# UncleBrian3007/UncleRenderer

Hardware: AMD Instinct MI355X
Metric: shaded Mpixels/s, 4K deferred pass (BuildHZB + CullIndirectArgs + DeferredLighting/Sky), Sponza; % HBM roofline (higher is better)
Workload: dtype f32

## Files before the change

### include/ur_hotpath.h

```cpp
#ifndef UR_HOTPATH_H
#define UR_HOTPATH_H

#include <stddef.h>
#include <stdint.h>

#ifdef __cplusplus
extern "C" {
#endif

#define UR_OK 0
#define UR_EINVAL (-1)
#define UR_EHIP (-2)
#define UR_ENOMEM (-3)
#define UR_ENODEVICE (-4)
#define UR_EUNSUPPORTED (-5)
#define UR_ETIMEOUT (-6)

#define UR_MAX_HZB_MIPS 16u
#define UR_CULL_CONSTANT_DWORDS 46u
#define UR_INDIRECT_COMMAND_STRIDE 64u
#define UR_INDIRECT_INSTANCE_COUNT_OFFSET 44u

typedef struct ur_ctx ur_ctx;

// ... 64 lines not shown
    uint32_t env_mip_count;
    const uint16_t* brdf_lut_rg16;
    uint32_t lut_width;
    uint32_t lut_height;
    uint64_t env_cube_texels;
} ur_lighting_tables;


ur_ctx* ur_create(int device, void* stream);
void ur_destroy(ur_ctx* ctx);
int ur_reserve(ur_ctx* ctx, uint32_t max_instances);
int ur_defer_hzb_tail(ur_ctx* ctx, int mode );
int ur_flush(ur_ctx* ctx);
int ur_debug_set_hzb_timeout(ur_ctx* ctx);
int ur_debug_lighting_schedule(const ur_ctx* ctx, uint32_t out8[8]);
int ur_debug_stream_ceiling(ur_ctx* ctx, const void* in0, const void* in1, const void* in2, const void* in3, void* out, uint64_t elements16,
                            void* start_event, void* stop_event);
int ur_debug_timeline(ur_ctx* ctx, unsigned long long* device_pairs, uint32_t capacity_pairs);
int ur_time_next_lighting(ur_ctx* ctx, void* start_event, void* stop_event);
int ur_time_next_cull(ur_ctx* ctx, void* stop_event);
int ur_time_cull_carried(const ur_ctx* ctx);

#define UR_OPT_LIGHTING_STREAM 1
#define UR_OPT_LIGHTING_WAVES_PER_WG 2
#define UR_OPT_LIGHTING_TILED_WAVES 3
#define UR_OPT_LIGHTING_LEAVE_CUS 4
#define UR_OPT_RIDE_WALKERS 5
#define UR_OPT_CULL_STORE 7
#define UR_OPT_LIGHTING_BALANCE 8
#define UR_OPT_BALANCE_POOL_16THS 9
#define UR_OPT_BALANCE_CHUNK_SHIFT 10
#define UR_OPT_DEBUG_HZB_RIDE_STALL 11
#define UR_OPT_TAA_TONEMAP_HISTORY_STORE 12
int ur_set_option(ur_ctx* ctx, int option, int value);
int ur_get_option(const ur_ctx* ctx, int option, int* value);
const char* ur_last_error(void);
const char* ur_version(void);


uint32_t ur_hzb_layout(uint32_t src_w, uint32_t src_h, ur_mip_desc* mips ,
                       uint32_t* mip_count);

int ur_build_hzb(ur_ctx* ctx, const float* depth, uint32_t src_w, uint32_t src_h, float* hzb_base,
                 const ur_mip_desc* mips, uint32_t mip_count);

typedef struct ur_hzb_slice {
    uint32_t offset;
    uint32_t count;
} ur_hzb_slice;
int ur_hzb_band_pieces(uint32_t src_h, uint32_t n_ranks, uint32_t rank, uint32_t* piece_row0, uint32_t* piece_rows);
int ur_hzb_band_slices(const ur_mip_desc* mips, uint32_t mip_count, uint32_t piece_row0, uint32_t piece_rows, ur_hzb_slice* out5);
int ur_build_hzb_band(ur_ctx* ctx, const float* depth, uint32_t src_w, uint32_t src_h, float* hzb_base, const ur_mip_desc* mips,
                      uint32_t mip_count, uint32_t piece_row0, uint32_t piece_rows);
int ur_build_hzb_tail(ur_ctx* ctx, float* hzb_base, const ur_mip_desc* mips, uint32_t mip_count);


int ur_cull_indirect_args(ur_ctx* ctx, const uint32_t* constants, const ur_float4* bounds,
                          const float* hzb_base, const ur_mip_desc* mips, void* indirect_args,
                          uint32_t* stats2, uint32_t* visible_idx, uint32_t* visible_count);
int ur_cull_indirect_args_ex(ur_ctx* ctx, const uint32_t* constants, const ur_float4* bounds,
                             const float* hzb_base, const ur_mip_desc* mips, void* indirect_args,
                             uint32_t* stats2, uint32_t* visible_idx, uint32_t* visible_count,
                             uint32_t index_base);

typedef struct ur_draw_ranges {
    const uint32_t* offsets;
// ... 146 lines not shown
```

### unclerenderer_amd/csrc/cull.hip

```cpp

#include "cull_kernels.h"

namespace ur {

int launch_cull(ur_ctx* ctx, const uint32_t* constants, const ur_float4* bounds, const float* hzb, const ur_mip_desc* mips,
                void* indirect_args, uint32_t* stats2, uint32_t* visible_idx, uint32_t* visible_count, uint32_t index_base,
                const ur_draw_ranges* draws, const ur_cull_view* views, uint32_t view_count)
{
    const int rc = flush_hzb_tail(ctx);
    if (rc != UR_OK) return rc;
    if (views != nullptr && view_count != 0) return launch_cull_views(ctx, constants, bounds, hzb, mips, indirect_args, stats2, visible_idx, visible_count, index_base, draws, views, view_count);
    return cull_launches<false>(ctx, constants, bounds, hzb, mips, indirect_args, stats2, visible_idx, visible_count, index_base, draws, nullptr, 0);
}

}
```

### unclerenderer_amd/csrc/cull_kernels.h

```cpp
#pragma once

#include "ur_internal.h"
#include "ur_device.h"

#include <hip/hip_ext.h>

#include <algorithm>
#include <cstring>

namespace {

struct CullParams {
    float4 FrustumPlanes[6];
    float ViewProjection[16];
    uint32_t ModelCount, HZBEnabled, HZBMipCount, HZBWidth, HZBHeight, DebugPrintEnabled;
    const float4* bounds;
    const float* hzb;
    uint8_t* args;
    uint32_t* stats;
    uint32_t* visible_idx;
    uint32_t* visible_count;
    uint32_t* block_counts;
    uint64_t* wave_masks;
    uint32_t index_base;
    uint32_t store_flavour;
    uint32_t record_valid;
    uint32_t mip_offset[UR_MAX_HZB_MIPS];
    uint32_t mip_width[UR_MAX_HZB_MIPS];
    unsigned long long* timeline;
};

struct DrawParams {
    const uint32_t* offsets;
    uint8_t* commands;
    uint32_t* counts;
    uint32_t range_count;
};

struct ViewParams {
    float4 planes[UR_MAX_CULL_VIEWS][6];
    uint32_t* mask[UR_MAX_CULL_VIEWS];
    uint32_t* visible_idx[UR_MAX_CULL_VIEWS];
    uint32_t* visible_count[UR_MAX_CULL_VIEWS];
    DrawParams D[UR_MAX_CULL_VIEWS];
    uint32_t* block_counts[UR_MAX_CULL_VIEWS];
    uint64_t* wave_masks[UR_MAX_CULL_VIEWS];
    uint32_t count;
};

template <bool RANGES, bool VIEWS = false> struct CullArgs : CullParams { DrawParams D; ViewParams V; };
template <> struct CullArgs<false, true> : CullParams { ViewParams V; };
template <> struct CullArgs<true, false> : CullParams { DrawParams D; };
template <> struct CullArgs<false, false> : CullParams {};

__device__ __forceinline__ float saturate_f(float x) { return fminf(fmaxf(x, 0.0f), 1.0f); }
__device__ __forceinline__ float dot3(float ax, float ay, float az, float bx, float by, float bz) { return (ax * bx + ay * by) + az * bz; }

__device__ __forceinline__ bool IsAabbVisible(const CullParams& C, float3 mn, float3 mx)
{
#pragma unroll
    for (int i = 0; i < 6; ++i) {
        const float4 plane = C.FrustumPlanes[i];
        const float px = plane.x >= 0.0f ? mx.x : mn.x;
        const float py = plane.y >= 0.0f ? mx.y : mn.y;
        const float pz = plane.z >= 0.0f ? mx.z : mn.z;
        if (dot3(plane.x, plane.y, plane.z, px, py, pz) + plane.w < 0.0f) return false;
    }
    return true;
}

__device__ __forceinline__ bool IsAabbInCameraFrustum(const float4* planes, float4 bmin, float4 bmax)
{
#pragma unroll
    for (int i = 0; i < 6; ++i) {
        const float4 P = planes[i];
        const float X = P.x >= 0.0f ? bmax.x : bmin.x;
        const float Y = P.y >= 0.0f ? bmax.y : bmin.y;
        const float Z = P.z >= 0.0f ? bmax.z : bmin.z;
        const float d = ((P.x * X + P.y * Y) + P.z * Z) + P.w * 1.0f;
        if (d < 0.0f) return false;
    }
    return true;
}

__device__ __forceinline__ bool IsOccluded(const CullParams& C, float3 mn, float3 mx)
{
    if (C.HZBEnabled == 0 || C.HZBWidth == 0 || C.HZBHeight == 0 || C.HZBMipCount == 0) return false;
    const float* M = C.ViewProjection;
    float minUx = 1.0f, minUy = 1.0f, maxUx = 0.0f, maxUy = 0.0f, maxDepth = 0.0f;
    bool anyBehind = false;
#pragma unroll
    for (int i = 0; i < 8; ++i) {
        const float cx = (i & 1) ? mx.x : mn.x, cy = (i & 2) ? mx.y : mn.y, cz = (i & 4) ? mx.z : mn.z;
        const float clx = ((cx * M[0] + cy * M[4]) + cz * M[8]) + 1.0f * M[12];
        const float cly = ((cx * M[1] + cy * M[5]) + cz * M[9]) + 1.0f * M[13];
        const float clz = ((cx * M[2] + cy * M[6]) + cz * M[10]) + 1.0f * M[14];
        const float clw = ((cx * M[3] + cy * M[7]) + cz * M[11]) + 1.0f * M[15];
        if (clw <= 0.0f) anyBehind = true;
        const float nx = clx / clw, ny = cly / clw, nz = clz / clw;
        const float ux = nx * 0.5f + 0.5f;
        const float uy = 1 - (ny * 0.5f + 0.5f);
        minUx = fminf(minUx, ux); minUy = fminf(minUy, uy);
        maxUx = fmaxf(maxUx, ux); maxUy = fmaxf(maxUy, uy);
        maxDepth = fmaxf(maxDepth, nz);
    }
    if (anyBehind) return false;
    if (maxUx < 0.0f || maxUy < 0.0f || minUx > 1.0f || minUy > 1.0f) return false;
    minUx = saturate_f(minUx); minUy = saturate_f(minUy);
    maxUx = saturate_f(maxUx); maxUy = saturate_f(maxUy);
    const float ex = maxUx - minUx, ey = maxUy - minUy;
    const float psx = ex * (float)C.HZBWidth, psy = ey * (float)C.HZBHeight;
    const float maxDim = fmaxf(psx, psy);
    uint32_t mipLevel = 0;
    if (maxDim > 1.0f) {
        const uint32_t e = ((__float_as_uint(maxDim) >> 23) & 0xFFu) - 127u;
        const float l = fminf(fmaxf((float)e, 0.0f), (float)(C.HZBMipCount - 1u));
        mipLevel = (uint32_t)l;
    }
    const uint32_t mipWidth = max(1u, C.HZBWidth >> mipLevel);
// ... 95 lines not shown
#pragma unroll
    for (uint32_t v = 0; v < UR_MAX_CULL_VIEWS; ++v) {
        if (v >= V.count) break;
        const uint64_t m = __ballot(active && IsAabbInCameraFrustum(V.planes[v], bmin, bmax));
        if (V.mask[v] != nullptr && lane < 2u) {
            const uint32_t w = wave_global * 2u + lane;
            if (w < words) V.mask[v][w] = (uint32_t)(m >> (32u * lane));
        }
        if (lane == 0) {
            svmask[v][wave] = m;
            if (!SINGLE_BLOCK && V.wave_masks[v] != nullptr) V.wave_masks[v][wave_global] = m;
        }
    }
}

template <bool SINGLE_BLOCK>
__device__ __forceinline__ void FinishViews(const ViewParams& V, const uint8_t* args, uint32_t n, uint32_t index_base, const uint64_t (*svmask)[4])
{
    const uint32_t tid = threadIdx.x;
#pragma unroll
    for (uint32_t v = 0; v < UR_MAX_CULL_VIEWS; ++v) {
        if (v >= V.count) break;
        const uint32_t total = __popcll(svmask[v][0]) + __popcll(svmask[v][1]) + __popcll(svmask[v][2]) + __popcll(svmask[v][3]);
        if (SINGLE_BLOCK) {
            if (V.visible_idx[v] != nullptr) {
                ScatterBlock(V.visible_idx[v], index_base, 0, svmask[v], 0);
                if (tid == 0) *V.visible_count[v] = total;
            }
            if (V.D[v].range_count != 0) PlaceBlock(V.D[v], args, svmask[v], n);
        } else if (tid == v && V.block_counts[v] != nullptr) V.block_counts[v][blockIdx.x] = total;
    }
}

template <bool SINGLE_BLOCK, bool RANGES, bool VIEWS = false>
__global__ __launch_bounds__(256) void cull_kernel(CullArgs<RANGES, VIEWS> C)
{
    __shared__ float4 sb[512];
    __shared__ uint64_t smask[4];
    __shared__ uint32_t scand[4];
    __shared__ uint8_t slist[256], socc[256];

    const uint32_t tid = threadIdx.x, lane = tid & 63u, wave = tid >> 6;
    const uint32_t first = blockIdx.x * 256u;
    const uint32_t index = first + tid;
    ur::timeline_entry(C.timeline);

    const uint32_t nb = min(512u, (C.ModelCount - first) * 2u);
    const float4* src = C.bounds + (size_t)first * 2u;
    typedef float cf32x4_t __attribute__((ext_vector_type(4)));
    const cf32x4_t* srcv = reinterpret_cast<const cf32x4_t*>(src);
    const cf32x4_t v0 = __builtin_nontemporal_load(srcv + min(tid, nb - 1u)), v1 = __builtin_nontemporal_load(srcv + min(tid + 256u, nb - 1u));
    const float4 s0 = make_float4(v0.x, v0.y, v0.z, v0.w), s1 = make_float4(v1.x, v1.y, v1.z, v1.w);

    bool visible = false, frustumVisible = true, occluded = false;
    const bool active = index < C.ModelCount;
    uint32_t old_word = 0xFFFFFFFFu;
    const bool from_record = !SINGLE_BLOCK && C.store_flavour == 4u && C.record_valid != 0u;
    uint64_t old_mask = 0;
    if (from_record) old_mask = C.wave_masks[(size_t)blockIdx.x * 4u + wave];
    else if (C.store_flavour >= 3u)
        old_word = *reinterpret_cast<const uint32_t*>(C.args + (size_t)min(index, C.ModelCount - 1u) * UR_INDIRECT_COMMAND_STRIDE + UR_INDIRECT_INSTANCE_COUNT_OFFSET);
    if (tid < nb) sb[tid] = s0;
    if (tid + 256u < nb) sb[tid + 256u] = s1;
    __syncthreads();
    if (active) {
        const float4 bmin = sb[2u * tid], bmax = sb[2u * tid + 1u];
        frustumVisible = IsAabbVisible(C, make_float3(bmin.x, bmin.y, bmin.z), make_float3(bmax.x, bmax.y, bmax.z));
    }
    if (SINGLE_BLOCK) {
        if (active && frustumVisible && C.HZBEnabled != 0) {
            const float4 bmin = sb[2u * tid], bmax = sb[2u * tid + 1u];
            occluded = IsOccluded(C, make_float3(bmin.x, bmin.y, bmin.z), make_float3(bmax.x, bmax.y, bmax.z));
        }
    } else if (C.HZBEnabled != 0) {
        const bool cand = active && frustumVisible;
        const uint64_t cm = __ballot(cand);
        if (lane == 0) scand[wave] = (uint32_t)__popcll(cm);
        __syncthreads();
        uint32_t at = 0, total = 0;
#pragma unroll
        for (uint32_t w = 0; w < 4u; ++w) { at += w < wave ? scand[w] : 0u; total += scand[w]; }
        if (cand) slist[at + (uint32_t)__popcll(cm & ((1ull << lane) - 1ull))] = (uint8_t)tid;
        __syncthreads();
        if (tid < total) {
            const uint32_t j = slist[tid];
            const float4 bmin = sb[2u * j], bmax = sb[2u * j + 1u];
            socc[j] = IsOccluded(C, make_float3(bmin.x, bmin.y, bmin.z), make_float3(bmax.x, bmax.y, bmax.z)) ? 1u : 0u;
        }
        __syncthreads();
        occluded = cand && socc[tid] != 0u;
    }
    if (active) {
        visible = frustumVisible && !occluded;
        uint32_t* word = reinterpret_cast<uint32_t*>(C.args + (size_t)index * UR_INDIRECT_COMMAND_STRIDE + UR_INDIRECT_INSTANCE_COUNT_OFFSET);
        const uint32_t value = visible ? 1u : 0u;
        if (C.store_flavour >= 3u) {
            if (from_record) old_word = (uint32_t)(old_mask >> lane) & 1u;
            if (old_word != value) asm volatile("global_store_dword %0, %1, off sc1" ::"v"(word), "v"(value) : "memory");
        } else if (C.store_flavour == 2u) asm volatile("global_store_dword %0, %1, off sc1" ::"v"(word), "v"(value) : "memory");
        else if (C.store_flavour == 1u) __builtin_nontemporal_store(value, word);
        else *word = value;
    }
    [[maybe_unused]] __shared__ uint64_t svmask[VIEWS ? UR_MAX_CULL_VIEWS : 1][4];
    if constexpr (VIEWS) CullViews<SINGLE_BLOCK>(C.V, C.ModelCount, active, sb, svmask);

    if (C.DebugPrintEnabled != 0 && C.stats != nullptr) {
        const uint32_t nf = __popcll(__ballot(active && !frustumVisible));
        const uint32_t no = __popcll(__ballot(active && frustumVisible && occluded));
        if (lane == 0) {
            if (nf) atomicAdd(&C.stats[0], nf);
            if (no) atomicAdd(&C.stats[1], no);
        }
    }

    if (!RANGES && !VIEWS && C.visible_idx == nullptr) {
        if (!SINGLE_BLOCK && C.store_flavour == 4u) {
            const uint64_t m = __ballot(visible);
            if (lane == 0) C.wave_masks[(size_t)blockIdx.x * 4u + wave] = m;
        }
        ur::timeline_exit(C.timeline, tid == 0);
        return;
    }
    const uint64_t mask = __ballot(visible);
    if (lane == 0) smask[wave] = mask;
    __syncthreads();
    if (SINGLE_BLOCK) {
        if ((!RANGES && !VIEWS) || C.visible_idx != nullptr) {
            ScatterBlock(C.visible_idx, C.index_base, 0, smask, 0);
            if (tid == 0) *C.visible_count = __popcll(smask[0]) + __popcll(smask[1]) + __popcll(smask[2]) + __popcll(smask[3]);
        }
        if constexpr (RANGES) PlaceBlock(C.D, C.args, smask, C.ModelCount);
    } else {
        if (lane == 0) C.wave_masks[(size_t)blockIdx.x * 4u + wave] = mask;
        if (tid == 0) C.block_counts[blockIdx.x] = __popcll(smask[0]) + __popcll(smask[1]) + __popcll(smask[2]) + __popcll(smask[3]);
    }
    if constexpr (VIEWS) FinishViews<SINGLE_BLOCK>(C.V, C.args, C.ModelCount, C.index_base, svmask);
    ur::timeline_exit(C.timeline, tid == 0);
}

template <bool VIEWS, class Args> __device__ __forceinline__ const auto* SelectRow(const Args* C, const CullArgs<true>* W)
{
    if constexpr (VIEWS) return W;
    else return C;
}

template <bool RANGES, bool VIEWS> struct CompactRow { typedef CullArgs<true> type; };
template <bool RANGES> struct CompactRow<RANGES, false> { typedef CullArgs<RANGES> type; };

template <bool RANGES, bool VIEWS = false>
__global__ __launch_bounds__(256) void compact_kernel(CullArgs<RANGES, VIEWS> C, uint32_t num_blocks)
{
    [[maybe_unused]] CullArgs<true> W{};
    if constexpr (VIEWS) {
        W.ModelCount = C.ModelCount;
        W.args = C.args;
        W.index_base = C.index_base;
        if (blockIdx.y == 0) {
            W.wave_masks = C.wave_masks;
            W.block_counts = C.block_counts;
            W.visible_idx = C.visible_idx;
            W.visible_count = C.visible_count;
            if constexpr (RANGES) W.D = C.D;
        } else {
#pragma unroll
            for (uint32_t v = 0; v < UR_MAX_CULL_VIEWS; ++v) {
                if (v + 1u != blockIdx.y) continue;
                W.wave_masks = C.V.wave_masks[v];
                W.block_counts = C.V.block_counts[v];
                W.visible_idx = C.V.visible_idx[v];
                W.visible_count = C.V.visible_count[v];
                W.D = C.V.D[v];
            }
// ... 94 lines not shown
        const uint32_t b = __builtin_ctzll(bits);
        A.visible_idx[at++] = first + b;
        bits &= bits - 1ull;
    }
    if (mi == num_masks - 1u) *A.visible_count = at;
}

struct ZeroArgs {
    uint32_t* count[1 + UR_MAX_CULL_VIEWS];
    uint32_t* counts[1 + UR_MAX_CULL_VIEWS];
    uint32_t range_count[1 + UR_MAX_CULL_VIEWS];
};
__global__ void zero_views_kernel(ZeroArgs Z)
{
    const uint32_t i = blockIdx.x * 256u + threadIdx.x;
#pragma unroll
    for (uint32_t k = 0; k < 1u + UR_MAX_CULL_VIEWS; ++k) {
        if (i == 0 && Z.count[k]) *Z.count[k] = 0;
        if (i < Z.range_count[k]) Z.counts[k][i] = 0;
    }
}

template <class K, class... Args>
int launch_stop(ur_ctx* ctx, hipEvent_t stop, K kernel, dim3 grid, const Args&... args)
{
    if (stop != nullptr) hipExtLaunchKernelGGL(kernel, grid, dim3(256), 0, ctx->stream, nullptr, stop, 0, args...);
    else hipLaunchKernelGGL(kernel, grid, dim3(256), 0, ctx->stream, args...);
    UR_HIP_TRY(hipGetLastError());
    return UR_OK;
}

DrawParams draw_params(const ur_draw_ranges& d) { return {d.offsets, static_cast<uint8_t*>(d.commands), d.counts, d.range_count}; }

template <bool VIEWS>
int cull_launches(ur_ctx* ctx, const uint32_t* constants, const ur_float4* bounds, const float* hzb, const ur_mip_desc* mips,
                  void* indirect_args, uint32_t* stats2, uint32_t* visible_idx, uint32_t* visible_count, uint32_t index_base,
                  const ur_draw_ranges* draws, const ur_cull_view* views, uint32_t view_count)
{
    if constexpr (!VIEWS) view_count = 0;
    CullArgs<true, VIEWS> P{};
    static_assert(sizeof(float4) * 6 + sizeof(float) * 16 + 6 * 4 == UR_CULL_CONSTANT_DWORDS * 4, "46 dwords");
    std::memcpy(static_cast<CullParams*>(&P), constants, UR_CULL_CONSTANT_DWORDS * 4);
    P.bounds = reinterpret_cast<const float4*>(bounds);
    P.hzb = hzb;
    P.args = static_cast<uint8_t*>(indirect_args);
    P.stats = stats2;
    P.visible_idx = visible_idx;
    P.visible_count = visible_count;
    P.index_base = index_base;
    P.store_flavour = (uint32_t)ctx->opt.cull_store;
    P.timeline = P.ModelCount != 0 ? ur::next_timeline_pair(ctx) : nullptr;
    if (P.HZBEnabled != 0) {
        for (uint32_t m = 0; m < P.HZBMipCount && m < UR_MAX_HZB_MIPS; ++m) {
            P.mip_offset[m] = mips[m].offset;
            P.mip_width[m] = mips[m].width;
        }
    }
    if (draws) P.D = draw_params(*draws);
    if constexpr (VIEWS) {
        P.V.count = view_count;
        for (uint32_t v = 0; v < view_count; ++v) {
            std::memcpy(P.V.planes[v], views[v].planes, sizeof(P.V.planes[v]));
            P.V.mask[v] = views[v].mask;
            P.V.visible_idx[v] = views[v].visible_idx;
            P.V.visible_count[v] = views[v].visible_count;
            if (views[v].draws) P.V.D[v] = draw_params(*views[v].draws);
        }
    }
    const uint32_t n = P.ModelCount;
    bool record_valid = P.store_flavour == 4u && ctx->cull_record_args == indirect_args && ctx->cull_record_n == n;
    ctx->cull_record_args = nullptr;
    hipEvent_t stop = ctx->time_cull_stop;
    auto compacted = [&](uint32_t v) { return views[v].visible_idx != nullptr || views[v].draws != nullptr; };

    if (n == 0) {
        ZeroArgs Z{};
        Z.count[0] = visible_count;
        if (draws) { Z.counts[0] = draws->counts; Z.range_count[0] = draws->range_count; }
        bool zero = visible_count != nullptr || draws != nullptr;
        uint32_t most = Z.range_count[0];
        for (uint32_t v = 0; v < view_count; ++v) {
            zero = zero || views[v].visible_count || views[v].draws;
            Z.count[1 + v] = views[v].visible_count;
            if (views[v].draws) {
                Z.counts[1 + v] = views[v].draws->counts;
                Z.range_count[1 + v] = views[v].draws->range_count;
                most = std::max(most, views[v].draws->range_count);
            }
        }
        if (!zero) return UR_OK;
// ... 22 lines not shown
        }
        P.block_counts = ctx->block_counts;
        P.wave_masks = ctx->wave_masks;
        if constexpr (VIEWS) {
            const uint32_t stride = ctx->ws_instances / 256u;
            for (uint32_t v = 0; v < view_count; ++v) {
                if (!compacted(v)) continue;
                compact = true;
                P.V.block_counts[v] = ctx->block_counts + (size_t)(1u + v) * stride;
                P.V.wave_masks[v] = ctx->wave_masks + (size_t)(1u + v) * stride * 4u;
            }
        }
    }
    P.record_valid = record_valid ? 1u : 0u;
    static_cast<CullParams&>(Q) = P;
    if constexpr (VIEWS) Q.V = P.V;
    const dim3 compaction_grid((blocks * 4u + 255u) / 256u, 1u + view_count);
    if (draws) {
        rc = launch_stop(ctx, compact ? nullptr : stop, cull_kernel<false, true, VIEWS>, dim3(blocks), P);
        if (rc == UR_OK && compact) rc = launch_stop(ctx, stop, compact_kernel<true, VIEWS>, compaction_grid, P, blocks);
    } else {
        rc = launch_stop(ctx, compact ? nullptr : stop, cull_kernel<false, false, VIEWS>, dim3(blocks), Q);
        if (rc == UR_OK && compact) rc = launch_stop(ctx, stop, compact_kernel<false, VIEWS>, compaction_grid, Q, blocks);
    }
    if (rc != UR_OK) return rc;
    if (P.store_flavour == 4u) {
        ctx->cull_record_args = indirect_args;
        ctx->cull_record_n = n;
    }
    ctx->time_cull_carried = stop != nullptr;
    return UR_OK;
}

}
```

### unclerenderer_amd/csrc/debug_print.hip

```cpp

#include "ur_internal.h"

namespace {

constexpr uint32_t kHeaderDwords = 1u;
constexpr uint32_t kEntryDwords = 4u;
constexpr uint32_t kMaxEntries = UR_DEBUG_PRINT_MAX_ENTRIES;
constexpr uint32_t kAdvance = 8u;
constexpr uint32_t kTextChunk = 256u;

__device__ __forceinline__ void print_char(uint32_t* buf, uint32_t x, uint32_t y, uint32_t code, uint32_t color)
{
    const uint32_t index = atomicAdd(buf, 1u);
    if (index >= kMaxEntries) return;
    uint32_t* e = buf + kHeaderDwords + index * kEntryDwords;
    e[0] = x; e[1] = y; e[2] = code; e[3] = color;
}

__device__ void print_label(uint32_t* buf, uint32_t x, uint32_t y, uint32_t color, const char (&c)[9])
{
    for (uint32_t i = 0; i < 8u; ++i) {
        const uint32_t code = (uint32_t)(uint8_t)c[i];
        if (code == 0u) return;
        print_char(buf, x, y, code, color);
// ... 148 lines not shown
        const int iu = (int)fu;
        const float dv = g.UvMax[1] - g.UvMin[1];
#pragma unroll
        for (uint32_t k = 0; k < kRowsPerThread; ++k) {
            const uint32_t ly = ly0 + k * kRowStep;
            const float cy = (float)(p.row0 + ly) + 0.5f;
            if (!(ly < p.rows && q.miny <= cy && cy < q.maxy)) continue;
            const float v = g.UvMin[1] + (cy - q.miny) / g.Size[1] * dv;
            const float tv = v * ah - 0.5f, fv = floorf(tv), wv = tv - fv;
            const int iv = (int)fv;
            const float t00 = atlas_texel(p, iu, iv), t10 = atlas_texel(p, iu + 1, iv), t01 = atlas_texel(p, iu, iv + 1), t11 = atlas_texel(p, iu + 1, iv + 1);
            const float top = t00 + (t10 - t00) * wu, bot = t01 + (t11 - t01) * wu;
            const float a = ca * (top + (bot - top) * wv);
            const uint32_t d = pix[k];
            const float ia = 1.0f - a;
            const float dr = (float)(d & 255u) / 255.0f, dg = (float)((d >> 8) & 255u) / 255.0f, db = (float)((d >> 16) & 255u) / 255.0f;
            pix[k] = unorm8(cr * a + dr * ia) | (unorm8(cg * a + dg * ia) << 8) | (unorm8(cb * a + db * ia) << 16) | (unorm8(a) << 24);
            dirty |= 1u << k;
        }
    }
#pragma unroll
    for (uint32_t k = 0; k < kRowsPerThread; ++k) {
        const uint32_t ly = ly0 + k * kRowStep;
        if (dirty & (1u << k)) p.ldr[(size_t)ly * p.w + px] = pix[k];
    }
}

}

namespace ur {

int launch_debug_print_reset(ur_ctx* ctx, void* buffer, uint32_t* stats)
{
    hipLaunchKernelGGL(debug_print_reset_kernel, dim3(1), dim3(64), 0, ctx->stream, static_cast<uint32_t*>(buffer), stats);
    UR_HIP_TRY(hipGetLastError());
    return UR_OK;
}

int launch_debug_print_stats(ur_ctx* ctx, const uint32_t* stats, void* buffer)
{
    hipLaunchKernelGGL(debug_print_stats_kernel, dim3(1), dim3(64), 0, ctx->stream, stats, static_cast<uint32_t*>(buffer));
    UR_HIP_TRY(hipGetLastError());
    return UR_OK;
}

int launch_debug_print_text(ur_ctx* ctx, void* buffer, uint32_t x, uint32_t y, uint32_t color, const char* text, uint32_t length)
{
    uint32_t n = 0;
    while (n < length && text[n] != 0) ++n;
    for (uint32_t at = 0; at < n; at += kTextChunk) {
        TextChunk chunk = {};
        const uint32_t count = n - at < kTextChunk ? n - at : kTextChunk;
        for (uint32_t i = 0; i < count; ++i) chunk.c[i] = (uint8_t)text[at + i];
        hipLaunchKernelGGL(debug_print_text_kernel, dim3(1), dim3(kTextChunk), 0, ctx->stream, static_cast<uint32_t*>(buffer), x + kAdvance * at, y, color,
                           count, chunk);
        UR_HIP_TRY(hipGetLastError());
    }
    return UR_OK;
}

int launch_debug_print_draw(ur_ctx* ctx, const ur_debug_print_constants* constants, const ur_debug_glyph* glyphs, uint32_t glyph_count,
                            const uint8_t* atlas_r8, uint32_t atlas_w, uint32_t atlas_h, const void* buffer, uint32_t* ldr_inout, uint32_t w,
                            uint32_t row0, uint32_t rows)
{
    if (rows == 0) return UR_OK;
    DrawParams p{};
    p.glyphs = glyphs; p.atlas = atlas_r8; p.buf = static_cast<const uint32_t*>(buffer); p.ldr = ldr_inout;
    p.glyph_count = glyph_count; p.atlas_w = atlas_w; p.atlas_h = atlas_h;
    p.first_char = constants->FirstChar; p.char_count = constants->CharCount;
    p.w = w; p.row0 = row0; p.rows = rows;
    const dim3 grid((w + kTileW - 1u) / kTileW, (rows + kTileH - 1u) / kTileH);
    if (grid.y > 65535u) { set_error("ur_debug_print_draw: band too tall"); return UR_EUNSUPPORTED; }
    hipLaunchKernelGGL(debug_print_draw_kernel, grid, dim3(kThreads), 0, ctx->stream, p);
    UR_HIP_TRY(hipGetLastError());
    return UR_OK;
}

}
```

### unclerenderer_amd/csrc/frame/HotPathRenderer.cpp

```cpp

#include "HotPathRenderer.h"

#include <hip/hip_runtime.h>

#include <cstdio>
#include <cstring>
#include <sstream>

#include "../../../include/ur_frame.h"
#include "../../../include/ur_host.h"
#include "../ur_internal.h"

int FHotPathRenderer::RenderFrame(FHIPCommandContext& Cmd, FHotPathResources& Res, const FHotPathFrameConstants& Constants,
                                  const FHotPathOptions& Options)
{
    PassError = UR_OK;
    if (bPostPending) {
        bPostPending = false;
        bLuminanceHistoryValid = false;
        ResetTaa();
    }
    FRenderGraph Graph;
    Graph.SetDevice(Device);
    Graph.SetGpuTimingEnabled(Options.bGpuTiming);
// ... 947 lines not shown
    O.bTaaBand = (flags & UR_FRAME_TAA_BAND) != 0;
    O.bDebugPrint = (flags & UR_FRAME_DEBUG_PRINT) != 0;
    O.bShardHZB = (flags & UR_FRAME_HZB_SHARD) != 0 && f->Cmd.GetWorldSize() > 1;
    O.bAsyncCompute = (flags & UR_FRAME_ASYNC_COMPUTE) != 0;
    if (O.bAsyncCompute && !f->AsyncCtx) {
        int dev = 0;
        if (hipGetDevice(&dev) != hipSuccess || hipStreamCreateWithPriority(&f->AsyncStream, hipStreamNonBlocking, -1) != hipSuccess) return UR_EHIP;
        f->AsyncCtx = ur_create(dev, f->AsyncStream);
        if (!f->AsyncCtx) return UR_EHIP;
        f->Cmd.SetAsyncCompute(f->AsyncCtx, f->AsyncStream);
    }
    O.bTimeLighting = (flags & (UR_FRAME_TIME_LIGHTING | UR_FRAME_TIME_LIGHTING_RECORD_COST | UR_FRAME_TIME_LIGHTING_KERNEL)) != 0;
    f->bKernelEvents = (flags & UR_FRAME_TIME_LIGHTING_KERNEL) != 0;
    f->bRecordAfter = (flags & UR_FRAME_TIME_LIGHTING_RECORD_COST) != 0;
    O.bGpuTiming = (flags & UR_FRAME_GPU_TIMING) != 0;
    O.bGraphDump = (flags & UR_FRAME_GRAPH_DUMP) != 0;
    O.bBarrierLogs = (flags & UR_FRAME_BARRIER_LOGS) != 0;
    f->Cmd.SetJoinAsyncAtEnd((flags & UR_FRAME_ASYNC_NO_JOIN) == 0);
    f->Cmd.BeginFrame();
    const bool chain_with_lighting = (flags & UR_FRAME_HZB_WITH_LIGHTING) != 0 && !O.bAsyncCompute;
    const bool tail_with_lighting = (chain_with_lighting || (flags & UR_FRAME_HZB_TAIL_WITH_LIGHTING) != 0) && !O.bAsyncCompute;
    if (tail_with_lighting) (void)ur_defer_hzb_tail(f->Cmd.GetContext(), chain_with_lighting ? 2 : 1);
    f->bStartOnCull = false;
    if (f->bKernelEvents && chain_with_lighting && O.bEnableIndirectDraw && O.bHZBEnabled && O.bDoDepthPrepass && R.IndirectArgs && R.ModelBounds &&
        R.IndirectCommandCount != 0) {
        constexpr size_t kRing = 1024;
        if (f->LightEvents.size() < kRing && f->LightCount == f->LightEvents.size()) {
            hipEvent_t a = nullptr, b = nullptr, c = nullptr;
            if (hipEventCreate(&a) == hipSuccess && hipEventCreate(&b) == hipSuccess && hipEventCreate(&c) == hipSuccess) f->LightEvents.push_back({a, b, c, false, false});
        }
        if (!f->LightEvents.empty() && ur_time_next_cull(f->Cmd.GetContext(), f->LightEvents[f->LightCount % f->LightEvents.size()].first) == UR_OK)
            f->bStartOnCull = true;
    }
    const int rc = f->Renderer.RenderFrame(f->Cmd, R, K, O);
    (void)ur_time_next_cull(f->Cmd.GetContext(), nullptr);
    if (tail_with_lighting) {
        const int rc2 = ur_defer_hzb_tail(f->Cmd.GetContext(), 0);
        const int rc3 = ur_flush(f->Cmd.GetContext());
        return rc != UR_OK ? rc : (rc2 != UR_OK ? rc2 : rc3);
    }
    return rc;
}

void ur_frame_join_async(ur_frame* f) { if (f) f->Cmd.JoinAsyncCompute(); }
int ur_frame_hzb_ready(const ur_frame* f) { return f && f->Renderer.IsHZBReady() ? 1 : 0; }
void ur_frame_reset_hzb(ur_frame* f) { if (f) f->Renderer.ResetHZB(); }

int ur_frame_set_post(ur_frame* f, const ur_frame_post* post)
{
    if (!f || !post) { ur::set_error("ur_frame_set_post: null argument"); return UR_EINVAL; }
    f->Post = *post;
    return UR_OK;
}

int ur_frame_set_draw_ranges(ur_frame* f, const ur_draw_ranges* draws)
{
    if (!f) { ur::set_error("ur_frame_set_draw_ranges: null frame"); return UR_EINVAL; }
    if (draws && (!draws->offsets || !draws->commands || !draws->counts || draws->range_count == 0)) {
        ur::set_error("ur_frame_set_draw_ranges: null member / no range");
        return UR_EINVAL;
    }
    f->bDrawRanges = draws != nullptr;
    f->DrawRanges = draws ? *draws : ur_draw_ranges{};
    return UR_OK;
}

int ur_frame_set_cull_views(ur_frame* f, const ur_cull_view* views, uint32_t count)
// ... 165 lines not shown
```

### unclerenderer_amd/csrc/gbuffer_resolve.hip

```cpp

#include "raster_rule.h"
#include "texture_sample.h"
#include "ur_device.h"
#include "ur_internal.h"

namespace {

using namespace ur_raster;

static_assert(sizeof(ur_texture2d) == 16 && sizeof(ur_material) == 80, "ur_material is 80 bytes");

struct ResolveParams {
    const uint8_t* commands;
    uint32_t mode;
    const uint32_t* visible_idx;
    uint32_t index_base;
    float V[16], Pr[16];
    const uint32_t* keys;
    uint2* gbuf_a; uint2* gbuf_b; uint32_t* gbuf_c; uint2* hdr; uint32_t* object_id;
    const float* table;
    uint32_t w, row0, n;
    float half_w, half_h;
    uint32_t key_bits;
    const ur_material* materials;
// ... 288 lines not shown
    ur::store_once_b64(p.gbuf_a + i, pack_half4(m[0] / ml, m[1] / ml, m[2] / ml, view_depth));
    ur::store_once_b64(p.gbuf_b + i, pack_half4(0.04f, cb[104], cb[105], 1.0f));
    ur::store_once_b32(p.gbuf_c + i, r8 | (g8 << 8) | (b8 << 16) | 0xFF000000u);
    ur::store_once_b64(p.hdr + i, pack_half4(cb[80], cb[81], cb[82], 1.0f));
    if constexpr (OBJECT_ID) ur::store_once_b32(p.object_id + i, reinterpret_cast<const uint32_t*>(cb)[148]);
}

int gbuffer_entry(const char* who, const char* who_parts, ur_ctx* ctx, const float* view, const float* projection, const ur_raster_draws* draws, const float* depth,
                  const ur_gbuffer_targets* targets, uint32_t w, uint32_t h, uint32_t row0, uint32_t rows, uint32_t flags, uint32_t key_triangle_bits,
                  uint32_t* stats6, uint32_t parts, const ur_material* materials, uint32_t material_count)
{
    int rc = ur::check_raster_call(who, ctx, view, projection, draws, depth, "depth", w, h, stats6);
    if (rc == UR_OK) rc = ur::check_depth_flags(who, flags);
    if (rc == UR_OK) rc = ur::check_gbuffer_targets(who, targets);
    if (rc == UR_OK) rc = ur::check_key_triangle_bits(who, key_triangle_bits);
    if (rc != UR_OK) return rc;
    if (rows == 0u || (uint64_t)row0 + rows > h) { ur::set_error("%s: rows [%u, %u + %u) of a target %u high", who, row0, row0, rows, h); return UR_EINVAL; }
    if (parts == 0u || (parts & ~(UR_GBUFFER_PART_RASTER | UR_GBUFFER_PART_RESOLVE))) { ur::set_error("%s: parts 0x%x (UR_GBUFFER_PART_RASTER | UR_GBUFFER_PART_RESOLVE)", who_parts, parts); return UR_EINVAL; }
    uint32_t key_bits = key_triangle_bits;
    if (key_bits == 0u) {
        if (draws->command_count >= (1u << 24)) {
            ur::set_error("%s: %u command slots leave fewer than 8 key bits for the triangle: pass key_triangle_bits", who, draws->command_count);
            return UR_EUNSUPPORTED;
        }
        uint32_t length = 0u;
        while ((draws->command_count >> length) != 0u) ++length;
        key_bits = min(32u - length, 31u);
    } else if ((uint64_t)draws->command_count >= (1ull << (32u - key_bits))) {
        ur::set_error("%s: %u command slots do not fit the %u key bits beside key_triangle_bits %u", who, draws->command_count, 32u - key_bits, key_bits);
        return UR_EINVAL;
    }
    if (!aligned(materials, 16)) { ur::set_error("%s: a misaligned material table (16 bytes)", who); return UR_EINVAL; }
    const uint32_t n = w * rows;
    if (parts & UR_GBUFFER_PART_RASTER) {
        rc = ur::launch_visibility_raster(ctx, view, projection, draws, depth, targets->keys, w, h, row0, rows, key_bits, (flags & UR_DEPTH_QUANTIZE_D24) != 0u, stats6);
        if (rc != UR_OK) return rc;
    }
    if (!(parts & UR_GBUFFER_PART_RESOLVE)) return UR_OK;
    ResolveParams r{};
    r.commands = static_cast<const uint8_t*>(ur::raster_commands(*draws));
    r.mode = draws->visible_idx != nullptr ? 1u : 0u;
    r.visible_idx = draws->visible_idx; r.index_base = draws->index_base;
    for (int k = 0; k < 16; ++k) { r.V[k] = view[k]; r.Pr[k] = projection[k]; }
    r.keys = targets->keys;
    r.gbuf_a = reinterpret_cast<uint2*>(targets->gbuf_a); r.gbuf_b = reinterpret_cast<uint2*>(targets->gbuf_b); r.gbuf_c = targets->gbuf_c;
    r.hdr = reinterpret_cast<uint2*>(targets->hdr); r.object_id = targets->object_id;
    r.table = ctx->srgb_encode_table;
    r.w = w; r.row0 = row0; r.n = n;
    r.half_w = 0.5f * (float)w; r.half_h = 0.5f * (float)h;
    r.key_bits = key_bits;
    const uint32_t blocks = (n + kThreads - 1u) / kThreads;
    if (materials) {
        r.materials = materials; r.material_count = material_count;
        r.decode = ctx->srgb_table; r.lod = ctx->lod_table;
        if (targets->object_id) hipLaunchKernelGGL((gbuffer_resolve_kernel<true, true>), dim3(blocks), dim3(kThreads), 0, ctx->stream, r);
        else hipLaunchKernelGGL((gbuffer_resolve_kernel<false, true>), dim3(blocks), dim3(kThreads), 0, ctx->stream, r);
        UR_HIP_TRY(hipGetLastError());
        return UR_OK;
    }
    if (targets->object_id) hipLaunchKernelGGL(gbuffer_resolve_kernel<true>, dim3(blocks), dim3(kThreads), 0, ctx->stream, r);
    else hipLaunchKernelGGL(gbuffer_resolve_kernel<false>, dim3(blocks), dim3(kThreads), 0, ctx->stream, r);
    UR_HIP_TRY(hipGetLastError());
    return UR_OK;
}

}
// ... 49 lines not shown
```

### unclerenderer_amd/csrc/hzb.hip

```cpp

#include "ur_internal.h"
#include "ur_device.h"
#include "hzb_tail.h"
#include "hzb_wide.h"

namespace {

using ur::HzbDispatch;

using ur::hzb_min4;

__global__ __launch_bounds__(256) void hzb_reduce4_kernel(HzbDispatch p)
{
    __shared__ float sh2[4][16];
    __shared__ float sh3[2][8];

    const uint32_t tx = threadIdx.x & 31u, ty = threadIdx.x >> 5;
    const uint32_t by = blockIdx.y + p.by0;
    const uint32_t x1 = blockIdx.x * 32u + tx, y1 = by * 8u + ty;
    const uint32_t sx = x1 * 4u, sy = y1 * 4u;

    float v0[2][2] = {{1.0f, 1.0f}, {1.0f, 1.0f}};
    const bool any0 = (x1 * 2u < p.W[0]) && (y1 * 2u < p.H[0]);
    if (any0) {
// ... 57 lines not shown
    if (((tx | ty) & 3u) == 0u) {
        const uint32_t x3 = x1 >> 2, y3 = y1 >> 2;
        if (x3 < p.W[3] && y3 < p.H[3]) {
            const uint32_t cx = tx >> 1, cy = ty >> 1;
            const float v3 = hzb_min4(sh2[cy][cx], sh2[cy][cx + 1], sh2[cy + 1][cx], sh2[cy + 1][cx + 1]);
            p.dst[3][(size_t)y3 * p.W[3] + x3] = v3;
            sh3[ty >> 2][tx >> 2] = v3;
        }
    }
    if (p.mips < 5u) return;
    __syncthreads();

    if (threadIdx.x < 4u) {
        const uint32_t x4 = blockIdx.x * 4u + threadIdx.x, y4 = by;
        if (x4 < p.W[4] && y4 < p.H[4]) {
            const uint32_t c0 = min(2u * x4, p.W[3] - 1u) & 7u, c1 = min(2u * x4 + 1u, p.W[3] - 1u) & 7u;
            const uint32_t r0 = min(2u * y4, p.H[3] - 1u) & 1u, r1 = min(2u * y4 + 1u, p.H[3] - 1u) & 1u;
            p.dst[4][(size_t)y4 * p.W[4] + x4] = hzb_min4(sh3[r0][c0], sh3[r0][c1], sh3[r1][c0], sh3[r1][c1]);
        }
    }
}

__global__ __launch_bounds__(1024) void hzb_tail_kernel(ur::HzbTail p)
{
    __shared__ float bufA[ur::kTailTexels], bufB[ur::kTailTexels / 2];
    ur::hzb_tail_run(p, bufA, bufB);
}

}

namespace ur {

static HzbTail make_tail(float* hzb, const ur_mip_desc* mips, uint32_t mip_count, uint32_t mip);

int launch_build_hzb(ur_ctx* ctx, const float* depth, uint32_t src_w, uint32_t src_h, float* hzb, const ur_mip_desc* mips,
                     uint32_t mip_count)
{
    {
        const int rc = flush_hzb_tail(ctx);
        if (rc != UR_OK) return rc;
    }
    uint32_t mip = 0;
    while (mip < mip_count) {
        if (mip > 0 && (uint64_t)mips[mip].width * mips[mip].height <= kTailTexels && mip_count - mip <= kTailMaxLevels) {
            const HzbTail t = make_tail(hzb, mips, mip_count, mip);
            if (ctx->defer_hzb_tail) {
                ctx->pending_tail = t;
                ctx->hzb_tail_pending = true;
                break;
            }
            hipLaunchKernelGGL(hzb_tail_kernel, dim3(1), dim3(1024), 0, ctx->stream, t);
            UR_HIP_TRY(hipGetLastError());
            break;
        }
        uint32_t n = (mip_count - mip) < 4u ? (mip_count - mip) : 4u;
        if (mip == 0 && mip_count > 4u && (uint64_t)mips[4].width * mips[4].height <= kTailTexels) n = 5u;
        else if (mip == 0 && mip_count > 5u && (uint64_t)mips[5].width * mips[5].height <= kTailTexels &&
                 mip_count - 5u <= kTailMaxLevels) n = 5u;
        HzbDispatch d{};
        if (mip == 0) {
            d.src = depth;
            d.SW = src_w;
            d.SH = src_h;
        } else {
            d.src = hzb + mips[mip - 1].offset;
            d.SW = mips[mip - 1].width;
            d.SH = mips[mip - 1].height;
        }
        for (uint32_t k = 0; k < 5; ++k) {
            if (k < n) {
                d.dst[k] = hzb + mips[mip + k].offset;
                d.W[k] = mips[mip + k].width;
// ... 20 lines not shown
        hipLaunchKernelGGL(hzb_reduce4_kernel, grid, dim3(256), 0, ctx->stream, d);
        UR_HIP_TRY(hipGetLastError());
        mip += n;
    }
    return UR_OK;
}

static bool chain_is_wide_plus_tail(const ur_mip_desc* mips, uint32_t mip_count)
{
    return mip_count > 5u && (uint64_t)mips[5].width * mips[5].height <= kTailTexels && mip_count - 5u <= kTailMaxLevels;
}

static HzbTail make_tail(float* hzb, const ur_mip_desc* mips, uint32_t mip_count, uint32_t mip)
{
    HzbTail t{};
    t.src = hzb + mips[mip - 1].offset;
    t.SW = mips[mip - 1].width;
    t.SH = mips[mip - 1].height;
    t.first_mip = mip;
    t.levels = mip_count - mip;
    for (uint32_t k = 0; k < t.levels; ++k) {
        t.dst[k] = hzb + mips[mip + k].offset;
        t.W[k] = mips[mip + k].width;
        t.H[k] = mips[mip + k].height;
        t.magic[k] = t.W[k] > 1u ? (uint32_t)((1ull << 32) / t.W[k] + 1ull) : 0u;
    }
    return t;
}

int launch_build_hzb_band(ur_ctx* ctx, const float* depth, uint32_t src_w, uint32_t src_h, float* hzb, const ur_mip_desc* mips, uint32_t mip_count,
                          uint32_t piece_row0, uint32_t piece_rows)
{
    {
        const int rc = flush_hzb_tail(ctx);
        if (rc != UR_OK) return rc;
    }
    if (!chain_is_wide_plus_tail(mips, mip_count)) {
        set_error("ur_build_hzb_band: a %u x %u frame's chain is not one five-level launch plus the tail (build it whole: ur_build_hzb)", src_w, src_h);
        return UR_EUNSUPPORTED;
    }
    HzbDispatch d{};
    d.src = depth; d.SW = src_w; d.SH = src_h;
    for (uint32_t k = 0; k < 5; ++k) { d.dst[k] = hzb + mips[k].offset; d.W[k] = mips[k].width; d.H[k] = mips[k].height; }
    d.mips = 5u;
    d.vec4_ok = ((d.SW & 3u) == 0u && (reinterpret_cast<uintptr_t>(d.src) & 15u) == 0u) ? 1u : 0u;
    d.pair_ok = ((d.W[0] & 1u) == 0u && (reinterpret_cast<uintptr_t>(d.dst[0]) & 7u) == 0u) ? 1u : 0u;
    d.by0 = piece_row0;
    const dim3 grid((d.W[0] + 63u) / 64u, piece_rows);
    if (piece_rows == 0u) return UR_OK;
    if (ctx->defer_hzb_tail && ctx->defer_hzb_wide) {
        ctx->pending_wide = d;
        ctx->pending_wide_grid_x = grid.x;
        ctx->pending_wide_grid_y = grid.y;
        ctx->hzb_wide_pending = true;
        return UR_OK;
    }
    hipLaunchKernelGGL(hzb_reduce4_kernel, grid, dim3(256), 0, ctx->stream, d);
    UR_HIP_TRY(hipGetLastError());
    return UR_OK;
}

int launch_build_hzb_tail(ur_ctx* ctx, float* hzb, const ur_mip_desc* mips, uint32_t mip_count)
{
    {
        const int rc = flush_hzb_tail(ctx);
        if (rc != UR_OK) return rc;
    }
    if (!chain_is_wide_plus_tail(mips, mip_count)) {
        set_error("ur_build_hzb_tail: the chain is not one five-level launch plus the tail");
        return UR_EUNSUPPORTED;
    }
    hipLaunchKernelGGL(hzb_tail_kernel, dim3(1), dim3(1024), 0, ctx->stream, make_tail(hzb, mips, mip_count, 5u));
    UR_HIP_TRY(hipGetLastError());
    return UR_OK;
}

int flush_hzb_tail(ur_ctx* ctx)
{
    if (ctx->hzb_wide_pending) {
        ctx->hzb_wide_pending = false;
        hipLaunchKernelGGL(hzb_reduce4_kernel, dim3(ctx->pending_wide_grid_x, ctx->pending_wide_grid_y), dim3(256), 0, ctx->stream, ctx->pending_wide);
        UR_HIP_TRY(hipGetLastError());
    }
    if (!ctx->hzb_tail_pending) return UR_OK;
    ctx->hzb_tail_pending = false;
    hipLaunchKernelGGL(hzb_tail_kernel, dim3(1), dim3(1024), 0, ctx->stream, ctx->pending_tail);
    UR_HIP_TRY(hipGetLastError());
    return UR_OK;
}

}
```

### unclerenderer_amd/csrc/lighting.hip

```cpp

#include "lighting_device.h"
#include "ur_device.h"
#include "hzb_tail.h"

#include <cstring>

namespace {

using namespace ur;

typedef float f2_t __attribute__((ext_vector_type(2)));
__device__ __forceinline__ f2_t f2(float x, float y) { return f2_t{x, y}; }

__device__ __forceinline__ float shadow_pcf_border_inline(const float* __restrict__ map, int W, int H, int ia, int ja, float fx, float fy, float cmp)
{
    float acc = 0.0f;
#pragma unroll
    for (int r = 0; r < 3; ++r) {
        float s = 0.0f;
        const int yj = ja + r;
        const uint32_t rowo = (uint32_t)min(max(yj, 0), H - 1) * (uint32_t)W;
#pragma unroll
        for (int c = 0; c < 3; ++c) {
            const int xi = ia + c;
            const bool in = (uint32_t)xi < (uint32_t)W && (uint32_t)yj < (uint32_t)H;
            const float t = in ? ld<float>(map, (rowo + (uint32_t)min(max(xi, 0), W - 1)) * 4u) : 1.0f;
            s += cmp <= t ? (c == 0 ? 1.0f - fx : (c == 1 ? 1.0f : fx)) : 0.0f;
        }
        acc = fmaf(r == 0 ? 1.0f - fy : (r == 1 ? 1.0f : fy), s, acc);
    }
    return 0.25f * acc;
}

constexpr uint32_t kLutE = kLutW + 2;
constexpr uint32_t kLdsSrgb = 0;
constexpr uint32_t kLdsIrrBytes = 6 * 9 * 64;
// ... 119 lines not shown
    uint32_t r;
    asm("s_cmp_eq_u64 %1, -1\n\ts_cselect_b32 %0, 1, 0" : "=s"(r) : "s"(m) : "scc");
    return r;
}

struct __attribute__((aligned(16))) MipEntry { float Nf, rowBf, faceBf, offBf; };

template <class V>
__device__ __forceinline__ void need(const V& a, const V& b, const V& c, const V& d)
{
    asm volatile("" ::"v"(a), "v"(b), "v"(c), "v"(d));
}

__device__ __forceinline__ uint32_t dyn_slot_load(const uint32_t* slot)
{
    return __builtin_amdgcn_readfirstlane(__hip_atomic_load(slot, __ATOMIC_RELAXED, __HIP_MEMORY_SCOPE_WORKGROUP));
}
template <class P>
__device__ __forceinline__ uint32_t dyn_slot_wait(const uint32_t* slot, P kp)
{
    uint32_t e = dyn_slot_load(slot), spins = 0;
    while (e == kDynNotReady) {
        __builtin_amdgcn_s_sleep(8);
        e = dyn_slot_load(slot);
        if (++spins > (1u << 21)) {
            __hip_atomic_store(kp->bal.timedOut, 1u, __ATOMIC_RELAXED, __HIP_MEMORY_SCOPE_SYSTEM);
            e = kDynEnd;
            break;
        }
    }
    return e;
}
template <class P>
__device__ __forceinline__ uint32_t dyn_claim(P kp, uint32_t* work, uint32_t* dynT, uint32_t c, uint32_t lane)
{
    const uint32_t d = c - kp->hot.staticClaims;
    const uint32_t s = min(d >> kp->bal.dynShift, kDynSlots - 1u);
    const uint32_t e = dyn_slot_wait(dynT + s, kp);
    if (e >= kDynEnd) return 0xFFFFFFFFu;
    const uint32_t idx = d & ((1u << kp->bal.dynShift) - 1u);
    if (idx == 0u) {
        const uint32_t k = s + kp->bal.lookahead;
        if (k < kDynSlots) {
            uint32_t out = kDynEnd;
            if (dyn_slot_wait(dynT + (k - 1u), kp) < kDynEnd && k + 1u < kDynSlots) {
                uint32_t v = 0;
                if (lane == 0) v = __hip_atomic_fetch_add(kp->bal.words + (blockIdx.x >> 3) * ur::kClaimWordStride, 1u, __ATOMIC_RELAXED, __HIP_MEMORY_SCOPE_AGENT);
                v = __builtin_amdgcn_readfirstlane(v);
                if (v < dyn_slot_load(work + 5)) out = kp->bal.staticTiles + ((dyn_slot_load(work + 4) + v) << kp->bal.dynShift);
                else {
                    uint32_t done = 0;
                    if (lane == 0) done = __hip_atomic_fetch_add(kp->bal.words + ur::kClaimWords * ur::kClaimWordStride, 1u, __ATOMIC_RELAXED, __HIP_MEMORY_SCOPE_AGENT);
                    if (__builtin_amdgcn_readfirstlane(done) == kp->hot.groups - 1u && lane <= ur::kClaimWords)
                        __hip_atomic_store(kp->bal.words + lane * ur::kClaimWordStride, 0u, __ATOMIC_RELAXED, __HIP_MEMORY_SCOPE_AGENT);
                }
            }
            if (lane == 0) __hip_atomic_store(dynT + k, out, __ATOMIC_RELAXED, __HIP_MEMORY_SCOPE_WORKGROUP);
        }
    }
    return e + idx;
}

__device__ __forceinline__ void store_hdr(void* base, uint32_t byte_offset, uint32_t lo, uint32_t hi)
{
    typedef uint32_t u32x2_t __attribute__((ext_vector_type(2)));
    const u32x2_t v = {lo, hi};
    asm volatile("global_store_dwordx2 %0, %1, %2 sc1 nt" ::"v"(byte_offset), "v"(v), "s"(base) : "memory");
}

struct HzbRide {
    ur::HzbDispatch d;
    uint32_t grid_x, pieces;
    uint32_t walkers;
    uint32_t want;
    uint32_t spin_limit;
    uint32_t pad;
    uint32_t* done;
    uint32_t* timed_out;
};

template <int MODE, bool SHADOWS, bool IRR_LDS, int WPB, bool RIDE_ALL>
__global__ __launch_bounds__(64 * WPB, 1) void lighting_stream_kernel(LightingParams p, ur::HzbTail hzbTail, HzbRide hzbRide)
{
    static_assert(MODE != ur::UR_MODE_SKY, "sky-only uses the per-tile kernel");
    ur::warm_kernarg<sizeof(LightingParams)>();
    extern __shared__ __attribute__((aligned(16))) unsigned char smem[];
    ur::timeline_entry(p.timeline);
    if (blockIdx.x >= p.hot.groups) {
        if constexpr (WPB == 16) {
            static_assert(kLdsTiles + 16u * 2u * kTileBytes >= (ur::kTailTexels + ur::kTailTexels / 2u) * sizeof(float), "the tail's two level buffers fit the launch's LDS");
            float* bufA = reinterpret_cast<float*>(smem);
            auto ka = __builtin_amdgcn_kernarg_segment_ptr();
            asm volatile("" : "+s"(ka));
            typedef const __attribute__((address_space(4))) ur::HzbTail* KTail;
            typedef const __attribute__((address_space(4))) HzbRide* KRide;
            static_assert(sizeof(LightingParams) % 8 == 0 && sizeof(ur::HzbTail) % 8 == 0, "the kernel arguments follow one another without padding");
            const KRide ride = (KRide)((const __attribute__((address_space(4))) char*)ka + sizeof(LightingParams) + sizeof(ur::HzbTail));
            if (ride->pieces != 0u) {
                if (threadIdx.x == 0) {
                    uint32_t* done = ride->done;
                    const uint32_t want = ride->want, limit = ride->spin_limit;
                    const bool stale = __hip_atomic_load(done + 1, __ATOMIC_RELAXED, __HIP_MEMORY_SCOPE_AGENT) != 0u;
                    uint32_t spins = 0;
                    bool gave_up = false;
                    while (__hip_atomic_load(done, __ATOMIC_RELAXED, __HIP_MEMORY_SCOPE_AGENT) < want) {
                        __builtin_amdgcn_s_sleep(32);
                        if (++spins > limit) { gave_up = true; break; }
                    }
                    __builtin_amdgcn_fence(__ATOMIC_ACQUIRE, "agent");
                    asm volatile("s_waitcnt vmcnt(0)" ::: "memory");
                    if (gave_up || stale) {
                        __hip_atomic_store(ride->timed_out, 1u, __ATOMIC_RELAXED, __HIP_MEMORY_SCOPE_SYSTEM);
                        if (gave_up) __hip_atomic_store(done + 1, 1u, __ATOMIC_RELAXED, __HIP_MEMORY_SCOPE_AGENT);
                    } else {
                        __hip_atomic_store(done, 0u, __ATOMIC_RELAXED, __HIP_MEMORY_SCOPE_AGENT);
                    }
                }
                __syncthreads();
            }
            if (ride->pieces != 0u) ur::hzb_tail_run<true>(*(KTail)((const __attribute__((address_space(4))) char*)ka + sizeof(LightingParams)), bufA, bufA + ur::kTailTexels);
            else ur::hzb_tail_run<false>(*(KTail)((const __attribute__((address_space(4))) char*)ka + sizeof(LightingParams)), bufA, bufA + ur::kTailTexels);
        }
        ur::timeline_exit(p.timeline, threadIdx.x == 0);
        return;
    }
    float* srgb = reinterpret_cast<float*>(smem + kLdsSrgb);
    MipEntry* mipT = reinterpret_cast<MipEntry*>(smem + kLdsMip);
    float4a* irrT = reinterpret_cast<float4a*>(smem + kLdsIrr);
    float2* lut = reinterpret_cast<float2*>(smem + kLdsLut);
    uint32_t* work = reinterpret_cast<uint32_t*>(smem + kLdsWork);
    uint32_t* dynT = reinterpret_cast<uint32_t*>(smem + kLdsDyn);

    const uint32_t lane = threadIdx.x & 63u;
    const uint32_t wave = __builtin_amdgcn_readfirstlane(threadIdx.x >> 6);
    constexpr uint32_t T = 64 * WPB, kLutN = kLutE * (kLutH + 2u), kLutTrips = (kLutN + T - 1) / T;
    uint32_t lt[kLutTrips];
#pragma unroll
    for (uint32_t k = 0; k < kLutTrips; ++k) {
        const uint32_t i = min(threadIdx.x + k * T, kLutN - 1u);
        const uint32_t by = i / kLutE, bx = i - by * kLutE;
        const uint32_t sx = min(max(bx, 1u), kLutW) - 1u, sy = min(max(by, 1u), kLutH) - 1u;
        lt[k] = p.lut[sy * kLutW + sx];
    }
    const float sv = threadIdx.x < 256u ? p.srgb[threadIdx.x] : 0.0f;
    half4_t ih = {}, ih10 = {}, ih01 = {}, ih11 = {};
    const uint32_t irrE = p.irrN0 + 2u;
    const uint32_t irrC = p.irrN0 + 1u, irrCount = IRR_LDS ? 6u * irrC * irrC : 0u;
    if (threadIdx.x < irrCount) {
        const uint32_t f = threadIdx.x / (irrC * irrC), r = threadIdx.x - f * irrC * irrC, cj = r / irrC, ci = r - cj * irrC;
        const uint32_t t0 = p.irrOffset0 + (f * irrE + cj) * irrE + ci;
        ih = p.env[t0]; ih10 = p.env[t0 + 1u]; ih01 = p.env[t0 + irrE]; ih11 = p.env[t0 + irrE + 1u];
    }
    constexpr uint32_t cs = kChunkShift, cmask = (1u << cs) - 1u;
    const uint32_t chunkStride = p.hot.groups << cs, base = blockIdx.x << cs;
    uint32_t tile = (wave >> cs) * chunkStride + base + (wave & cmask);
    uint32_t tile1 = ((wave + WPB) >> cs) * chunkStride + base + ((wave + WPB) & cmask);
    const bool have0 = tile < p.hot.numTiles;
    uint32_t ty = (uint32_t)(((uint64_t)tile * p.hot.tilesXMagic) >> 32), tx = tile - ty * p.hot.tilesX;
    uint32_t ty1 = (uint32_t)(((uint64_t)tile1 * p.hot.tilesXMagic) >> 32), tx1 = tile1 - ty1 * p.hot.tilesX;
    const uint32_t col = lane & 15u, row = lane >> 4;
    const TileSrc src = tile_src<MODE>(&p, lane, 3u);
    const uint32_t bufBase = __builtin_amdgcn_readfirstlane(lds_address(smem + kLdsTiles + wave * (2u * kTileBytes)));
    const unsigned char* myTiles = smem + kLdsTiles + wave * (2u * kTileBytes);
    const uint32_t laneHdr = (row * p.hot.W + col) * 8u;


    if (have0) tile_prefetch<MODE>(&p, p.hot.W, p.hot.rows, src, lane, tx, ty, bufBase);
    const uint32_t cubeLds = __builtin_amdgcn_readfirstlane(lds_address(smem + kLdsTiles + WPB * (2u * kTileBytes)));
    const uint32_t cubeLdsAdj = p.hot.cubeLdsBase - cubeLds;
    {
        const uint32_t nb = p.hot.cubeLdsBytes;
        for (uint32_t pc = wave; pc * 1024u < nb; pc += WPB) {
            const uint32_t at = min(pc * 1024u + lane * 16u, nb - 16u);
            dma16(reinterpret_cast<const char*>(p.hot.env) + p.hot.cubeLdsBase + at, cubeLds + pc * 1024u);
        }
    }
    const float ndcxL = fmaf((float)col, p.invW2, 0.5f * p.invW2 - 1.0f);
    const float rowh = (float)row + 0.5f;
    const float negBig = vreg(-0x1p126f);
    float R[9], WC[3], shC[3], shT[3];
#pragma unroll
    for (int k = 0; k < 9; ++k) R[k] = vreg(p.hot.R[k]);
#pragma unroll
    for (int k = 0; k < 3; ++k) {
        WC[k] = vreg(p.hot.WC[k]); shC[k] = vreg(p.hot.shC[k]); shT[k] = vreg(p.hot.shT[k]);
    }
    {
        if (threadIdx.x == 0) { work[0] = 2u * WPB; work[1] = 0u; work[2] = 0u; work[3] = 0u; }
        if (p.bal.poolChunks != 0u && threadIdx.x < kDynSlots) {
            const uint32_t q8 = blockIdx.x & ~7u, nq = min(8u, p.hot.groups - q8), j = blockIdx.x - q8, la = p.bal.lookahead;
            const uint32_t P0 = (uint32_t)(((unsigned long long)q8 * p.bal.poolMagic) >> 32);
            const uint32_t P1 = (uint32_t)(((unsigned long long)(q8 + nq) * p.bal.poolMagic) >> 32);
            const uint32_t first = P0 + la * nq;
            dynT[threadIdx.x] = threadIdx.x < la ? p.bal.staticTiles + ((P0 + j * la + threadIdx.x) << p.bal.dynShift) : kDynNotReady;
            if (threadIdx.x == 0) { work[4] = first; work[5] = P1 - first; }
        }
        if (threadIdx.x < 256u) srgb[threadIdx.x] = sv;
        if (threadIdx.x < irrCount) {
            const float a[3] = {(float)ih.x, (float)ih.y, (float)ih.z}, b[3] = {(float)ih10.x, (float)ih10.y, (float)ih10.z};
            const float c[3] = {(float)ih01.x, (float)ih01.y, (float)ih01.z}, d[3] = {(float)ih11.x, (float)ih11.y, (float)ih11.z};
            float A_[3], B_[3], C_[3], D_[3];
#pragma unroll
            for (int k = 0; k < 3; ++k) { A_[k] = a[k]; B_[k] = b[k] - a[k]; C_[k] = c[k] - a[k]; D_[k] = (d[k] - b[k]) - (c[k] - a[k]); }
            irrT[threadIdx.x * 4u + 0u] = float4a{A_[0], A_[1], B_[0], B_[1]};
            irrT[threadIdx.x * 4u + 1u] = float4a{C_[0], C_[1], D_[0], D_[1]};
            irrT[threadIdx.x * 4u + 2u] = float4a{A_[2], B_[2], C_[2], D_[2]};
        }
        if (threadIdx.x < 17u) {
            const uint32_t m = min(threadIdx.x, p.envMips - 1u);
            const uint32_t N = max(1u, p.envBase >> m), E = N + 2u;
            uint32_t bordered = 0u, before = 0u;
            for (uint32_t k = 0; k < p.envMips; ++k) {
                const uint32_t e = max(1u, p.envBase >> k) + 2u;
                bordered += 6u * e * e;
                if (k < m) before += 6u * e * (e - 1u);
            }
            mipT[threadIdx.x] = MipEntry{(float)N, (float)(12u * E), (float)(12u * E * (E - 1u)), (float)(bordered * 8u + before * 12u)};
        }
#pragma unroll
        for (uint32_t k = 0; k < kLutTrips; ++k) {
            const uint32_t i = threadIdx.x + k * T;
            if (i < kLutN) lut[i] = float2{(float)(lt[k] & 0xFFFFu) * (1.0f / 65535.0f), (float)(lt[k] >> 16) * (1.0f / 65535.0f)};
        }
    }
    __syncthreads();
    if (have0 && tile1 < p.hot.numTiles) {
        tile_prefetch<MODE>(&p, p.hot.W, p.hot.rows, src, lane, tx1, ty1, bufBase + kTileBytes);
        asm volatile("s_waitcnt vmcnt(2)" ::: "memory");
    } else {
        asm volatile("s_waitcnt vmcnt(0)" ::: "memory");
    }
    if (lane == 0) __hip_atomic_fetch_add(work + 3, 1u, __ATOMIC_RELAXED, __HIP_MEMORY_SCOPE_WORKGROUP);

    if constexpr (WPB == 16) {
        constexpr uint32_t kWalkers = WPB;
        if (RIDE_ALL || wave == kWalkers - 1u) {
            auto ka = __builtin_amdgcn_kernarg_segment_ptr();
            asm volatile("" : "+s"(ka));
            typedef const __attribute__((address_space(4))) HzbRide* KRide;
            const KRide ride = (KRide)((const __attribute__((address_space(4))) char*)ka + sizeof(LightingParams) + sizeof(ur::HzbTail));
            const uint32_t pieces = ride->pieces;
            if (pieces != 0u) {
                const uint32_t gx = ride->grid_x, groups = p.hot.groups;
                float* sh2 = reinterpret_cast<float*>(smem + kLdsHzb) + (RIDE_ALL ? wave * 80u : 0u);
                const uint32_t first = RIDE_ALL ? blockIdx.x + (kWalkers - 1u - wave) * groups : blockIdx.x, step = RIDE_ALL ? groups * kWalkers : groups;
                __builtin_amdgcn_s_setprio(3);
                for (uint32_t piece = first; piece < pieces; piece += step) {
                    const uint32_t by = piece / gx, bx = piece - by * gx;
                    ur::hzb_wide_piece_by_one_wave<true>(ride->d, bx, by + ride->d.by0, lane, sh2, sh2 + 64);
                }
                asm volatile("s_waitcnt vmcnt(0)" ::: "memory");
                __builtin_amdgcn_s_setprio(0);
                bool signals = true;
                if (RIDE_ALL) {
                    uint32_t before = 0;
                    if (lane == 0) before = __hip_atomic_fetch_add(work + 2, 1u, __ATOMIC_RELAXED, __HIP_MEMORY_SCOPE_WORKGROUP);
                    signals = __builtin_amdgcn_readfirstlane(before) == kWalkers - 1u;
                }
                uint32_t* done = ride->done;
                if (signals && done != nullptr) {
                    uint64_t keep_exec;
                    const uint32_t zero = 0u, one = 1u;
                    asm volatile("s_mov_b64 %0, exec\n\ts_mov_b64 exec, 1\n\tglobal_atomic_add %1, %2, %3\n\ts_mov_b64 exec, %0"
                                 : "=&s"(keep_exec)
                                 : "v"(zero), "v"(one), "s"(done)
                                 : "memory");
                }
            }
        }
    }

    uint32_t parity = 0;
#define UR_PREFETCH_POINT()                                                                                              \
    do {                                                                                                                 \
        const uint32_t c = __builtin_amdgcn_readfirstlane(claim);             \
        if (__builtin_expect(c >= p.hot.staticClaims, 0)) tile2 = dyn_claim(kp, work, dynT, c, lane);       \
        else tile2 = (c >> cs) * chunkStride + base + (c & cmask);                                                       \
        uint32_t in_band;                                                                                                \
        asm("s_cmp_lt_u32 %1, %2\n\ts_cselect_b32 %0, 1, 0" : "=s"(in_band) : "s"(tile2), "s"(p.hot.numTiles) : "scc"); \
        more2 = in_band & more1;                                                 \
        if (more2) {                                                                                                     \
            ty2 = __builtin_amdgcn_readfirstlane((uint32_t)(((uint64_t)tile2 * p.hot.tilesXMagic) >> 32));                  \
            tx2 = tile2 - ty2 * p.hot.tilesX;                                                                               \
            tile_prefetch<MODE>(kp, p.hot.W, p.hot.rows, src, lane, tx2, ty2, bufBase + parity * kTileBytes);                  \
        } else {                                                                                                         \
            tile2 = 0xFFFFFFFFu;                                                           \
        }                                                                                                                \
    } while (0)
    while (have0) {
        const KParams kp = fresh_params();
        uint32_t tile2 = 0xFFFFFFFFu, tx2 = 0, ty2 = 0;
        uint32_t more2 = 0u;
        uint32_t more1;
        asm("s_cmp_lt_u32 %1, %2\n\ts_cselect_b32 %0, 1, 0" : "=s"(more1) : "s"(__builtin_amdgcn_readfirstlane(tile1)), "s"(p.hot.numTiles) : "scc");
        uint32_t claim = 0;
        if (more1 && lane == 0) claim = __hip_atomic_fetch_add(work, 1u, __ATOMIC_RELAXED, __HIP_MEMORY_SCOPE_WORKGROUP);
        __builtin_amdgcn_s_setprio(0);
        const unsigned char* buf = myTiles + parity * kTileBytes;
        const uint2 ga = *reinterpret_cast<const uint2*>(buf + lane * 8u);
        const uint2 gb = *reinterpret_cast<const uint2*>(buf + 512u + lane * 8u);
        const uint2 gd = *reinterpret_cast<const uint2*>(buf + 1024u + lane * 8u);
        const uint32_t gc = *reinterpret_cast<const uint32_t*>(buf + 1536u + lane * 4u);
        const float ndcx = fmaf((float)(tx * 16u), p.hot.invW2, ndcxL), ndcy = fmaf((float)(p.hot.row0 + ty * 4u) + rowh, p.hot.invH2, -1.0f);

        bool sky = false;
        uint32_t all_sky = 0u;
        F3 out = f3(0.0f, 0.0f, 0.0f);
        if (MODE == ur::UR_MODE_FUSED) {
            const float depth = *reinterpret_cast<const float*>(buf + 1792u + lane * 4u);
// ... 237 lines not shown
#undef UR_CHANNEL
            }
            if (!sky) {
                out = f3(h2f_lo(gd.x) + colxy.x, h2f_hi(gd.x) + colxy.y, h2f_lo(gd.y) + colz);
                outw = h2f_hi(gd.y) + 1.0f;
            }
        } else {
            __builtin_amdgcn_sched_barrier(0);
            asm volatile("s_waitcnt vmcnt(0)" ::: "memory");
            UR_PREFETCH_POINT();
            __builtin_amdgcn_sched_barrier(0);
        }
        if (ty * 4u + row < p.hot.rows) {
            half4_t o;
            o.x = (_Float16)out.x; o.y = (_Float16)out.y; o.z = (_Float16)out.z; o.w = (_Float16)outw;
            uint2 ob;
            __builtin_memcpy(&ob, &o, 8);
            store_hdr(p.hot.hdr, ((ty * 4u) * p.hot.W + tx * 16u) * 8u + laneHdr, ob.x, ob.y);
        }
        if (!more1) break;
        tile = tile1; tile1 = tile2;
        tx = tx1; ty = ty1; tx1 = tx2; ty1 = ty2;
        parity ^= 1u;
    }
#undef UR_PREFETCH_POINT
    unsigned long long* const tl = fresh_params()->timeline;
    if (tl != nullptr) {
        uint32_t left = 0;
        if (lane == 0) left = __hip_atomic_fetch_add(work + 1, 1u, __ATOMIC_RELAXED, __HIP_MEMORY_SCOPE_WORKGROUP);
        ur::timeline_exit(tl, lane == 0 && left == WPB - 1u);
    }
}

typedef void (*kernel_t)(LightingParams, ur::HzbTail, HzbRide);
#define UR_WAVES(M, S, I) lighting_stream_kernel<M, S, I, 12, true>, lighting_stream_kernel<M, S, I, 12, false>, lighting_stream_kernel<M, S, I, 16, true>, lighting_stream_kernel<M, S, I, 16, false>
#define UR_MODE(M) UR_WAVES(M, true, true), UR_WAVES(M, true, false), UR_WAVES(M, false, true), UR_WAVES(M, false, false)
const kernel_t kStreamKernels[32] = {UR_MODE(ur::UR_MODE_LIGHTING), UR_MODE(ur::UR_MODE_FUSED)};
#undef UR_MODE
#undef UR_WAVES

}

namespace ur {

int launch_lighting_stream(ur_ctx* ctx, const LightingParams& params, int mode, bool shadows, bool irr_lds)
{
    const uint32_t wpb = ctx->opt.lighting_wpb == 12 ? 12u : 16u;
    const ur_ctx::Options& o = ctx->opt;
    const StreamPlan s = plan_stream({ctx->cu_count, o.leave_cus, o.ride_walkers, o.balance, o.balance_pool_16ths, o.balance_chunk_shift, o.debug_hzb_ride_stall,
                                      params.W, params.rows, wpb, ctx->hzb_tail_pending, ctx->hzb_wide_pending, ctx->pending_wide_grid_x,
                                      ctx->pending_wide_grid_y, ctx->claim_words != nullptr ? kClaimWords : 0u});
    LightingParams p = params;
    p.timeline = next_timeline_pair(ctx);
    StreamHot& h = p.hot;
    h.tilesX = s.tilesX; h.numTiles = s.numTiles; h.tilesXMagic = s.tilesXMagic; h.groups = s.groups; h.staticClaims = s.staticClaims;
    p.bal = Balance{};
    if (s.poolChunks != 0u) p.bal = Balance{s.poolChunks, s.staticTiles, s.dynShift, s.lookahead, s.poolMagic, ctx->claim_words, ctx->claim_timed_out_dev};
    HzbTail tail{};
    HzbRide ride{};
    if (s.carry_tail) { tail = ctx->pending_tail; ctx->hzb_tail_pending = false; }
    if (s.rides) {
        ride.d = ctx->pending_wide;
        ride.grid_x = s.ride_grid_x; ride.pieces = s.ride_pieces; ride.walkers = s.ride_walkers; ride.spin_limit = s.ride_spin_limit;
        if (s.carry_tail) { ride.done = ctx->hzb_done; ride.timed_out = ctx->hzb_timed_out_dev; }
        ctx->hzb_wide_pending = false;
    } else if (s.flush_first) {
        const int frc = flush_hzb_tail(ctx);
        if (frc != UR_OK) return frc;
    }
    ride.want = s.ride_want;
    const bool ride_all = ride.pieces != 0u && ride.walkers > 1u;
    const uint32_t form = (mode == UR_MODE_FUSED ? 16u : 0u) | (shadows ? 0u : 8u) | (irr_lds ? 0u : 4u) | (wpb == 16u ? 2u : 0u) | (ride_all ? 0u : 1u);
    const kernel_t kern = kStreamKernels[form];
    const uint32_t lds = kLdsTiles + wpb * 2u * kTileBytes + kLdsCubeBytes;
    static bool attr_set[32][64] = {};
    const int dev = ctx->device >= 0 && ctx->device < 64 ? ctx->device : -1;
    if (dev < 0 || !attr_set[form][dev]) {
        UR_HIP_TRY(hipFuncSetAttribute(reinterpret_cast<const void*>(kern), hipFuncAttributeMaxDynamicSharedMemorySize, (int)lds));
        if (dev >= 0) attr_set[form][dev] = true;
    }
    std::memcpy(ctx->last_schedule, s.reported, sizeof(ctx->last_schedule));
    launch_timed(ctx, kern, dim3(s.groups + (s.carry_tail ? 1u : 0u)), dim3(64 * wpb), lds, p, tail, ride);
    return UR_OK;
}

}
```

### unclerenderer_amd/csrc/lighting_host.hip

```cpp

#include "lighting_params.h"

#include <algorithm>
#include <cmath>
#include <cstring>

namespace {

void mat4_mul(const float* a, const float* b, float* o)
{
    for (int i = 0; i < 4; ++i)
        for (int j = 0; j < 4; ++j) {
            float s = 0.0f;
            for (int k = 0; k < 4; ++k) s += a[i * 4 + k] * b[k * 4 + j];
            o[i * 4 + j] = s;
        }
}

}

namespace ur {

int launch_lighting(ur_ctx* ctx, const ur_scene_constants* S, const ur_sky_constants* K, const ur_half4* A, const ur_half4* B,
                    const uint32_t* C, const float* depth, const ur_lighting_tables* T, ur_half4* hdr, uint32_t w, uint32_t h,
// ... 141 lines not shown
            h.skyInvP11 = p.skyInvP11; h.nSkyInvP22 = -p.skyInvP22;
            h.skyNearOverR2 = p.skyNearOverR * p.skyNearOverR;
            h.maxMip = p.maxMip;
            h.envMaxLevel = (float)(p.envMips - 1u);
            const uint32_t iE = p.irrN0 + 2u;
            h.irrN0 = p.irrN0; h.irrNf = (float)p.irrN0; h.irrEf = (float)iE; h.irrEEf = (float)(iE * iE);
            if (p.irrN0 <= 2u) { h.irrEf = (float)(p.irrN0 + 1u); h.irrEEf = (float)((p.irrN0 + 1u) * (p.irrN0 + 1u)); }
            h.irrOfff = (float)p.irrOffset0; h.irrRowBytes = iE * 8u;
            h.env = p.env; h.hdr = p.hdr;
            for (int k = 0; k < 9; ++k) h.R[k] = p.R[k];
            for (int k = 0; k < 3; ++k) {
                h.Lw[k] = (p.L[0] * p.R[k] + p.L[1] * p.R[3 + k]) + p.L[2] * p.R[6 + k];
                h.WA[k] = p.invP11 * p.R[k];
                h.WB[k] = -p.invP22 * p.R[3 + k];
                h.WC[k] = p.R[6 + k];
                h.lightRGB[k] = p.lightRGB[k];
            }
            {
                const double vx = p.skyInvP11, vy = p.skyInvP22;
                h.skyDepthMax = (float)(p.skyNearOverR * std::sqrt(vx * vx + vy * vy + 1.0) * (1.0 + 1e-5));
            }
            {
                const uint32_t first = cube_first_mip_within(cube, kLdsCubeBytes);
                h.cubeLdsLevel = first < p.envMips ? (float)first : 16.0f;
                h.cubeLdsBase = (uint32_t)cube.pairs[first];
                h.cubeLdsBytes = (uint32_t)(cube.bytes - cube.pairs[first]);
            }
            streamed = true;
            const int rc = launch_lighting_stream(ctx, p, mode, shadows, p.irrN0 <= 2u);
            if (rc != UR_OK) return rc;
        }
    }
    if (!streamed) {
        const int frc = flush_hzb_tail(ctx);
        if (frc != UR_OK) return frc;
        launch_lighting_tiled(ctx, p, mode, shadows);
    }
    UR_HIP_TRY(hipGetLastError());
    return UR_OK;
}

}
```

### unclerenderer_amd/csrc/lighting_params.h

```cpp
#pragma once

#include "ur_internal.h"
#include "lighting_plan.h"

#include <hip/hip_ext.h>

namespace ur {

typedef _Float16 half4_t __attribute__((ext_vector_type(4)));
typedef _Float16 half2_t __attribute__((ext_vector_type(2)));

struct StreamHot {
    uint32_t groups;
    uint32_t tilesX, numTiles, tilesXMagic, W, rows, row0, irrN0, irrRowBytes;
    uint32_t staticClaims;
    float invW2, invH2, invP11, nInvP22;
    float skyInvP11, nSkyInvP22, skyNearOverR2, maxMip;
    float envMaxLevel, irrNf, irrEf, irrEEf, irrOfff;
    float shadowWm3, shadowHm3, shadowWf;
    float shadowXmax, shadowYmax, shadowStrength, shadowQuarterStrength, shadowOneMinusStrength;
    uint32_t shadowRowBytes;
    int32_t shadowWi, shadowHi;
    const void* env;
    const float* shadow;
// ... 14 lines not shown
    unsigned long long poolMagic;
    uint32_t* words;
    uint32_t* timedOut;
};

struct LightingParams {
    uint32_t W, H, row0, rows;
    float invW2, invH2;
    float invP11, invP22;
    float L[3];
    float R[9];
    float SQ[12];
    float VIt[3], camPos[3];
    uint32_t general;
    uint32_t shadowSmall;
    float ST[4];
    float lightRGB[3];
    float shadowStrength, shadowBias;
    float shadowW, shadowH, shadowTexelX, shadowTexelY;
    int32_t shadowWi, shadowHi;
    float maxMip;
    uint32_t envBase, envMips;
    uint32_t envMipOffset[16];
    uint32_t irrOffset0, irrOffset1, irrN0, irrN1;
    float irrFrac;
    uint32_t lutW, lutH;
    float skyRot[9];
    float skyInvP11, skyInvP22;
    float skyNearOverR;
    float sunDir[3];
    float skyScatterR[3];
    float skyMie[3];
    float sunAttenuation;
    StreamHot hot;
    Balance bal;
    unsigned long long* timeline;
    const half4_t* A;
    const half4_t* B;
    const uint32_t* C;
    const float* depth;
    const float* shadow;
    const half4_t* env;
    const uint32_t* lut;
    const float* srgb;
    half4_t* hdr;
};

constexpr uint32_t kLutW = 128, kLutH = 32;

template <class K, class... Args>
void launch_timed(ur_ctx* ctx, K kern, dim3 grid, dim3 block, uint32_t lds, Args... args)
{
    if (ctx->time_stop != nullptr) {
        hipExtLaunchKernelGGL(kern, grid, block, lds, ctx->stream, ctx->time_start, ctx->time_stop, 0, args...);
        ctx->time_start = ctx->time_stop = nullptr;
    } else {
        hipLaunchKernelGGL(kern, grid, block, lds, ctx->stream, args...);
    }
}

int launch_lighting_stream(ur_ctx* ctx, const LightingParams& p, int mode, bool shadows, bool irr_lds);
void launch_lighting_tiled(ur_ctx* ctx, const LightingParams& p, int mode, bool shadows);

}
```

### unclerenderer_amd/csrc/lighting_plan.cpp

```cpp
#include "lighting_plan.h"

#include <algorithm>

namespace ur {

CubeLayout cube_layout(uint32_t base_size, uint32_t mip_count)
{
    CubeLayout L{};
    if (base_size == 0 || mip_count == 0 || mip_count > 16) return L;
    L.mips = mip_count;
    uint64_t texels = 0;
    for (uint32_t m = 0; m < mip_count; ++m) {
        L.edge[m] = std::max(1u, base_size >> m) + 2u;
        L.bordered[m] = texels;
        texels += 6u * L.edge[m] * L.edge[m];
    }
    uint64_t bytes = texels * 8u;
    for (uint32_t m = 0; m < mip_count; ++m) {
        L.pairs[m] = bytes;
        bytes += 6u * L.edge[m] * (L.edge[m] - 1u) * 12u;
        texels += 9u * L.edge[m] * (L.edge[m] - 1u);
    }
    L.pairs[mip_count] = L.bytes = bytes;
    L.texels = texels;
// ... 5 lines not shown
    uint32_t first = L.mips;
    while (first > 0 && L.bytes - L.pairs[first - 1u] <= budget) --first;
    return first;
}

uint32_t ride_walkers(uint32_t pieces, uint32_t tiles, uint32_t lighting_groups, uint32_t wpb, int forced)
{
    const double per_group = (double)pieces / lighting_groups, tiles_per_wave = (double)tiles / (lighting_groups * wpb);
    uint32_t wk = 1;
    while (wk < wpb && (double)wk * tiles_per_wave < 7.0 * per_group) wk *= 2;
    if (forced >= 1) wk = (uint32_t)forced;
    return wk >= 4u ? wpb : 1u;
}

StreamPlan plan_stream(const StreamPlanInput& in)
{
    StreamPlan s{};
    const uint32_t WPB = in.wpb;
    s.tilesX = in.W / 16u;
    s.numTiles = s.tilesX * ((in.rows + 3u) / 4u);
    const int cus = std::max(in.cus, 1);
    const int leave_cus = std::min(in.leave_cus, cus - 1);
    const bool can_ride = WPB == 16u && cus >= 16;
    s.carry_tail = in.tail_pending && can_ride && cus - leave_cus >= 2;
    s.rides = in.wide_pending && (s.carry_tail || (!in.tail_pending && can_ride));
    if (s.rides) {
        s.ride_grid_x = in.wide_grid_x;
        s.ride_pieces = in.wide_grid_x * in.wide_grid_y;
        if (s.carry_tail) s.ride_spin_limit = in.debug_hzb_ride_stall != 0 ? (1u << 9) : (1u << 22);
        s.ride_walkers = ride_walkers(s.ride_pieces, s.numTiles, (uint32_t)std::max(1, cus - (s.carry_tail ? 1 : 0) - leave_cus), WPB, in.ride_walkers);
    } else {
        s.flush_first = in.wide_pending;
    }
    const uint32_t groups = std::min<uint32_t>((uint32_t)std::max(1, cus - (s.carry_tail ? 1 : 0) - leave_cus), (s.numTiles + WPB - 1) / WPB);
    s.groups = groups;
    s.ride_want = groups + (in.debug_hzb_ride_stall != 0 ? 1u : 0u);
    s.tilesXMagic = (uint32_t)((1ull << 32) / s.tilesX + 1ull);
    s.staticClaims = 0xFFFFFFFFu;
    if (in.balance != 0 && groups >= 16u && groups <= 8u * in.claim_words) {
        constexpr uint32_t cs = kChunkShift;
        const uint32_t round = groups << cs;
        const uint32_t want_pool = (uint32_t)((uint64_t)s.numTiles * (uint32_t)in.balance_pool_16ths / 16u);
        do {
            const uint32_t sh = (uint32_t)in.balance_chunk_shift;
            const uint32_t la = sh >= 4u ? 2u : (sh == 3u ? 3u : 4u);
            const uint32_t rounds = (s.numTiles - want_pool) / round;
            if ((rounds << cs) < 2u * WPB) break;
            const uint32_t static_tiles = rounds * round, chunks = (s.numTiles - static_tiles + (1u << sh) - 1u) >> sh;
            if (chunks < (la + 2u) * groups) break;
            if ((uint64_t)chunks * 8u / groups + la + 8u > kDynSlots) break;
            const unsigned long long magic = (((unsigned long long)chunks << 32) + groups - 1u) / groups;
            bool ok = true;
            for (uint32_t q8 = 0; q8 < groups && ok; q8 += 8u) {
                const uint32_t nq = std::min(8u, groups - q8);
                const uint32_t P0 = (uint32_t)((q8 * magic) >> 32), P1 = (uint32_t)(((q8 + nq) * magic) >> 32);
                ok = P1 >= P0 + la * nq && P1 <= chunks;
            }
            if (!ok) break;
            s.staticClaims = rounds << cs;
            s.poolChunks = chunks; s.staticTiles = static_tiles; s.dynShift = sh; s.lookahead = la;
            s.poolMagic = magic;
        } while (false);
    }
    const uint32_t sched[8] = {groups, s.numTiles, s.poolChunks != 0u ? s.staticTiles : s.numTiles, s.poolChunks, s.dynShift, s.lookahead, WPB, s.ride_pieces};
    std::copy(sched, sched + 8, s.reported);
    return s;
}

}
```

### unclerenderer_amd/csrc/lighting_plan.h

```cpp
#pragma once

#include <cstdint>

namespace ur {

constexpr uint32_t kChunkShift = 2;
constexpr uint32_t kDynSlots = 256;
constexpr uint32_t kLdsCubeBytes = 32768;

struct CubeLayout {
    uint32_t mips;
    uint64_t edge[16];
    uint64_t bordered[16];
    uint64_t pairs[17];
    uint64_t texels, bytes;
    uint32_t size(uint32_t m) const { return (uint32_t)(edge[m] - 2u); }
};
CubeLayout cube_layout(uint32_t base_size, uint32_t mip_count);
uint32_t cube_first_mip_within(const CubeLayout& L, uint64_t budget);

struct StreamPlanInput {
    int cus;
    int leave_cus, ride_walkers, balance, balance_pool_16ths, balance_chunk_shift, debug_hzb_ride_stall;
    uint32_t W, rows;
    uint32_t wpb;
    bool tail_pending;
    bool wide_pending;
    uint32_t wide_grid_x, wide_grid_y;
    uint32_t claim_words;
};

struct StreamPlan {
    uint32_t tilesX, numTiles, tilesXMagic;
    uint32_t groups;
    bool carry_tail;
    bool rides;
    uint32_t ride_pieces, ride_grid_x, ride_walkers, ride_want, ride_spin_limit;
    bool flush_first;
    uint32_t staticClaims;
    uint32_t poolChunks, staticTiles, dynShift, lookahead;
    unsigned long long poolMagic;
    uint32_t reported[8];
};
StreamPlan plan_stream(const StreamPlanInput& in);

uint32_t ride_walkers(uint32_t pieces, uint32_t tiles, uint32_t lighting_groups, uint32_t wpb, int forced);

}
```

### unclerenderer_amd/csrc/post.hip

```cpp

#include "ur_internal.h"
#include "ur_device.h"
#include "post_common.h"

namespace {

using ur_post::half4_t;
using ur_post::TonemapParams;
using ur_post::tonemap_pixel;
using ur_post::final_exposure;
using ur_post::unorm8;

typedef uint32_t u32x4_t __attribute__((ext_vector_type(4)));
typedef uint32_t u32x2_t __attribute__((ext_vector_type(2)));

constexpr float kLumR = 0.2126f, kLumG = 0.7152f, kLumB = 0.0722f;

struct AeParams {
    const half4_t* hdr;
    const float* prev;
    float* out;
    uint32_t W, H;
    float size_x, size_y;
    float delta_time, speed_up, speed_down;
// ... 359 lines not shown
    tm.exposure = tonemap->Exposure;
    tm.inv_gamma = 1.0f / (tonemap->Gamma > 1e-3f ? tonemap->Gamma : 1e-3f);
    return tm;
}

int launch_cas(ur_ctx* ctx, const char* who, const ur_cas_constants* cas, In mode, bool halo, const void* src, const void* above, const void* below,
               const TonemapParams* tm, uint32_t* out, uint32_t w, uint32_t h, uint32_t row0, uint32_t rows)
{
    if (w == 0 || h == 0 || rows == 0 || (uint64_t)row0 + rows > h) { ur::set_error("%s: empty or out-of-frame band", who); return UR_EINVAL; }
    if (halo && ((row0 > 0 && !above) || (row0 + rows < h && !below))) {
        ur::set_error("%s: hdr_above may be null only when row0 == 0, hdr_below only when row0 + rows == h", who);
        return UR_EINVAL;
    }
    const size_t src_bytes = (size_t)w * (halo ? rows : h) * (mode == In::Hdr ? 8u : 4u), out_bytes = (size_t)w * rows * 4u, halo_bytes = (size_t)w * 8u;
    if (overlaps(src, src_bytes, out, out_bytes) || (above && overlaps(above, halo_bytes, out, out_bytes)) || (below && overlaps(below, halo_bytes, out, out_bytes))) {
        ur::set_error("%s: the output band overlaps the input frame", who);
        return UR_EINVAL;
    }
    const float dx = 1.0f / (float)w, dy = 1.0f / (float)h;
    if (!(fabsf(cas->TexelDelta[0] - dx) <= 1e-6f * dx) || !(fabsf(cas->TexelDelta[1] - dy) <= 1e-6f * dy)) {
        ur::set_error("%s: TexelDelta must be (1/w, 1/h) (neighbour texels)", who);
        return UR_EUNSUPPORTED;
    }
    const uint32_t grid_y = (rows + (uint32_t)kRows - 1u) / (uint32_t)kRows;
    if (grid_y > 65535u) { ur::set_error("%s: band too tall", who); return UR_EUNSUPPORTED; }
    CasParams p{};
    p.src = src; p.out = out;
    p.W = w; p.H = h; p.row0 = row0; p.rows = rows;
    p.sharpness = cas->Sharpness;
    if (tm) p.tm = *tm;
    auto aligned = [](const void* q, uintptr_t m) { return (reinterpret_cast<uintptr_t>(q) & m) == 0u; };
    const bool pairs = (w % 2u) == 0u && aligned(src, mode == In::Hdr ? 15u : 7u) && aligned(out, 7u) && aligned(above, 15u) && aligned(below, 15u);
    const uint32_t px = pairs ? 2u : 1u;
    const dim3 grid((w + 256u * px - 1u) / (256u * px), grid_y);
    if (halo) {
        const CasHaloParams q{p, above, below};
        if (mode == In::Hdr) {
            if (pairs) hipLaunchKernelGGL((cas_halo_kernel<In::Hdr, 2>), grid, dim3(256), 0, ctx->stream, q);
            else hipLaunchKernelGGL((cas_halo_kernel<In::Hdr, 1>), grid, dim3(256), 0, ctx->stream, q);
        } else {
            if (pairs) hipLaunchKernelGGL((cas_halo_kernel<In::LdrHdrHalo, 2>), grid, dim3(256), 0, ctx->stream, q);
            else hipLaunchKernelGGL((cas_halo_kernel<In::LdrHdrHalo, 1>), grid, dim3(256), 0, ctx->stream, q);
        }
    } else if (mode == In::Hdr) {
        if (pairs) hipLaunchKernelGGL((cas_strip_kernel<true, 2>), grid, dim3(256), 0, ctx->stream, p);
        else hipLaunchKernelGGL((cas_strip_kernel<true, 1>), grid, dim3(256), 0, ctx->stream, p);
    } else {
        if (pairs) hipLaunchKernelGGL((cas_strip_kernel<false, 2>), grid, dim3(256), 0, ctx->stream, p);
        else hipLaunchKernelGGL((cas_strip_kernel<false, 1>), grid, dim3(256), 0, ctx->stream, p);
    }
    UR_HIP_TRY(hipGetLastError());
    return UR_OK;
}

AeParams ae_params(const ur_auto_exposure_constants* constants, uint32_t w, uint32_t h, const float* prev_ev, float* out_ev)
{
    AeParams p{};
    p.prev = prev_ev; p.out = out_ev;
    p.W = w; p.H = h;
    p.size_x = constants->InputSize[0]; p.size_y = constants->InputSize[1];
    p.delta_time = constants->DeltaTime; p.speed_up = constants->AdaptationSpeedUp; p.speed_down = constants->AdaptationSpeedDown;
    p.use_history = constants->UseHistory;
    p.key = constants->AutoExposureKey; p.ev_min = constants->AutoExposureMin; p.ev_max = constants->AutoExposureMax;
    return p;
}

}

extern "C" int ur_auto_exposure(ur_ctx* ctx, const ur_auto_exposure_constants* constants, const ur_half4* hdr_full, uint32_t w, uint32_t h,
                                const float* prev_ev, float* out_ev)
{
    if (!ctx || !constants || !hdr_full || !out_ev || (constants->UseHistory != 0u && !prev_ev)) {
        ur::set_error("ur_auto_exposure: null argument");
        return UR_EINVAL;
    }
    if (w == 0 || h == 0 || constants->InputSize[0] != (float)w || constants->InputSize[1] != (float)h) {
        ur::set_error("ur_auto_exposure: InputSize must be (w, h) of a non-empty frame");
        return UR_EINVAL;
    }
    AeParams p = ae_params(constants, w, h, prev_ev, out_ev);
    p.hdr = reinterpret_cast<const half4_t*>(hdr_full);
    hipLaunchKernelGGL(auto_exposure_kernel, dim3(1), dim3(256), 0, ctx->stream, p);
    UR_HIP_TRY(hipGetLastError());
    return UR_OK;
}

extern "C" int ur_cas(ur_ctx* ctx, const ur_cas_constants* constants, const uint32_t* ldr_full, uint32_t* out_band,
                      uint32_t w, uint32_t h, uint32_t row0, uint32_t rows)
{
    if (!ctx || !constants || !ldr_full || !out_band) { ur::set_error("ur_cas: null argument"); return UR_EINVAL; }
    return launch_cas(ctx, "ur_cas", constants, In::Ldr, false, ldr_full, nullptr, nullptr, nullptr, out_band, w, h, row0, rows);
}

extern "C" int ur_tonemap_cas(ur_ctx* ctx, const ur_tonemap_constants* tonemap, const ur_cas_constants* cas, const ur_half4* hdr_full,
                              const float* exposure_ev, uint32_t* out_band, uint32_t w, uint32_t h, uint32_t row0, uint32_t rows)
{
    if (!ctx || !tonemap || !cas || !hdr_full || !out_band) { ur::set_error("ur_tonemap_cas: null argument"); return UR_EINVAL; }
    const TonemapParams tm = tonemap_params(tonemap, exposure_ev);
    return launch_cas(ctx, "ur_tonemap_cas", cas, In::Hdr, false, hdr_full, nullptr, nullptr, &tm, out_band, w, h, row0, rows);
}


extern "C" uint64_t ur_post_record_bytes(uint32_t w) { return ((uint64_t)2u * w + kTapTexels) * 8u; }

extern "C" int ur_pack_post_record(ur_ctx* ctx, const ur_half4* hdr_band, uint32_t w, uint32_t h, uint32_t row0, uint32_t rows, void* record)
{
    if (!ctx || !hdr_band || !record) { ur::set_error("ur_pack_post_record: null argument"); return UR_EINVAL; }
    if (w == 0 || h == 0 || rows == 0 || (uint64_t)row0 + rows > h) { ur::set_error("ur_pack_post_record: empty or out-of-frame band"); return UR_EINVAL; }
    if (overlaps(hdr_band, (size_t)w * rows * 8u, record, ur_post_record_bytes(w))) { ur::set_error("ur_pack_post_record: the record overlaps the band"); return UR_EINVAL; }
    PackParams p{reinterpret_cast<const half4_t*>(hdr_band), static_cast<half4_t*>(record), w, h, row0, rows};
    const uint32_t n = 2u * w + kTapTexels;
    hipLaunchKernelGGL(post_record_kernel, dim3((n + 255u) / 256u), dim3(256), 0, ctx->stream, p);
    UR_HIP_TRY(hipGetLastError());
    return UR_OK;
}

extern "C" int ur_auto_exposure_records(ur_ctx* ctx, const ur_auto_exposure_constants* constants, const void* records, uint32_t n_ranks, uint32_t w,
                                        uint32_t h, const float* prev_ev, float* out_ev)
{
    if (!ctx || !constants || !records || !out_ev || (constants->UseHistory != 0u && !prev_ev)) {
        ur::set_error("ur_auto_exposure_records: null argument");
        return UR_EINVAL;
    }
    if (w == 0 || h == 0 || constants->InputSize[0] != (float)w || constants->InputSize[1] != (float)h) {
        ur::set_error("ur_auto_exposure_records: InputSize must be (w, h) of a non-empty frame");
        return UR_EINVAL;
    }
    if (n_ranks == 0 || h % n_ranks != 0) { ur::set_error("ur_auto_exposure_records: n_ranks must divide h (equal bands)"); return UR_EINVAL; }
    AeRecordsParams q{};
    q.ae = ae_params(constants, w, h, prev_ev, out_ev);
    q.records = static_cast<const half4_t*>(records);
    q.record_texels = 2u * w + kTapTexels;
    q.band_rows = h / n_ranks;
    hipLaunchKernelGGL(ae_records_kernel, dim3(1), dim3(256), 0, ctx->stream, q);
    UR_HIP_TRY(hipGetLastError());
    return UR_OK;
}

extern "C" int ur_tonemap_cas_halo(ur_ctx* ctx, const ur_tonemap_constants* tonemap, const ur_cas_constants* cas, const ur_half4* hdr_band,
                                   const ur_half4* hdr_above, const ur_half4* hdr_below, const float* exposure_ev, uint32_t* out_band,
                                   uint32_t w, uint32_t h, uint32_t row0, uint32_t rows)
{
    if (!ctx || !tonemap || !cas || !hdr_band || !out_band) { ur::set_error("ur_tonemap_cas_halo: null argument"); return UR_EINVAL; }
    const TonemapParams tm = tonemap_params(tonemap, exposure_ev);
    return launch_cas(ctx, "ur_tonemap_cas_halo", cas, In::Hdr, true, hdr_band, hdr_above, hdr_below, &tm, out_band, w, h, row0, rows);
}

extern "C" int ur_cas_halo(ur_ctx* ctx, const ur_tonemap_constants* tonemap, const ur_cas_constants* cas, const uint32_t* ldr_band,
                           const ur_half4* hdr_above, const ur_half4* hdr_below, const float* exposure_ev, uint32_t* out_band,
                           uint32_t w, uint32_t h, uint32_t row0, uint32_t rows)
{
    if (!ctx || !tonemap || !cas || !ldr_band || !out_band) { ur::set_error("ur_cas_halo: null argument"); return UR_EINVAL; }
    const TonemapParams tm = tonemap_params(tonemap, exposure_ev);
    return launch_cas(ctx, "ur_cas_halo", cas, In::LdrHdrHalo, true, ldr_band, hdr_above, hdr_below, &tm, out_band, w, h, row0, rows);
}
```

### unclerenderer_amd/csrc/raster.hip

```cpp

#include "raster_rule.h"
#include "ur_internal.h"

namespace {

using namespace ur_raster;

typedef float f32x4_t __attribute__((ext_vector_type(4)));

constexpr uint32_t kQueueHeaderDwords = 16u;
constexpr uint32_t kEntryDwords = 12u;
constexpr uint32_t kKeyedEntryDwords = 16u;
constexpr uint32_t kLargeStamps = 64u;
constexpr uint32_t kOwnPixels = 4u;
constexpr uint32_t kNoTile = 0xFFFFFFFFu;

struct RasterParams {
    const uint8_t* commands;
    uint32_t command_count;
    uint32_t mode;
    const uint32_t* visible_idx;
    const uint32_t* visible_count;
    uint32_t index_base;
    uint32_t range_count;
// ... 390 lines not shown
{
    const uint32_t lane = threadIdx.x & 63u;
    const uint32_t wave = __builtin_amdgcn_readfirstlane(blockIdx.x * kWaves + (threadIdx.x >> 6));
    const uint32_t wave_count = gridDim.x * kWaves;
    const uint32_t count = (uint32_t)min(*reinterpret_cast<const unsigned long long*>(queue), (unsigned long long)queue_cap);
    for (uint32_t e = wave; e < count; e += wave_count) {
        const u32x4_t* q = reinterpret_cast<const u32x4_t*>(queue + kQueueHeaderDwords + (size_t)e * P::kEntryDwords);
        const u32x4_t q0 = q[0], q1 = q[1], q2 = q[2];
        uint32_t key = 0u;
        if constexpr (P::kKeyed) key = q[3].x;
        if (q2.y == kNoTile) continue;
        Tri t;
        t.x0 = (int)q0.x; t.y0 = (int)q0.y; t.x1 = (int)q0.z; t.y1 = (int)q0.w; t.x2 = (int)q1.x; t.y2 = (int)q1.y;
        t.z0 = __uint_as_float(q1.z); t.k1 = __uint_as_float(q1.w); t.k2 = __uint_as_float(q2.x);
        const int tx = (int)(q2.y & 0xFFFFu) * 64, ty = (int)(q2.y >> 16) * 64;
        const int px0 = max((int)(q2.z & 0xFFFFu), tx), py0 = max((int)(q2.z >> 16), ty);
        const int px1 = min((int)(q2.w & 0xFFFFu), tx + 63), py1 = min((int)(q2.w >> 16), ty + 63);
        if (edge_max(t.x0, t.y0, t.x1, t.y1, px0, py0, px1, py1) < 0 || edge_max(t.x1, t.y1, t.x2, t.y2, px0, py0, px1, py1) < 0 ||
            edge_max(t.x2, t.y2, t.x0, t.y0, px0, py0, px1, py1) < 0)
            continue;
        stamp_rect<P>(t, map, w, px0, py0, px1, py1, lane, depth, row0, key);
    }
}

struct VisArgs {
    const float* depth;
    uint32_t row0, rows, key_bits;
};

template <class P>
int launch_raster(ur_ctx* ctx, const float* m0, const float* m1, const ur_raster_draws* draws, uint32_t* map, uint32_t n, uint32_t w, uint32_t h, float clear,
                  uint32_t* stats, const VisArgs* vis)
{
    const ur_draw_ranges* rg = draws->ranges;
    const bool list = draws->visible_idx != nullptr;
    const uint32_t head = min((uint32_t)((16u - (reinterpret_cast<uintptr_t>(map) & 15u)) & 15u) / 4u, n);
    uint32_t* queue = ctx->raster_queue_cap != 0u ? ctx->raster_queue : nullptr;
    const uint32_t clear_blocks = min((n / 4u + kThreads - 1u) / kThreads + 1u, (uint32_t)ctx->cu_count * 16u);
    hipLaunchKernelGGL(shadow_clear_kernel, dim3(clear_blocks), dim3(kThreads), 0, ctx->stream, reinterpret_cast<float*>(map), n, head, queue, clear);
    UR_HIP_TRY(hipGetLastError());
    if (draws->command_count == 0u) return UR_OK;

    RasterParams p{};
    p.commands = static_cast<const uint8_t*>(ur::raster_commands(*draws));
    p.command_count = draws->command_count;
    p.mode = list ? 1u : (rg ? 2u : 0u);
    p.visible_idx = draws->visible_idx; p.visible_count = draws->visible_count; p.index_base = draws->index_base;
    if (rg) { p.range_count = rg->range_count; p.offsets = rg->offsets; p.counts = rg->counts; }
    for (int k = 0; k < 16; ++k) { p.L[k] = m0[k]; p.Pr[k] = m1 ? m1[k] : 0.0f; }
    p.map = map;
    p.w = w; p.h = h;
    p.half_w = 0.5f * (float)w; p.half_h = 0.5f * (float)h;
    p.stats = stats;
    p.queue = queue; p.queue_cap = queue ? ctx->raster_queue_cap : 0u;
    if (vis) { p.depth = vis->depth; p.row0 = vis->row0; p.rows = vis->rows; p.key_bits = vis->key_bits; }
    const uint32_t want_waves = (uint32_t)ctx->cu_count * 16u;
    p.segments = max(1u, min(1024u, want_waves / p.command_count));
    const uint64_t items = (uint64_t)p.command_count * p.segments;
    p.items = (uint32_t)items;
    if (items > 0xFFFFFFFFull) { p.segments = 1u; p.items = p.command_count; }
    const uint32_t blocks = min((p.items + kWaves - 1u) / kWaves, (uint32_t)ctx->cu_count * 32u);
    hipLaunchKernelGGL(raster_kernel<P>, dim3(blocks), dim3(kThreads), 0, ctx->stream, p);
    UR_HIP_TRY(hipGetLastError());
    if (queue) {
        hipLaunchKernelGGL(large_kernel<P>, dim3((uint32_t)ctx->cu_count * 8u), dim3(kThreads), 0, ctx->stream, queue, p.queue_cap, p.map, w, p.depth, p.row0);
        UR_HIP_TRY(hipGetLastError());
// ... 13 lines not shown
    if (rg && (!rg->offsets || !rg->commands || !rg->counts || rg->range_count == 0u)) { set_error("%s: a null member of ranges / no range", who); return UR_EINVAL; }
    const void* commands = raster_commands(draws);
    if (!commands && draws.command_count != 0u) { set_error("%s: null commands", who); return UR_EINVAL; }
    if (!aligned(commands, 16) || !aligned(target, 4) || !aligned(stats, 4) || !aligned(draws.visible_idx, 4) || !aligned(draws.visible_count, 4) ||
        (rg && (!aligned(rg->offsets, 4) || !aligned(rg->counts, 4)))) {
        set_error("%s: a misaligned buffer (commands 16 bytes, the others 4)", who);
        return UR_EINVAL;
    }
    return UR_OK;
}

int ur::check_raster_call(const char* who, const ur_ctx* ctx, const float* m0, const float* m1, const ur_raster_draws* draws, const void* target, const char* target_name,
                          uint32_t w, uint32_t h, const void* stats)
{
    if (!ctx || !m0 || !m1 || !draws) { set_error("%s: null context, matrix or draws", who); return UR_EINVAL; }
    if (w == 0u || h == 0u || w > UR_RASTER_MAX_TARGET || h > UR_RASTER_MAX_TARGET) { set_error("%s: a %u x %u target (1..%u)", who, w, h, UR_RASTER_MAX_TARGET); return UR_EINVAL; }
    return check_raster_draws(who, *draws, target, target_name, stats);
}

int ur::launch_visibility_raster(ur_ctx* ctx, const float* view, const float* projection, const ur_raster_draws* draws, const float* depth, uint32_t* keys, uint32_t w,
                                 uint32_t h, uint32_t row0, uint32_t rows, uint32_t key_bits, bool d24, uint32_t* stats)
{
    const VisArgs vis{depth, row0, rows, key_bits};
    if (d24) return launch_raster<VisPolicy<true>>(ctx, view, projection, draws, keys, w * rows, w, h, 0.0f, stats, &vis);
    return launch_raster<VisPolicy<false>>(ctx, view, projection, draws, keys, w * rows, w, h, 0.0f, stats, &vis);
}

extern "C" {

int ur_raster_reserve(ur_ctx* ctx, uint32_t max_large_work_items)
{
    if (!ctx) { ur::set_error("ur_raster_reserve: null context"); return UR_EINVAL; }
    if (max_large_work_items == ctx->raster_queue_cap) return UR_OK;
    UR_HIP_TRY(hipStreamSynchronize(ctx->stream));
    if (ctx->raster_queue) (void)hipFree(ctx->raster_queue);
    ctx->raster_queue = nullptr;
    ctx->raster_queue_cap = 0;
    if (max_large_work_items == 0u) return UR_OK;
    const size_t bytes = ((size_t)kQueueHeaderDwords + (size_t)max_large_work_items * kKeyedEntryDwords) * sizeof(uint32_t);
    if (hipMalloc(&ctx->raster_queue, bytes) != hipSuccess) {
        ctx->raster_queue = nullptr;
        ur::set_error("ur_raster_reserve: allocation of %u large work items failed", max_large_work_items);
        return UR_ENOMEM;
    }
    ctx->raster_queue_cap = max_large_work_items;
    return UR_OK;
}

int ur_shadow_map(ur_ctx* ctx, const float* lvp, const ur_raster_draws* draws, float* shadow_map, uint32_t w, uint32_t h, uint32_t* stats4)
{
    const int rc = ur::check_raster_call("ur_shadow_map", ctx, lvp, lvp, draws, shadow_map, "shadow_map", w, h, stats4);
    if (rc != UR_OK) return rc;
    if (!(lvp[3] == 0.0f && lvp[7] == 0.0f && lvp[11] == 0.0f && lvp[15] == 1.0f)) {
        ur::set_error("ur_shadow_map: the light's fourth column is (%g, %g, %g, %g), not (0, 0, 0, 1): only orthographic lights are rasterised", lvp[3], lvp[7], lvp[11], lvp[15]);
        return UR_EUNSUPPORTED;
    }
    return launch_raster<ShadowPolicy>(ctx, lvp, nullptr, draws, reinterpret_cast<uint32_t*>(shadow_map), w * h, w, h, 1.0f, stats4, nullptr);
}

int ur_depth_prepass(ur_ctx* ctx, const float* view, const float* projection, const ur_raster_draws* draws, float* depth, uint32_t w, uint32_t h, uint32_t flags,
                     uint32_t* stats6)
{
    int rc = ur::check_raster_call("ur_depth_prepass", ctx, view, projection, draws, depth, "depth", w, h, stats6);
    if (rc == UR_OK) rc = ur::check_depth_flags("ur_depth_prepass", flags);
    if (rc != UR_OK) return rc;
    if (flags & UR_DEPTH_QUANTIZE_D24) return launch_raster<DepthPolicy<true>>(ctx, view, projection, draws, reinterpret_cast<uint32_t*>(depth), w * h, w, h, 0.0f, stats6, nullptr);
// ... 5 lines not shown
```

### unclerenderer_amd/csrc/stream_ceiling.hip

```cpp

#include <hip/hip_ext.h>

#include "ur_internal.h"

namespace {

struct StreamPtrs { const float4* in[4]; float4* out; uint32_t n; };

__global__ __launch_bounds__(256) void stream4_kernel(StreamPtrs p)
{
    const uint32_t i = blockIdx.x * 256u + threadIdx.x;
    const uint32_t j = min(i, p.n - 1u);
    typedef float sf32x4_t __attribute__((ext_vector_type(4)));
    const sf32x4_t a = __builtin_nontemporal_load(reinterpret_cast<const sf32x4_t*>(p.in[0]) + j), b = __builtin_nontemporal_load(reinterpret_cast<const sf32x4_t*>(p.in[1]) + j),
                   c = __builtin_nontemporal_load(reinterpret_cast<const sf32x4_t*>(p.in[2]) + j), d = __builtin_nontemporal_load(reinterpret_cast<const sf32x4_t*>(p.in[3]) + j);
    if (i < p.n) __builtin_nontemporal_store(sf32x4_t{(a.x + b.x) + (c.x + d.x), (a.y + b.y) + (c.y + d.y), (a.z + b.z) + (c.z + d.z), (a.w + b.w) + (c.w + d.w)}, reinterpret_cast<sf32x4_t*>(p.out) + i);
}

}

extern "C" int ur_debug_stream_ceiling(ur_ctx* ctx, const void* in0, const void* in1, const void* in2, const void* in3, void* out, uint64_t elements16,
                                       void* start_event, void* stop_event)
{
    if (!ctx || !in0 || !in1 || !in2 || !in3 || !out || elements16 == 0 || elements16 > 0xFFFFFF00ull || (start_event != nullptr && stop_event == nullptr)) {
        ur::set_error("ur_debug_stream_ceiling: bad argument");
        return UR_EINVAL;
    }
    StreamPtrs p{{static_cast<const float4*>(in0), static_cast<const float4*>(in1), static_cast<const float4*>(in2), static_cast<const float4*>(in3)},
                 static_cast<float4*>(out), (uint32_t)elements16};
    const dim3 grid((uint32_t)((elements16 + 255u) / 256u));
    if (stop_event != nullptr)
        hipExtLaunchKernelGGL(stream4_kernel, grid, dim3(256), 0, ctx->stream, static_cast<hipEvent_t>(start_event), static_cast<hipEvent_t>(stop_event), 0, p);
    else
        hipLaunchKernelGGL(stream4_kernel, grid, dim3(256), 0, ctx->stream, p);
    UR_HIP_TRY(hipGetLastError());
    return UR_OK;
}
```

### unclerenderer_amd/csrc/taa.hip

```cpp

#include "ur_internal.h"
#include "ur_device.h"
#include "post_common.h"

namespace {

typedef _Float16 half4_t __attribute__((ext_vector_type(4)));

struct TaaParams {
    const half4_t* current;
    const half4_t* history;
    half4_t* output;
    uint32_t W, H, row0, rows;
    float weight;
    uint32_t use_history;
};

constexpr int kStripRows = 8;
typedef _Float16 half2_t __attribute__((ext_vector_type(2)));
typedef uint32_t u32x2_t __attribute__((ext_vector_type(2)));

struct RowMinMax { half2_t mn0, mn1, mx0, mx1; };

__device__ __forceinline__ half2_t as_h2(uint32_t u) { union { uint32_t u; half2_t h; } c; c.u = u; return c.h; }
// ... 172 lines not shown
    if (j >= 4u * W) return;
    const uint32_t part = j / W, x = j - part * W;
    const uint32_t second = min(1u, p.rows - 1u), second_last = p.rows >= 2u ? p.rows - 2u : 0u;
    u32x2_t v = {0u, 0u};
    if (part < 2u) v = p.band[(size_t)(part == 0u ? second : second_last) * W + x];
    else if (p.history != nullptr) v = p.history[(size_t)(part == 2u ? 0u : p.rows - 1u) * W + x];
    p.record[j] = v;
}

}

static int fill_params(const char* who, TaaParams& p, ur_ctx* ctx, const ur_half4* current_frame, const ur_half4* history_band, ur_half4* output_band,
                       float history_weight, uint32_t use_history, uint32_t w, uint32_t h, uint32_t row0, uint32_t rows)
{
    if (!ctx || !current_frame || !output_band || (use_history && !history_band)) { ur::set_error("%s: null argument", who); return UR_EINVAL; }
    if (w == 0 || h == 0 || (uint64_t)row0 + rows > h) { ur::set_error("%s: bad frame/band", who); return UR_EINVAL; }
    p.current = reinterpret_cast<const half4_t*>(current_frame);
    p.history = reinterpret_cast<const half4_t*>(history_band);
    p.output = reinterpret_cast<half4_t*>(output_band);
    p.W = w; p.H = h; p.row0 = row0; p.rows = rows;
    p.weight = history_weight < 0.0f ? 0.0f : (history_weight > 1.0f ? 1.0f : history_weight);
    if (!(history_weight == history_weight)) p.weight = 0.0f;
    p.use_history = use_history ? 1u : 0u;
    return UR_OK;
}

extern "C" int ur_temporal_aa(ur_ctx* ctx, const ur_half4* current_frame, const ur_half4* history_band, ur_half4* output_band, float history_weight,
                              uint32_t use_history, uint32_t w, uint32_t h, uint32_t row0, uint32_t rows)
{
    TaaParams p{};
    const int rc = fill_params("ur_temporal_aa", p, ctx, current_frame, history_band, output_band, history_weight, use_history, w, h, row0, rows);
    if (rc != UR_OK) return rc;
    if (rows == 0) return UR_OK;
    hipLaunchKernelGGL(taa_strip_kernel<NoPost>, dim3((w + 255u) / 256u, (rows + kStripRows - 1u) / kStripRows), dim3(256), 0, ctx->stream, p, NoPost{});
    UR_HIP_TRY(hipGetLastError());
    return UR_OK;
}

extern "C" int ur_temporal_aa_tonemap(ur_ctx* ctx, const ur_tonemap_constants* tonemap, const ur_half4* current_frame, const ur_half4* history_band,
                                      ur_half4* history_out_band, const float* exposure_ev, uint32_t* ldr_out_band, float history_weight,
                                      uint32_t use_history, uint32_t w, uint32_t h, uint32_t row0, uint32_t rows)
{
    if (!tonemap || !ldr_out_band) { ur::set_error("ur_temporal_aa_tonemap: null argument"); return UR_EINVAL; }
    TaaParams p{};
    const int rc = fill_params("ur_temporal_aa_tonemap", p, ctx, current_frame, history_band, history_out_band, history_weight, use_history, w, h, row0, rows);
    if (rc != UR_OK) return rc;
    if (rows == 0) return UR_OK;
    ur_post::TonemapParams tm{};
    tm.exposure_ev = exposure_ev;
    tm.out = ldr_out_band;
    tm.enable_tonemap = tonemap->EnableTonemap;
    tm.enable_auto_exposure = tonemap->EnableAutoExposure;
    tm.exposure = tonemap->Exposure;
    tm.inv_gamma = 1.0f / (tonemap->Gamma > 1e-3f ? tonemap->Gamma : 1e-3f);
    const dim3 grid((w + 255u) / 256u, (rows + kStripRows - 1u) / kStripRows);
    if (ctx->opt.taa_tonemap_history_store == 0) hipLaunchKernelGGL(taa_strip_kernel<TonemapPost<true>>, grid, dim3(256), 0, ctx->stream, p, TonemapPost<true>{tm});
    else hipLaunchKernelGGL(taa_strip_kernel<TonemapPost<false>>, grid, dim3(256), 0, ctx->stream, p, TonemapPost<false>{tm});
    UR_HIP_TRY(hipGetLastError());
    return UR_OK;
}


static bool overlaps(const void* a, size_t a_bytes, const void* b, size_t b_bytes)
{
    const uintptr_t x = reinterpret_cast<uintptr_t>(a), y = reinterpret_cast<uintptr_t>(b);
    return x < y + b_bytes && y < x + a_bytes;
}

extern "C" uint64_t ur_taa_record_bytes(uint32_t w) { return (uint64_t)4u * w * 8u; }

extern "C" int ur_pack_taa_record(ur_ctx* ctx, const ur_half4* hdr_band, const ur_half4* history_read_band, uint32_t use_history, uint32_t w, uint32_t h,
                                  uint32_t row0, uint32_t rows, void* record)
{
    if (!ctx || !hdr_band || !record || (use_history && !history_read_band)) { ur::set_error("ur_pack_taa_record: null argument"); return UR_EINVAL; }
    if (w == 0 || h == 0 || rows == 0 || (uint64_t)row0 + rows > h) { ur::set_error("ur_pack_taa_record: empty or out-of-frame band"); return UR_EINVAL; }
    if (rows < 2u && rows != h) { ur::set_error("ur_pack_taa_record: a band that is not the whole frame needs at least 2 rows"); return UR_EUNSUPPORTED; }
    const size_t band_bytes = (size_t)w * rows * 8u;
    if (overlaps(hdr_band, band_bytes, record, ur_taa_record_bytes(w)) || (use_history && overlaps(history_read_band, band_bytes, record, ur_taa_record_bytes(w)))) {
        ur::set_error("ur_pack_taa_record: the record overlaps a band");
        return UR_EINVAL;
    }
    const TaaRecordParams p{reinterpret_cast<const u32x2_t*>(hdr_band), use_history ? reinterpret_cast<const u32x2_t*>(history_read_band) : nullptr,
                            static_cast<u32x2_t*>(record), w, rows};
    hipLaunchKernelGGL(taa_record_kernel, dim3((uint32_t)(((uint64_t)4u * w + 255u) / 256u)), dim3(256), 0, ctx->stream, p);
    UR_HIP_TRY(hipGetLastError());
    return UR_OK;
}

static int fill_band_params(const char* who, TaaBandParams& q, uint32_t& grid_y, ur_ctx* ctx, const ur_half4* current_band, const ur_half4* cur_above,
                            const ur_half4* cur_below, const ur_half4* history_band, ur_half4* output_band, const ur_half4* above2, const ur_half4* hist_above,
                            const ur_half4* below2, const ur_half4* hist_below, ur_half4* resolved_above, ur_half4* resolved_below, float history_weight,
                            uint32_t use_history, uint32_t w, uint32_t h, uint32_t row0, uint32_t rows)
{
    TaaParams p{};
    const int rc = fill_params(who, p, ctx, current_band, history_band, output_band, history_weight, use_history, w, h, row0, rows);
    if (rc != UR_OK) return rc;
    if (rows == 0) { ur::set_error("%s: empty band", who); return UR_EINVAL; }
    const bool top = row0 == 0, bottom = row0 + rows == h;
    if ((!top && !cur_above) || (!bottom && !cur_below)) {
        ur::set_error("%s: cur_above may be null only when row0 == 0, cur_below only when row0 + rows == h", who);
        return UR_EINVAL;
    }
    if ((top && (cur_above || above2 || hist_above || resolved_above)) || (bottom && (cur_below || below2 || hist_below || resolved_below))) {
        ur::set_error("%s: there is no row beyond the frame's edge: the pointers of that side must be null", who);
        return UR_EINVAL;
    }
    if ((resolved_above != nullptr) != (above2 != nullptr) || (resolved_below != nullptr) != (below2 != nullptr) ||
        (hist_above && !resolved_above) || (hist_below && !resolved_below) ||
        (use_history && ((resolved_above && !hist_above) || (resolved_below && !hist_below)))) {
        ur::set_error("%s: resolved_above goes with above2 (and hist_above when use_history), resolved_below with below2 (and hist_below)", who);
        return UR_EINVAL;
    }
    const size_t band_bytes = (size_t)w * rows * 8u, row_bytes = (size_t)w * 8u;
    const void* ins[] = {cur_above, cur_below, above2, below2, hist_above, hist_below};
    void* outs[] = {resolved_above, resolved_below};
    for (void* o : outs) {
// ... 2 lines not shown
                   (use_history && overlaps(o, row_bytes, history_band, band_bytes));
        for (const void* i : ins) bad = bad || (i && overlaps(o, row_bytes, i, row_bytes));
        if (bad) { ur::set_error("%s: a resolved row overlaps another buffer", who); return UR_EINVAL; }
    }
    if (resolved_above && resolved_below && overlaps(resolved_above, row_bytes, resolved_below, row_bytes)) { ur::set_error("%s: the resolved rows overlap", who); return UR_EINVAL; }
    bool bad = overlaps(current_band, band_bytes, output_band, band_bytes);
    for (const void* i : ins) bad = bad || (i && overlaps(i, row_bytes, output_band, band_bytes));
    if (bad) { ur::set_error("%s: the output band overlaps a current or neighbour row", who); return UR_EINVAL; }
    const uint32_t strips = (rows + (uint32_t)kStripRows - 1u) / (uint32_t)kStripRows;
    grid_y = strips + (resolved_above ? 1u : 0u) + (resolved_below ? 1u : 0u);
    if (grid_y > 65535u) { ur::set_error("%s: band too tall", who); return UR_EUNSUPPORTED; }
    auto in = [](const ur_half4* x) { return reinterpret_cast<const u32x2_t*>(x); };
    BandRows& R = q.R;
    R.band = in(current_band); R.above = in(cur_above); R.below = in(cur_below); R.above2 = in(above2); R.below2 = in(below2);
    R.history = in(history_band); R.hist_above = in(hist_above); R.hist_below = in(hist_below);
    R.output = reinterpret_cast<u32x2_t*>(output_band); R.res_above = reinterpret_cast<u32x2_t*>(resolved_above); R.res_below = reinterpret_cast<u32x2_t*>(resolved_below);
    R.W = w; R.row0 = row0; R.rows = rows;
    R.ylo = top ? 0u : (above2 ? (row0 >= 2u ? row0 - 2u : 0u) : row0 - 1u);
    R.yhi = bottom ? h - 1u : (below2 ? min(row0 + rows + 1u, h - 1u) : row0 + rows);
    q.H = h; q.weight = p.weight; q.use_history = p.use_history; q.strips = strips;
    return UR_OK;
}

extern "C" int ur_temporal_aa_halo(ur_ctx* ctx, const ur_half4* current_band, const ur_half4* cur_above, const ur_half4* cur_below, const ur_half4* history_band,
                                   ur_half4* output_band, const ur_half4* above2, const ur_half4* hist_above, const ur_half4* below2, const ur_half4* hist_below,
                                   ur_half4* resolved_above, ur_half4* resolved_below, float history_weight, uint32_t use_history, uint32_t w, uint32_t h,
                                   uint32_t row0, uint32_t rows)
{
    TaaBandParams q{};
    uint32_t grid_y = 0;
    const int rc = fill_band_params("ur_temporal_aa_halo", q, grid_y, ctx, current_band, cur_above, cur_below, history_band, output_band, above2, hist_above, below2,
                                    hist_below, resolved_above, resolved_below, history_weight, use_history, w, h, row0, rows);
    if (rc != UR_OK) return rc;
    hipLaunchKernelGGL(taa_band_kernel<NoPost>, dim3((w + 255u) / 256u, grid_y), dim3(256), 0, ctx->stream, q, NoPost{});
    UR_HIP_TRY(hipGetLastError());
    return UR_OK;
}

extern "C" int ur_temporal_aa_tonemap_halo(ur_ctx* ctx, const ur_tonemap_constants* tonemap, const ur_half4* current_band, const ur_half4* cur_above,
                                           const ur_half4* cur_below, const ur_half4* history_band, ur_half4* history_out_band, const float* exposure_ev,
                                           uint32_t* ldr_out_band, const ur_half4* above2, const ur_half4* hist_above, const ur_half4* below2,
                                           const ur_half4* hist_below, ur_half4* resolved_above, ur_half4* resolved_below, float history_weight,
                                           uint32_t use_history, uint32_t w, uint32_t h, uint32_t row0, uint32_t rows)
{
    if (!tonemap || !ldr_out_band) { ur::set_error("ur_temporal_aa_tonemap_halo: null argument"); return UR_EINVAL; }
    TaaBandParams q{};
    uint32_t grid_y = 0;
    const int rc = fill_band_params("ur_temporal_aa_tonemap_halo", q, grid_y, ctx, current_band, cur_above, cur_below, history_band, history_out_band, above2,
                                    hist_above, below2, hist_below, resolved_above, resolved_below, history_weight, use_history, w, h, row0, rows);
    if (rc != UR_OK) return rc;
    ur_post::TonemapParams tm{};
    tm.exposure_ev = exposure_ev;
    tm.out = ldr_out_band;
    tm.enable_tonemap = tonemap->EnableTonemap;
    tm.enable_auto_exposure = tonemap->EnableAutoExposure;
    tm.exposure = tonemap->Exposure;
    tm.inv_gamma = 1.0f / (tonemap->Gamma > 1e-3f ? tonemap->Gamma : 1e-3f);
    hipLaunchKernelGGL(taa_band_kernel<TonemapPost<true>>, dim3((w + 255u) / 256u, grid_y), dim3(256), 0, ctx->stream, q, TonemapPost<true>{tm});
    UR_HIP_TRY(hipGetLastError());
    return UR_OK;
}
```

### unclerenderer_amd/csrc/tonemap.hip

```cpp

#include "ur_internal.h"
#include "ur_device.h"
#include "post_common.h"

namespace {

using ur_post::half4_t;
using ur_post::TonemapParams;
using ur_post::tonemap_pixel;
using ur_post::final_exposure;

__global__ __launch_bounds__(256) void tonemap_kernel(TonemapParams p)
{
    const float finalExposure = final_exposure(p);
    for (uint32_t i = blockIdx.x * 256u + threadIdx.x; i < p.count; i += gridDim.x * 256u) p.out[i] = tonemap_pixel(p, finalExposure, p.hdr[i]);
}

typedef uint32_t u32x4_t __attribute__((ext_vector_type(4)));
typedef uint32_t u32x2_t __attribute__((ext_vector_type(2)));
template <uint32_t kPairTrips>
__global__ __launch_bounds__(256) void tonemap_pairs_kernel(TonemapParams p)
{
    const float finalExposure = final_exposure(p);
    const uint32_t wave = threadIdx.x >> 6, lane = threadIdx.x & 63u;
// ... 1 lines not shown
    const u32x4_t* src = reinterpret_cast<const u32x4_t*>(p.hdr);
    u32x4_t v[kPairTrips];
#pragma unroll
    for (uint32_t k = 0; k < kPairTrips; ++k) v[k] = __builtin_nontemporal_load(src + min(pair0 + k * 64u, npairs - 1u));
#pragma unroll
    for (uint32_t k = 0; k < kPairTrips; ++k) {
        const uint32_t pr = pair0 + k * 64u;
        if (pr < npairs) {
            union { u32x2_t u; half4_t h; } a, b;
            a.u = u32x2_t{v[k].x, v[k].y}; b.u = u32x2_t{v[k].z, v[k].w};
            ur::store_once_b64(reinterpret_cast<u32x2_t*>(p.out) + pr, ur::once_u32x2_t{tonemap_pixel(p, finalExposure, a.h), tonemap_pixel(p, finalExposure, b.h)});
        }
    }
}

}

extern "C" int ur_tonemap(ur_ctx* ctx, const ur_tonemap_constants* constants, const ur_half4* hdr, const float* exposure_ev, uint32_t* out_rgba8,
                          uint32_t w, uint32_t rows)
{
    if (!ctx || !constants || !hdr || !out_rgba8) { ur::set_error("ur_tonemap: null argument"); return UR_EINVAL; }
    const uint64_t n = (uint64_t)w * rows;
    if (n == 0) return UR_OK;
    if (n > 0xFFFFFFFFull) { ur::set_error("ur_tonemap: band too large"); return UR_EUNSUPPORTED; }
    TonemapParams p{};
    p.hdr = reinterpret_cast<const half4_t*>(hdr);
    p.exposure_ev = exposure_ev;
    p.out = out_rgba8;
    p.count = (uint32_t)n;
    p.enable_tonemap = constants->EnableTonemap;
    p.enable_auto_exposure = constants->EnableAutoExposure;
    p.exposure = constants->Exposure;
    p.inv_gamma = 1.0f / (constants->Gamma > 1e-3f ? constants->Gamma : 1e-3f);
    const bool aligned = ((reinterpret_cast<uintptr_t>(hdr) & 15u) == 0u) && ((reinterpret_cast<uintptr_t>(out_rgba8) & 7u) == 0u);
    if (aligned && n >= 2u) {
        if (n < (24u << 20)) hipLaunchKernelGGL(tonemap_pairs_kernel<1>, dim3((uint32_t)((n / 2u * 2u + 511u) / 512u)), dim3(256), 0, ctx->stream, p);
        else hipLaunchKernelGGL(tonemap_pairs_kernel<2>, dim3((uint32_t)((n / 2u * 2u + 1023u) / 1024u)), dim3(256), 0, ctx->stream, p);
        UR_HIP_TRY(hipGetLastError());
        if ((n & 1u) == 0u) return UR_OK;
        p.hdr += n - 1u; p.out += n - 1u; p.count = 1u;
    }
    uint32_t blocks = (uint32_t)((p.count + 255u) / 256u);
    const uint32_t cap = (uint32_t)ctx->cu_count * 8u * 2u;
    if (blocks > cap) blocks = cap;
    hipLaunchKernelGGL(tonemap_kernel, dim3(blocks), dim3(256), 0, ctx->stream, p);
    UR_HIP_TRY(hipGetLastError());
    return UR_OK;
}
```

### unclerenderer_amd/csrc/ur_api.hip

```cpp

#include <dlfcn.h>

#include <algorithm>
#include <cmath>
#include <cstdarg>
#include <cstring>
#include <vector>

#include "ur_internal.h"
#include "lighting_plan.h"

#include "../../include/ur_host.h"

namespace ur {

static thread_local char g_error[512] = "";

void set_error(const char* fmt, ...)
{
    va_list ap;
    va_start(ap, fmt);
    vsnprintf(g_error, sizeof(g_error), fmt, ap);
    va_end(ap);
}

}

using ur::set_error;

namespace ur {

int check_hzb_timeout(ur_ctx* ctx, const char* who)
{
    if (ctx && ctx->claim_timed_out && *ctx->claim_timed_out != 0u) {
        *ctx->claim_timed_out = 0u;
        (void)hipMemsetAsync(ctx->claim_words, 0, (kClaimWords + 1u) * kClaimWordStride * sizeof(uint32_t), ctx->stream);
        set_error("%s: a wave of a balanced Lighting launch gave up waiting for a tile claim of its workgroup: tiles of that launch were not shaded — "
                  "shade the frame again (reported once; the context is usable)", who);
        return UR_ETIMEOUT;
    }
    if (!ctx || !ctx->hzb_timed_out || *ctx->hzb_timed_out == 0u) return UR_OK;
    *ctx->hzb_timed_out = 0u;
    (void)hipMemsetAsync(ctx->hzb_done, 0, 64, ctx->stream);
    set_error("%s: the tail of a Build HZB chain that rode a Lighting launch gave up waiting for its producers: the HZB's small levels are stale — "
              "build it again (reported once; the context is usable)", who);
    return UR_ETIMEOUT;
}

}

namespace {

struct FaceAxes { int major, su, sv; double ms, us, vs; };
const FaceAxes kFaces[6] = {
    {0, 2, 1, +1, -1, -1},
    {0, 2, 1, -1, +1, -1},
    {1, 0, 2, +1, +1, +1},
    {1, 0, 2, -1, +1, -1},
    {2, 0, 1, +1, +1, -1},
    {2, 0, 1, -1, -1, -1},
};

void resolve_border(int N, int face, int i, int j, int& oface, int& oi, int& oj)
{
    const bool iOut = i < 0 || i >= N, jOut = j < 0 || j >= N;
    if (!iOut && !jOut) { oface = face; oi = i; oj = j; return; }
    if (iOut && jOut) j = j < 0 ? 0 : N - 1;
    const double s = 2.0 * (i + 0.5) / N - 1.0, t = 2.0 * (j + 0.5) / N - 1.0;
    const FaceAxes& F = kFaces[face];
    double p[3];
    p[F.major] = F.ms; p[F.su] = F.us * s; p[F.sv] = F.vs * t;
    const double over = (iOut ? std::fabs(s) : std::fabs(t)) - 1.0;
    p[F.major] *= (1.0 - over);
    const int oa = iOut ? F.su : F.sv;
    p[oa] = p[oa] > 0 ? 1.0 : -1.0;
    const int nf = oa * 2 + (p[oa] > 0 ? 0 : 1);
    const FaceAxes& G = kFaces[nf];
    const double ns = p[G.su] / G.us, nt = p[G.sv] / G.vs;
// ... 49 lines not shown
    }
    if (hipSetDevice(device) != hipSuccess) {
        set_error("ur_create: hipSetDevice(%d) failed", device);
        return nullptr;
    }
    ur_ctx* ctx = new ur_ctx();
    ctx->device = device;
    ctx->stream = static_cast<hipStream_t>(stream);
    hipDeviceProp_t prop;
    if (hipGetDeviceProperties(&prop, device) == hipSuccess) ctx->cu_count = prop.multiProcessorCount > 0 ? prop.multiProcessorCount : 256;
    float table[256];
    ur_host_srgb_decode_table(table);
    if (hipMalloc(&ctx->srgb_table, sizeof(table)) != hipSuccess ||
        hipMemcpy(ctx->srgb_table, table, sizeof(table), hipMemcpyHostToDevice) != hipSuccess) {
        set_error("ur_create: sRGB table upload failed");
        ur_destroy(ctx);
        return nullptr;
    }
    float encode[255];
    ur_host_srgb_encode_table(encode);
    if (hipMalloc(&ctx->srgb_encode_table, sizeof(encode)) != hipSuccess ||
        hipMemcpy(ctx->srgb_encode_table, encode, sizeof(encode), hipMemcpyHostToDevice) != hipSuccess) {
        set_error("ur_create: sRGB encode table upload failed");
        ur_destroy(ctx);
        return nullptr;
    }
    float lod[127];
    ur_host_lod_table(lod);
    if (hipMalloc(&ctx->lod_table, sizeof(lod)) != hipSuccess || hipMemcpy(ctx->lod_table, lod, sizeof(lod), hipMemcpyHostToDevice) != hipSuccess) {
        set_error("ur_create: level-of-detail table upload failed");
        ur_destroy(ctx);
        return nullptr;
    }
    if (hipMalloc(&ctx->hzb_done, 64) != hipSuccess || hipMemset(ctx->hzb_done, 0, 64) != hipSuccess) {
        set_error("ur_create: HZB arrival counter allocation failed");
        ur_destroy(ctx);
        return nullptr;
    }
    {
        void* host = nullptr;
        void* devp = nullptr;
        if (hipHostMalloc(&host, 64, hipHostMallocMapped | hipHostMallocCoherent) != hipSuccess || hipHostGetDevicePointer(&devp, host, 0) != hipSuccess) {
            if (host) (void)hipHostFree(host);
            set_error("ur_create: host-visible time-out flag allocation failed");
            ur_destroy(ctx);
            return nullptr;
        }
        ctx->hzb_timed_out = static_cast<volatile uint32_t*>(host);
        ctx->hzb_timed_out_dev = static_cast<uint32_t*>(devp);
        *ctx->hzb_timed_out = 0u;
        ctx->claim_timed_out = ctx->hzb_timed_out + 1;
        ctx->claim_timed_out_dev = ctx->hzb_timed_out_dev + 1;
        *ctx->claim_timed_out = 0u;
    }
    {
        const size_t bytes = (ur::kClaimWords + 1u) * ur::kClaimWordStride * sizeof(uint32_t);
        if (hipMalloc(&ctx->claim_words, bytes) != hipSuccess || hipMemset(ctx->claim_words, 0, bytes) != hipSuccess) {
            set_error("ur_create: tile-claim words allocation failed");
            ur_destroy(ctx);
            return nullptr;
        }
    }
    if (ur_reserve(ctx, 1u << 20) != UR_OK) {
        ur_destroy(ctx);
        return nullptr;
    }
    return ctx;
}

void ur_destroy(ur_ctx* ctx)
{
    if (!ctx) return;
    ctx->hzb_tail_pending = false;
    ctx->hzb_wide_pending = false;
    if (ctx->hzb_done) (void)hipFree(ctx->hzb_done);
    if (ctx->claim_words) (void)hipFree(ctx->claim_words);
    if (ctx->hzb_timed_out) (void)hipHostFree(const_cast<uint32_t*>(ctx->hzb_timed_out));
    if (ctx->srgb_table) (void)hipFree(ctx->srgb_table);
    if (ctx->srgb_encode_table) (void)hipFree(ctx->srgb_encode_table);
    if (ctx->lod_table) (void)hipFree(ctx->lod_table);
    if (ctx->block_counts) (void)hipFree(ctx->block_counts);
    if (ctx->wave_masks) (void)hipFree(ctx->wave_masks);
    if (ctx->raster_queue) (void)hipFree(ctx->raster_queue);
    delete ctx;
}

int ur_defer_hzb_tail(ur_ctx* ctx, int enable)
{
    if (!ctx) { set_error("ur_defer_hzb_tail: null context"); return UR_EINVAL; }
    if (enable < 0 || enable > 2) { set_error("ur_defer_hzb_tail: mode %d (0 off, 1 tail, 2 whole chain)", enable); return UR_EINVAL; }
    const bool narrower = (enable == 0) || (enable == 1 && ctx->defer_hzb_wide);
    ctx->defer_hzb_tail = enable != 0;
    ctx->defer_hzb_wide = enable == 2;
    return narrower ? ur::flush_hzb_tail(ctx) : UR_OK;
}

int ur_debug_timeline(ur_ctx* ctx, unsigned long long* device_pairs, uint32_t capacity_pairs)
{
    if (!ctx || (device_pairs != nullptr && capacity_pairs == 0)) { set_error("ur_debug_timeline: bad argument"); return UR_EINVAL; }
    ctx->timeline = device_pairs;
    ctx->timeline_cap = device_pairs ? capacity_pairs : 0u;
    ctx->timeline_pos = 0;
    return UR_OK;
}

int ur_time_next_lighting(ur_ctx* ctx, void* start_event, void* stop_event)
{
    if (!ctx || (start_event != nullptr && stop_event == nullptr)) { set_error("ur_time_next_lighting: a start event needs a stop event"); return UR_EINVAL; }
    ctx->time_start = static_cast<hipEvent_t>(start_event);
    ctx->time_stop = static_cast<hipEvent_t>(stop_event);
    return UR_OK;
}

int ur_time_next_cull(ur_ctx* ctx, void* stop_event)
{
    if (!ctx) { set_error("ur_time_next_cull: null context"); return UR_EINVAL; }
    ctx->time_cull_stop = static_cast<hipEvent_t>(stop_event);
    ctx->time_cull_carried = false;
    return UR_OK;
}

int ur_time_cull_carried(const ur_ctx* ctx) { return ctx && ctx->time_cull_carried ? 1 : 0; }

namespace {
struct OptionSlot { int ur_ctx::Options::*field; int lo, hi; bool pair; };
bool option_slot(int option, OptionSlot& o)
{
    typedef ur_ctx::Options O;
    switch (option) {
    case UR_OPT_LIGHTING_STREAM: o = {&O::lighting_stream, 0, 1, false}; return true;
    case UR_OPT_LIGHTING_WAVES_PER_WG: o = {&O::lighting_wpb, 12, 16, true}; return true;
    case UR_OPT_LIGHTING_TILED_WAVES: o = {&O::tiled_waves, 4, 6, true}; return true;
    case UR_OPT_LIGHTING_LEAVE_CUS: o = {&O::leave_cus, 0, 128, false}; return true;
    case UR_OPT_RIDE_WALKERS: o = {&O::ride_walkers, 0, 16, false}; return true;
    case UR_OPT_CULL_STORE: o = {&O::cull_store, 0, 4, false}; return true;
    case UR_OPT_LIGHTING_BALANCE: o = {&O::balance, 0, 1, false}; return true;
    case UR_OPT_BALANCE_POOL_16THS: o = {&O::balance_pool_16ths, 1, 8, false}; return true;
    case UR_OPT_BALANCE_CHUNK_SHIFT: o = {&O::balance_chunk_shift, 2, 6, false}; return true;
    case UR_OPT_DEBUG_HZB_RIDE_STALL: o = {&O::debug_hzb_ride_stall, 0, 1, false}; return true;
    case UR_OPT_TAA_TONEMAP_HISTORY_STORE: o = {&O::taa_tonemap_history_store, 0, 1, false}; return true;
    default: return false;
    }
}
}

int ur_set_option(ur_ctx* ctx, int option, int value)
{
    OptionSlot o;
    if (!ctx || !option_slot(option, o)) { set_error("ur_set_option: unknown option %d", option); return UR_EINVAL; }
    if (value < o.lo || value > o.hi || (o.pair && value != o.lo && value != o.hi)) {
        set_error("ur_set_option: option %d takes %d%s%d, not %d", option, o.lo, o.pair ? " or " : " .. ", o.hi, value);
        return UR_EINVAL;
    }
    ctx->opt.*(o.field) = value;
    if (option == UR_OPT_CULL_STORE) ctx->cull_record_args = nullptr;
    return UR_OK;
}

int ur_get_option(const ur_ctx* ctx, int option, int* value)
{
    OptionSlot o;
    if (!ctx || !value || !option_slot(option, o)) { set_error("ur_get_option: unknown option %d", option); return UR_EINVAL; }
    *value = ctx->opt.*(o.field);
    return UR_OK;
}

int ur_flush(ur_ctx* ctx)
{
    if (!ctx) { set_error("ur_flush: null context"); return UR_EINVAL; }
    const int trc = ur::check_hzb_timeout(ctx, "ur_flush");
    if (trc != UR_OK) return trc;
    return ur::flush_hzb_tail(ctx);
}

int ur_debug_lighting_schedule(const ur_ctx* ctx, uint32_t out8[8])
{
    if (!ctx || !out8) { set_error("ur_debug_lighting_schedule: null argument"); return UR_EINVAL; }
    std::memcpy(out8, ctx->last_schedule, sizeof(ctx->last_schedule));
    return UR_OK;
}

int ur_debug_set_hzb_timeout(ur_ctx* ctx)
{
    if (!ctx || !ctx->hzb_timed_out) { set_error("ur_debug_set_hzb_timeout: null context"); return UR_EINVAL; }
    *ctx->hzb_timed_out = 1u;
    return UR_OK;
}

int ur_reserve(ur_ctx* ctx, uint32_t max_instances)
{
    if (!ctx) return UR_EINVAL;
    if (max_instances <= ctx->ws_instances) return UR_OK;
    UR_HIP_TRY(hipStreamSynchronize(ctx->stream));
    if (ctx->block_counts) (void)hipFree(ctx->block_counts);
    if (ctx->wave_masks) (void)hipFree(ctx->wave_masks);
    ctx->block_counts = nullptr; ctx->wave_masks = nullptr; ctx->ws_instances = 0;
    ctx->cull_record_args = nullptr;
    const size_t blocks = ((size_t)max_instances + 255u) / 256u;
    const size_t slices = 1u + UR_MAX_CULL_VIEWS;
    if (hipMalloc(&ctx->block_counts, slices * blocks * sizeof(uint32_t)) != hipSuccess ||
        hipMalloc(&ctx->wave_masks, slices * blocks * 4u * sizeof(uint64_t)) != hipSuccess) {
        set_error("ur_reserve: workspace allocation for %u instances failed", max_instances);
        return UR_ENOMEM;
    }
    ctx->ws_instances = (uint32_t)(blocks * 256u);
    return UR_OK;
}

uint32_t ur_hzb_layout(uint32_t src_w, uint32_t src_h, ur_mip_desc* mips, uint32_t* mip_count)
{
    if (!mips || !mip_count || src_w == 0 || src_h == 0) return 0;
    uint32_t w = (src_w + 1) / 2, h = (src_h + 1) / 2;
    w = w ? w : 1; h = h ? h : 1;
    uint32_t n = 0, off = 0;
    for (;;) {
        if (n >= UR_MAX_HZB_MIPS) return 0;
        mips[n].offset = off; mips[n].width = w; mips[n].height = h;
        ++n;
        off += (w * h + 63u) & ~63u;
        if (!(w > 1 || h > 1)) break;
        w = w / 2 ? w / 2 : 1; h = h / 2 ? h / 2 : 1;
    }
    *mip_count = n;
    return off;
}
// ... 281 lines not shown
    const int rc = check_band("ur_debug_print_draw", ctx, w, h, row0, rows);
    if (rc != UR_OK) return rc;
    if (!constants || !glyphs || !atlas_r8 || !buffer || !ldr_inout) { set_error("ur_debug_print_draw: null argument"); return UR_EINVAL; }
    if (glyph_count == 0 || atlas_w == 0 || atlas_h == 0 || atlas_w > 16384u || atlas_h > 16384u) {
        set_error("ur_debug_print_draw: glyph table of %u entries, atlas %u x %u (1..16384)", glyph_count, atlas_w, atlas_h);
        return UR_EINVAL;
    }
    if (constants->ScreenSize[0] != (float)w || constants->ScreenSize[1] != (float)h) {
        set_error("ur_debug_print_draw: ScreenSize (%g, %g) is not the frame's (%u, %u)", constants->ScreenSize[0], constants->ScreenSize[1], w, h);
        return UR_EINVAL;
    }
    return ur::launch_debug_print_draw(ctx, constants, glyphs, glyph_count, atlas_r8, atlas_w, atlas_h, buffer, ldr_inout, w, row0, rows);
}

static void* rccl_symbol(const char* name)
{
    void* fn = dlsym(RTLD_DEFAULT, name);
    if (!fn) {
        static void* lib = nullptr;
        if (!lib) lib = dlopen("librccl.so", RTLD_NOW | RTLD_GLOBAL);
        if (!lib) lib = dlopen("librccl.so.1", RTLD_NOW | RTLD_GLOBAL);
        if (lib) fn = dlsym(lib, name);
    }
    return fn;
}

int ur_allgather_rows_bytes_ex(ur_ctx* ctx, void* comm, void* image, uint32_t row_bytes, uint32_t h, uint32_t n_ranks, uint32_t rank, int mode)
{
    if (!ctx || !comm || !image || row_bytes == 0 || h == 0 || n_ranks == 0 || rank >= n_ranks || h % n_ranks != 0) {
        set_error("ur_allgather_rows: bad argument (row_bytes=%u h=%u ranks=%u rank=%u)", row_bytes, h, n_ranks, rank);
        return UR_EINVAL;
    }
    if (mode != UR_GATHER_RING && mode != UR_GATHER_DIRECT) { set_error("ur_allgather_rows: mode %d (0 ring, 1 direct)", mode); return UR_EINVAL; }
    const size_t band_bytes = (size_t)row_bytes * (h / n_ranks);
    char* base = reinterpret_cast<char*>(image);
    const char* send = base + band_bytes * rank;
    if (mode == UR_GATHER_RING) {
        static nccl_allgather_fn fn = nullptr;
        if (!fn) fn = reinterpret_cast<nccl_allgather_fn>(rccl_symbol("ncclAllGather"));
        if (!fn) { set_error("ur_allgather_rows: ncclAllGather not found"); return UR_EUNSUPPORTED; }
        const int rc = fn(send, image, band_bytes,  0, comm, ctx->stream);
        if (rc != 0) { set_error("ncclAllGather failed (%d)", rc); return UR_EHIP; }
        return UR_OK;
    }
    typedef int (*group_fn)(void);
    typedef int (*send_fn)(const void*, size_t, int, int, void*, hipStream_t);
    typedef int (*recv_fn)(void*, size_t, int, int, void*, hipStream_t);
    static group_fn g_start = nullptr, g_end = nullptr;
    static send_fn f_send = nullptr;
    static recv_fn f_recv = nullptr;
    if (!g_start) {
        g_start = reinterpret_cast<group_fn>(rccl_symbol("ncclGroupStart"));
        g_end = reinterpret_cast<group_fn>(rccl_symbol("ncclGroupEnd"));
        f_send = reinterpret_cast<send_fn>(rccl_symbol("ncclSend"));
        f_recv = reinterpret_cast<recv_fn>(rccl_symbol("ncclRecv"));
    }
    if (!g_start || !g_end || !f_send || !f_recv) { g_start = nullptr; set_error("ur_allgather_rows: ncclGroupStart/End, ncclSend, ncclRecv not found"); return UR_EUNSUPPORTED; }
    int rc = g_start();
    for (uint32_t k = 1; k < n_ranks && rc == 0; ++k) {
        const uint32_t to = (rank + k) % n_ranks, from = (rank + n_ranks - k) % n_ranks;
        rc = f_send(send, band_bytes,  0, (int)to, comm, ctx->stream);
        if (rc == 0) rc = f_recv(base + band_bytes * from, band_bytes,  0, (int)from, comm, ctx->stream);
    }
    const int rc_end = g_end();
    if (rc != 0 || rc_end != 0) { set_error("grouped ncclSend/ncclRecv failed (%d, %d)", rc, rc_end); return UR_EHIP; }
    return UR_OK;
// ... 17 lines not shown
```

### unclerenderer_amd/csrc/ur_internal.h

```cpp
#pragma once

#include <hip/hip_runtime.h>

#include <cstdint>
#include <cstdio>

#include "../../include/ur_hotpath.h"
#include "../../include/ur_raster.h"

namespace ur {
constexpr uint32_t kTailMaxLevels = 12, kTailTexels = 16384;
constexpr uint32_t kClaimWords = 32, kClaimWordStride = 32;
struct HzbTail {
    const float* src;
    uint32_t SW, SH, first_mip, levels;
    float* dst[kTailMaxLevels];
    uint32_t W[kTailMaxLevels], H[kTailMaxLevels];
    uint32_t magic[kTailMaxLevels];
};
}
#include "hzb_wide.h"

struct ur_ctx {
    int device = 0;
    hipStream_t stream = nullptr;
    uint32_t* block_counts = nullptr;
    uint64_t* wave_masks = nullptr;
    uint32_t ws_instances = 0;
    const void* cull_record_args = nullptr;
    uint32_t cull_record_n = 0;
    float* srgb_table = nullptr;
    float* srgb_encode_table = nullptr;
    float* lod_table = nullptr;
    int cu_count = 256;
    bool defer_hzb_tail = false;
    bool hzb_tail_pending = false;
    ur::HzbTail pending_tail{};
    bool defer_hzb_wide = false;
    bool hzb_wide_pending = false;
    ur::HzbDispatch pending_wide{};
    uint32_t pending_wide_grid_x = 0, pending_wide_grid_y = 0;
    unsigned long long* timeline = nullptr;
    uint32_t timeline_cap = 0, timeline_pos = 0;
    uint32_t* hzb_done = nullptr;
    volatile uint32_t* hzb_timed_out = nullptr;
    uint32_t* hzb_timed_out_dev = nullptr;
    hipEvent_t time_start = nullptr, time_stop = nullptr;
    hipEvent_t time_cull_stop = nullptr;
    bool time_cull_carried = false;
    struct Options {
        int lighting_stream = 1, lighting_wpb = 16, tiled_waves = 6, leave_cus = 0, ride_walkers = 0, cull_store = 3;
        int balance = 1, balance_pool_16ths = 3, balance_chunk_shift = 4;
        int debug_hzb_ride_stall = 0;
        int taa_tonemap_history_store = 0;
    } opt;
    uint32_t* claim_words = nullptr;
    uint32_t last_schedule[8] = {};
    volatile uint32_t* claim_timed_out = nullptr;
    uint32_t* claim_timed_out_dev = nullptr;
    uint32_t* raster_queue = nullptr;
    uint32_t raster_queue_cap = 0;
};

namespace ur {

void set_error(const char* fmt, ...);

#define UR_HIP_TRY(expr)                                                                          \
    do {                                                                                          \
        hipError_t _e = (expr);                                                                   \
        if (_e != hipSuccess) {                                                                   \
            ::ur::set_error("%s failed: %s (%s:%d)", #expr, hipGetErrorString(_e), __FILE__, __LINE__); \
            return UR_EHIP;                                                                       \
        }                                                                                         \
    } while (0)

int launch_build_hzb(ur_ctx* ctx, const float* depth, uint32_t src_w, uint32_t src_h, float* hzb_base,
                     const ur_mip_desc* mips, uint32_t mip_count);
int launch_build_hzb_band(ur_ctx* ctx, const float* depth, uint32_t src_w, uint32_t src_h, float* hzb_base, const ur_mip_desc* mips, uint32_t mip_count,
                          uint32_t piece_row0, uint32_t piece_rows);
int launch_build_hzb_tail(ur_ctx* ctx, float* hzb_base, const ur_mip_desc* mips, uint32_t mip_count);
int launch_cull(ur_ctx* ctx, const uint32_t* constants, const ur_float4* bounds, const float* hzb_base,
                const ur_mip_desc* mips, void* indirect_args, uint32_t* stats2, uint32_t* visible_idx,
                uint32_t* visible_count, uint32_t index_base, const ur_draw_ranges* draws, const ur_cull_view* views,
// ... 5 lines not shown
int check_cull_views(const ur_cull_view* views, uint32_t view_count);
inline const void* raster_commands(const ur_raster_draws& draws) { return draws.ranges ? draws.ranges->commands : draws.commands; }
int check_raster_draws(const char* who, const ur_raster_draws& draws, const void* target, const char* target_name, const void* stats);
int check_raster_call(const char* who, const ur_ctx* ctx, const float* m0, const float* m1, const ur_raster_draws* draws, const void* target, const char* target_name,
                      uint32_t w, uint32_t h, const void* stats);
inline int check_depth_flags(const char* who, uint32_t flags)
{
    if (flags & ~UR_DEPTH_QUANTIZE_D24) { set_error("%s: unknown flag bits 0x%x", who, flags & ~UR_DEPTH_QUANTIZE_D24); return UR_EINVAL; }
    return UR_OK;
}
int check_gbuffer_targets(const char* who, const ur_gbuffer_targets* targets);
inline int check_key_triangle_bits(const char* who, uint32_t bits)
{
    if (bits > 31u) { set_error("%s: key_triangle_bits %u (0 = automatic, 1..31)", who, bits); return UR_EINVAL; }
    return UR_OK;
}
int launch_visibility_raster(ur_ctx* ctx, const float* view, const float* projection, const ur_raster_draws* draws, const float* depth, uint32_t* keys, uint32_t w,
                             uint32_t h, uint32_t row0, uint32_t rows, uint32_t key_bits, bool d24, uint32_t* stats);
int launch_lighting(ur_ctx* ctx, const ur_scene_constants* scene, const ur_sky_constants* sky, const ur_half4* gbuf_a,
                    const ur_half4* gbuf_b, const uint32_t* gbuf_c, const float* depth, const ur_lighting_tables* tables,
                    ur_half4* hdr, uint32_t w, uint32_t h, uint32_t row0, uint32_t rows, int mode);
enum { UR_MODE_LIGHTING = 0, UR_MODE_SKY = 1, UR_MODE_FUSED = 2 };
int launch_debug_print_reset(ur_ctx* ctx, void* buffer, uint32_t* stats);
int launch_debug_print_stats(ur_ctx* ctx, const uint32_t* stats, void* buffer);
int launch_debug_print_text(ur_ctx* ctx, void* buffer, uint32_t x, uint32_t y, uint32_t color, const char* text, uint32_t length);
int launch_debug_print_draw(ur_ctx* ctx, const ur_debug_print_constants* constants, const ur_debug_glyph* glyphs, uint32_t glyph_count,
                            const uint8_t* atlas_r8, uint32_t atlas_w, uint32_t atlas_h, const void* buffer, uint32_t* ldr_inout, uint32_t w,
                            uint32_t row0, uint32_t rows);
inline unsigned long long* next_timeline_pair(ur_ctx* ctx)
{
    if (!ctx->timeline || ctx->timeline_pos >= ctx->timeline_cap) return nullptr;
    return ctx->timeline + 2u * (size_t)ctx->timeline_pos++;
}
int flush_hzb_tail(ur_ctx* ctx);
int check_hzb_timeout(ur_ctx* ctx, const char* who);

}
```

### unclerenderer_amd/lib.py

```python
from __future__ import annotations

import ctypes as C
import os
from pathlib import Path

import numpy as np

_LIB_PATH = Path(__file__).resolve().parent / "csrc" / "_build" / "libur_hotpath.so"
if os.environ.get("UR_HOTPATH_LIB"):
    _LIB_PATH = Path(os.environ["UR_HOTPATH_LIB"]).resolve()

UR_OK = 0
UR_EINVAL, UR_EHIP, UR_ENOMEM, UR_ENODEVICE, UR_EUNSUPPORTED, UR_ETIMEOUT = -1, -2, -3, -4, -5, -6
UR_MAX_HZB_MIPS = 16
UR_CULL_CONSTANT_DWORDS = 46
UR_INDIRECT_COMMAND_STRIDE = 64
UR_INDIRECT_INSTANCE_COUNT_OFFSET = 44


UR_OPT_LIGHTING_STREAM, UR_OPT_LIGHTING_WAVES_PER_WG, UR_OPT_LIGHTING_TILED_WAVES, UR_OPT_LIGHTING_LEAVE_CUS, UR_OPT_RIDE_WALKERS = 1, 2, 3, 4, 5
UR_OPT_CULL_STORE, UR_OPT_LIGHTING_BALANCE, UR_OPT_BALANCE_POOL_16THS, UR_OPT_BALANCE_CHUNK_SHIFT, UR_OPT_DEBUG_HZB_RIDE_STALL = 7, 8, 9, 10, 11
UR_OPT_TAA_TONEMAP_HISTORY_STORE = 12


class MipDesc(C.Structure):
    _fields_ = [("offset", C.c_uint32), ("width", C.c_uint32), ("height", C.c_uint32)]


class DrawRanges(C.Structure):
    _fields_ = [("offsets", C.c_void_p), ("range_count", C.c_uint32), ("commands", C.c_void_p), ("counts", C.c_void_p)]


UR_MAX_CULL_VIEWS = 4


class CullView(C.Structure):
    _fields_ = [("planes", C.c_float * 24), ("mask", C.c_void_p), ("visible_idx", C.c_void_p), ("visible_count", C.c_void_p),
                ("draws", C.POINTER(DrawRanges))]


class RasterDraws(C.Structure):
    _fields_ = [("commands", C.c_void_p), ("command_count", C.c_uint32), ("visible_idx", C.c_void_p), ("visible_count", C.c_void_p),
                ("index_base", C.c_uint32), ("ranges", C.POINTER(DrawRanges))]


class FrameShadowPass(C.Structure):
    _fields_ = [("draws", RasterDraws), ("shadow_map", C.c_void_p), ("stats4", C.c_void_p)]


class FrameDepthPass(C.Structure):
    _fields_ = [("draws", RasterDraws), ("depth", C.c_void_p), ("stats6", C.c_void_p), ("flags", C.c_uint32)]


class GBufferTargets(C.Structure):
    _fields_ = [("gbuf_a", C.c_void_p), ("gbuf_b", C.c_void_p), ("gbuf_c", C.c_void_p), ("hdr", C.c_void_p), ("object_id", C.c_void_p),
# ... 337 lines not shown
```

Measured before the change: 109,100.

## Let single-block cull ride inside the lighting launch ahead of the HZB chain

```diff
diff --git a/include/ur_hotpath.h b/include/ur_hotpath.h
--- a/include/ur_hotpath.h
+++ b/include/ur_hotpath.h
@@ -120,6 +120,7 @@
 #define UR_OPT_BALANCE_CHUNK_SHIFT 10
 #define UR_OPT_DEBUG_HZB_RIDE_STALL 11
 #define UR_OPT_TAA_TONEMAP_HISTORY_STORE 12
+#define UR_OPT_CULL_RIDE 13
 int ur_set_option(ur_ctx* ctx, int option, int value);
 int ur_get_option(const ur_ctx* ctx, int option, int* value);
 const char* ur_last_error(void);
diff --git a/unclerenderer_amd/csrc/cull.hip b/unclerenderer_amd/csrc/cull.hip
--- a/unclerenderer_amd/csrc/cull.hip
+++ b/unclerenderer_amd/csrc/cull.hip
@@ -1,15 +1,43 @@
 
 #include "cull_kernels.h"
+#include "lighting_plan.h"
 
 namespace ur {
+
+int launch_pending_cull(ur_ctx* ctx)
+{
+    if (!ctx->cull_pending) return UR_OK;
+    ctx->cull_pending = false;
+    CullArgs<false, false> Q{};
+    static_cast<CullParams&>(Q) = ctx->pending_cull;
+    Q.timeline = next_timeline_pair(ctx);
+    return launch_stop(ctx, nullptr, cull_kernel<true, false, false>, dim3(1), Q);
+}
+
+int flush_held(ur_ctx* ctx, bool flush_chain, bool keep_cull)
+{
+    if (!ctx) return UR_OK;
+    const FlushOrder order = flush_order(ctx->cull_pending, ctx->hzb_wide_pending || ctx->hzb_tail_pending, flush_chain, keep_cull);
+    for (const Held h : {order.first, order.second}) {
+        const int rc = h == Held::cull ? launch_pending_cull(ctx) : (h == Held::chain ? launch_pending_chain(ctx) : UR_OK);
+        if (rc != UR_OK) return rc;
+    }
+    return UR_OK;
+}
 
 int launch_cull(ur_ctx* ctx, const uint32_t* constants, const ur_float4* bounds, const float* hzb, const ur_mip_desc* mips,
                 void* indirect_args, uint32_t* stats2, uint32_t* visible_idx, uint32_t* visible_count, uint32_t index_base,
                 const ur_draw_ranges* draws, const ur_cull_view* views, uint32_t view_count)
 {
-    const int rc = flush_hzb_tail(ctx);
+    const int rc = flush_held(ctx, true, false);
     if (rc != UR_OK) return rc;
     if (views != nullptr && view_count != 0) return launch_cull_views(ctx, constants, bounds, hzb, mips, indirect_args, stats2, visible_idx, visible_count, index_base, draws, views, view_count);
+    if (cull_holds({ctx->cull_ride_on, ctx->opt.cull_ride, constants[40], draws != nullptr, 0u, ctx->time_cull_stop != nullptr})) {
+        ctx->pending_cull = CullParams{};
+        fill_cull_params(ctx->pending_cull, ctx, constants, bounds, hzb, mips, indirect_args, stats2, visible_idx, visible_count, index_base);
+        ctx->cull_pending = true;
+        return UR_OK;
+    }
     return cull_launches<false>(ctx, constants, bounds, hzb, mips, indirect_args, stats2, visible_idx, visible_count, index_base, draws, nullptr, 0);
 }
 
diff --git a/unclerenderer_amd/csrc/cull_kernels.h b/unclerenderer_amd/csrc/cull_kernels.h
--- a/unclerenderer_amd/csrc/cull_kernels.h
+++ b/unclerenderer_amd/csrc/cull_kernels.h
@@ -10,25 +10,7 @@
 
 namespace {
 
-struct CullParams {
-    float4 FrustumPlanes[6];
-    float ViewProjection[16];
-    uint32_t ModelCount, HZBEnabled, HZBMipCount, HZBWidth, HZBHeight, DebugPrintEnabled;
-    const float4* bounds;
-    const float* hzb;
-    uint8_t* args;
-    uint32_t* stats;
-    uint32_t* visible_idx;
-    uint32_t* visible_count;
-    uint32_t* block_counts;
-    uint64_t* wave_masks;
-    uint32_t index_base;
-    uint32_t store_flavour;
-    uint32_t record_valid;
-    uint32_t mip_offset[UR_MAX_HZB_MIPS];
-    uint32_t mip_width[UR_MAX_HZB_MIPS];
-    unsigned long long* timeline;
-};
+using ur::CullParams;
 
 struct DrawParams {
     const uint32_t* offsets;
@@ -54,13 +36,19 @@
 template <> struct CullArgs<false, false> : CullParams {};
 
 __device__ __forceinline__ float saturate_f(float x) { return fminf(fmaxf(x, 0.0f), 1.0f); }
-__device__ __forceinline__ float dot3(float ax, float ay, float az, float bx, float by, float bz) { return (ax * bx + ay * by) + az * bz; }
-
-__device__ __forceinline__ bool IsAabbVisible(const CullParams& C, float3 mn, float3 mx)
-{
+__device__ __forceinline__ float dot3(float ax, float ay, float az, float bx, float by, float bz)
+{
+#pragma clang fp contract(off)
+    return (ax * bx + ay * by) + az * bz;
+}
+
+template <class CP>
+__device__ __forceinline__ bool IsAabbVisible(const CP& C, float3 mn, float3 mx)
+{
+#pragma clang fp contract(off)
 #pragma unroll
     for (int i = 0; i < 6; ++i) {
-        const float4 plane = C.FrustumPlanes[i];
+        const float4 plane = make_float4(C.FrustumPlanes[i].x, C.FrustumPlanes[i].y, C.FrustumPlanes[i].z, C.FrustumPlanes[i].w);
         const float px = plane.x >= 0.0f ? mx.x : mn.x;
         const float py = plane.y >= 0.0f ? mx.y : mn.y;
         const float pz = plane.z >= 0.0f ? mx.z : mn.z;
@@ -83,8 +71,10 @@
     return true;
 }
 
-__device__ __forceinline__ bool IsOccluded(const CullParams& C, float3 mn, float3 mx)
-{
+template <class CP>
+__device__ __forceinline__ bool IsOccluded(const CP& C, float3 mn, float3 mx)
+{
+#pragma clang fp contract(off)
     if (C.HZBEnabled == 0 || C.HZBWidth == 0 || C.HZBHeight == 0 || C.HZBMipCount == 0) return false;
     const float* M = C.ViewProjection;
     float minUx = 1.0f, minUy = 1.0f, maxUx = 0.0f, maxUy = 0.0f, maxDepth = 0.0f;
@@ -246,18 +236,35 @@
     }
 }
 
-template <bool SINGLE_BLOCK, bool RANGES, bool VIEWS = false>
-__global__ __launch_bounds__(256) void cull_kernel(CullArgs<RANGES, VIEWS> C)
-{
-    __shared__ float4 sb[512];
-    __shared__ uint64_t smask[4];
-    __shared__ uint32_t scand[4];
-    __shared__ uint8_t slist[256], socc[256];
-
+constexpr uint32_t kCullLdsBytes = 512 * 16 + 4 * 8 + 4 * 4 + 256 + 256;
+
+template <bool SINGLE_BLOCK, bool RANGES, bool VIEWS, bool RIDING, class Args>
+__device__ __forceinline__ void cull_block(const Args& C, [[maybe_unused]] unsigned char* ride_lds, [[maybe_unused]] uint32_t* gate)
+{
+    static_assert(!RIDING || (SINGLE_BLOCK && !RANGES && !VIEWS), "only the plain single-block form rides");
+    float4* sb;
+    uint64_t* smask;
+    uint32_t* scand;
+    uint8_t *slist, *socc;
+    if constexpr (RIDING) {
+        sb = reinterpret_cast<float4*>(ride_lds);
+        smask = reinterpret_cast<uint64_t*>(ride_lds + 8192);
+        scand = reinterpret_cast<uint32_t*>(ride_lds + 8224);
+        slist = ride_lds + 8240;
+        socc = ride_lds + 8496;
+    } else {
+        __shared__ float4 sb_[512];
+        __shared__ uint64_t smask_[4];
+        __shared__ uint32_t scand_[4];
+        __shared__ uint8_t slist_[256], socc_[256];
+        static_assert(sizeof(sb_) + sizeof(smask_) + sizeof(scand_) + sizeof(slist_) + sizeof(socc_) == kCullLdsBytes, "what a riding cull reserves");
+        sb = sb_; smask = smask_; scand = scand_; slist = slist_; socc = socc_;
+    }
     const uint32_t tid = threadIdx.x, lane = tid & 63u, wave = tid >> 6;
-    const uint32_t first = blockIdx.x * 256u;
+    const uint32_t block = RIDING ? 0u : blockIdx.x;
+    const uint32_t first = block * 256u;
     const uint32_t index = first + tid;
-    ur::timeline_entry(C.timeline);
+    if constexpr (!RIDING) ur::timeline_entry(C.timeline);
 
     const uint32_t nb = min(512u, (C.ModelCount - first) * 2u);
     const float4* src = C.bounds + (size_t)first * 2u;
@@ -271,7 +278,7 @@
     uint32_t old_word = 0xFFFFFFFFu;
     const bool from_record = !SINGLE_BLOCK && C.store_flavour == 4u && C.record_valid != 0u;
     uint64_t old_mask = 0;
-    if (from_record) old_mask = C.wave_masks[(size_t)blockIdx.x * 4u + wave];
+    if (from_record) old_mask = C.wave_masks[(size_t)block * 4u + wave];
     else if (C.store_flavour >= 3u)
         old_word = *reinterpret_cast<const uint32_t*>(C.args + (size_t)min(index, C.ModelCount - 1u) * UR_INDIRECT_COMMAND_STRIDE + UR_INDIRECT_INSTANCE_COUNT_OFFSET);
     if (tid < nb) sb[tid] = s0;
@@ -303,6 +310,10 @@
         }
         __syncthreads();
         occluded = cand && socc[tid] != 0u;
+    }
+    if constexpr (RIDING) {
+        asm volatile("s_waitcnt vmcnt(0)" ::: "memory");
+        if (lane == 0) __hip_atomic_fetch_add(gate, 1u, __ATOMIC_RELAXED, __HIP_MEMORY_SCOPE_AGENT);
     }
     if (active) {
         visible = frustumVisible && !occluded;
@@ -330,9 +341,9 @@
     if (!RANGES && !VIEWS && C.visible_idx == nullptr) {
         if (!SINGLE_BLOCK && C.store_flavour == 4u) {
             const uint64_t m = __ballot(visible);
-            if (lane == 0) C.wave_masks[(size_t)blockIdx.x * 4u + wave] = m;
-        }
-        ur::timeline_exit(C.timeline, tid == 0);
+            if (lane == 0) C.wave_masks[(size_t)block * 4u + wave] = m;
+        }
+        if constexpr (!RIDING) ur::timeline_exit(C.timeline, tid == 0);
         return;
     }
     const uint64_t mask = __ballot(visible);
@@ -345,13 +356,20 @@
         }
         if constexpr (RANGES) PlaceBlock(C.D, C.args, smask, C.ModelCount);
     } else {
-        if (lane == 0) C.wave_masks[(size_t)blockIdx.x * 4u + wave] = mask;
-        if (tid == 0) C.block_counts[blockIdx.x] = __popcll(smask[0]) + __popcll(smask[1]) + __popcll(smask[2]) + __popcll(smask[3]);
+        if (lane == 0) C.wave_masks[(size_t)block * 4u + wave] = mask;
+        if (tid == 0) C.block_counts[block] = __popcll(smask[0]) + __popcll(smask[1]) + __popcll(smask[2]) + __popcll(smask[3]);
     }
     if constexpr (VIEWS) FinishViews<SINGLE_BLOCK>(C.V, C.args, C.ModelCount, C.index_base, svmask);
-    ur::timeline_exit(C.timeline, tid == 0);
-}
-
+    if constexpr (!RIDING) ur::timeline_exit(C.timeline, tid == 0);
+}
+
+template <bool SINGLE_BLOCK, bool RANGES, bool VIEWS = false>
+__global__ __launch_bounds__(256) void cull_kernel(CullArgs<RANGES, VIEWS> C)
+{
+    cull_block<SINGLE_BLOCK, RANGES, VIEWS, false>(C, nullptr, nullptr);
+}
+
+#ifndef UR_CULL_BLOCK_ONLY
 template <bool VIEWS, class Args> __device__ __forceinline__ const auto* SelectRow(const Args* C, const CullArgs<true>* W)
 {
     if constexpr (VIEWS) return W;
@@ -512,15 +530,11 @@
 
 DrawParams draw_params(const ur_draw_ranges& d) { return {d.offsets, static_cast<uint8_t*>(d.commands), d.counts, d.range_count}; }
 
-template <bool VIEWS>
-int cull_launches(ur_ctx* ctx, const uint32_t* constants, const ur_float4* bounds, const float* hzb, const ur_mip_desc* mips,
-                  void* indirect_args, uint32_t* stats2, uint32_t* visible_idx, uint32_t* visible_count, uint32_t index_base,
-                  const ur_draw_ranges* draws, const ur_cull_view* views, uint32_t view_count)
-{
-    if constexpr (!VIEWS) view_count = 0;
-    CullArgs<true, VIEWS> P{};
+inline void fill_cull_params(CullParams& P, const ur_ctx* ctx, const uint32_t* constants, const ur_float4* bounds, const float* hzb, const ur_mip_desc* mips,
+                             void* indirect_args, uint32_t* stats2, uint32_t* visible_idx, uint32_t* visible_count, uint32_t index_base)
+{
     static_assert(sizeof(float4) * 6 + sizeof(float) * 16 + 6 * 4 == UR_CULL_CONSTANT_DWORDS * 4, "46 dwords");
-    std::memcpy(static_cast<CullParams*>(&P), constants, UR_CULL_CONSTANT_DWORDS * 4);
+    std::memcpy(&P, constants, UR_CULL_CONSTANT_DWORDS * 4);
     P.bounds = reinterpret_cast<const float4*>(bounds);
     P.hzb = hzb;
     P.args = static_cast<uint8_t*>(indirect_args);
@@ -529,13 +543,23 @@
     P.visible_count = visible_count;
     P.index_base = index_base;
     P.store_flavour = (uint32_t)ctx->opt.cull_store;
-    P.timeline = P.ModelCount != 0 ? ur::next_timeline_pair(ctx) : nullptr;
     if (P.HZBEnabled != 0) {
         for (uint32_t m = 0; m < P.HZBMipCount && m < UR_MAX_HZB_MIPS; ++m) {
             P.mip_offset[m] = mips[m].offset;
             P.mip_width[m] = mips[m].width;
         }
     }
+}
+
+template <bool VIEWS>
+int cull_launches(ur_ctx* ctx, const uint32_t* constants, const ur_float4* bounds, const float* hzb, const ur_mip_desc* mips,
+                  void* indirect_args, uint32_t* stats2, uint32_t* visible_idx, uint32_t* visible_count, uint32_t index_base,
+                  const ur_draw_ranges* draws, const ur_cull_view* views, uint32_t view_count)
+{
+    if constexpr (!VIEWS) view_count = 0;
+    CullArgs<true, VIEWS> P{};
+    fill_cull_params(P, ctx, constants, bounds, hzb, mips, indirect_args, stats2, visible_idx, visible_count, index_base);
+    P.timeline = P.ModelCount != 0 ? ur::next_timeline_pair(ctx) : nullptr;
     if (draws) P.D = draw_params(*draws);
     if constexpr (VIEWS) {
         P.V.count = view_count;
@@ -624,4 +648,6 @@
     return UR_OK;
 }
 
-}
+#endif
+
+}
diff --git a/unclerenderer_amd/csrc/debug_print.hip b/unclerenderer_amd/csrc/debug_print.hip
--- a/unclerenderer_amd/csrc/debug_print.hip
+++ b/unclerenderer_amd/csrc/debug_print.hip
@@ -204,6 +204,7 @@
 
 int launch_debug_print_reset(ur_ctx* ctx, void* buffer, uint32_t* stats)
 {
+    UR_FLUSH_CULL(ctx);
     hipLaunchKernelGGL(debug_print_reset_kernel, dim3(1), dim3(64), 0, ctx->stream, static_cast<uint32_t*>(buffer), stats);
     UR_HIP_TRY(hipGetLastError());
     return UR_OK;
@@ -211,6 +212,7 @@
 
 int launch_debug_print_stats(ur_ctx* ctx, const uint32_t* stats, void* buffer)
 {
+    UR_FLUSH_CULL(ctx);
     hipLaunchKernelGGL(debug_print_stats_kernel, dim3(1), dim3(64), 0, ctx->stream, stats, static_cast<uint32_t*>(buffer));
     UR_HIP_TRY(hipGetLastError());
     return UR_OK;
@@ -218,6 +220,7 @@
 
 int launch_debug_print_text(ur_ctx* ctx, void* buffer, uint32_t x, uint32_t y, uint32_t color, const char* text, uint32_t length)
 {
+    UR_FLUSH_CULL(ctx);
     uint32_t n = 0;
     while (n < length && text[n] != 0) ++n;
     for (uint32_t at = 0; at < n; at += kTextChunk) {
@@ -235,6 +238,7 @@
                             const uint8_t* atlas_r8, uint32_t atlas_w, uint32_t atlas_h, const void* buffer, uint32_t* ldr_inout, uint32_t w,
                             uint32_t row0, uint32_t rows)
 {
+    UR_FLUSH_CULL(ctx);
     if (rows == 0) return UR_OK;
     DrawParams p{};
     p.glyphs = glyphs; p.atlas = atlas_r8; p.buf = static_cast<const uint32_t*>(buffer); p.ldr = ldr_inout;
diff --git a/unclerenderer_amd/csrc/frame/HotPathRenderer.cpp b/unclerenderer_amd/csrc/frame/HotPathRenderer.cpp
--- a/unclerenderer_amd/csrc/frame/HotPathRenderer.cpp
+++ b/unclerenderer_amd/csrc/frame/HotPathRenderer.cpp
@@ -1003,7 +1003,9 @@
         if (!f->LightEvents.empty() && ur_time_next_cull(f->Cmd.GetContext(), f->LightEvents[f->LightCount % f->LightEvents.size()].first) == UR_OK)
             f->bStartOnCull = true;
     }
+    f->Cmd.GetContext()->cull_ride_on = chain_with_lighting && !f->bStartOnCull && f->Cmd.GetContext()->opt.cull_ride != 0;
     const int rc = f->Renderer.RenderFrame(f->Cmd, R, K, O);
+    f->Cmd.GetContext()->cull_ride_on = false;
     (void)ur_time_next_cull(f->Cmd.GetContext(), nullptr);
     if (tail_with_lighting) {
         const int rc2 = ur_defer_hzb_tail(f->Cmd.GetContext(), 0);
diff --git a/unclerenderer_amd/csrc/gbuffer_resolve.hip b/unclerenderer_amd/csrc/gbuffer_resolve.hip
--- a/unclerenderer_amd/csrc/gbuffer_resolve.hip
+++ b/unclerenderer_amd/csrc/gbuffer_resolve.hip
@@ -344,6 +344,7 @@
     }
     if (!aligned(materials, 16)) { ur::set_error("%s: a misaligned material table (16 bytes)", who); return UR_EINVAL; }
     const uint32_t n = w * rows;
+    UR_FLUSH_CULL(ctx);
     if (parts & UR_GBUFFER_PART_RASTER) {
         rc = ur::launch_visibility_raster(ctx, view, projection, draws, depth, targets->keys, w, h, row0, rows, key_bits, (flags & UR_DEPTH_QUANTIZE_D24) != 0u, stats6);
         if (rc != UR_OK) return rc;
diff --git a/unclerenderer_amd/csrc/hzb.hip b/unclerenderer_amd/csrc/hzb.hip
--- a/unclerenderer_amd/csrc/hzb.hip
+++ b/unclerenderer_amd/csrc/hzb.hip
@@ -113,12 +113,14 @@
 namespace ur {
 
 static HzbTail make_tail(float* hzb, const ur_mip_desc* mips, uint32_t mip_count, uint32_t mip);
+static bool chain_is_wide_plus_tail(const ur_mip_desc* mips, uint32_t mip_count);
 
 int launch_build_hzb(ur_ctx* ctx, const float* depth, uint32_t src_w, uint32_t src_h, float* hzb, const ur_mip_desc* mips,
                      uint32_t mip_count)
 {
     {
-        const int rc = flush_hzb_tail(ctx);
+        const bool holds_whole = ctx->defer_hzb_tail && ctx->defer_hzb_wide && ctx->hzb_done != nullptr && chain_is_wide_plus_tail(mips, mip_count);
+        const int rc = flush_held(ctx, true, holds_whole);
         if (rc != UR_OK) return rc;
     }
     uint32_t mip = 0;
@@ -205,7 +207,7 @@
                           uint32_t piece_row0, uint32_t piece_rows)
 {
     {
-        const int rc = flush_hzb_tail(ctx);
+        const int rc = flush_held(ctx, true, ctx->defer_hzb_tail && ctx->defer_hzb_wide);
         if (rc != UR_OK) return rc;
     }
     if (!chain_is_wide_plus_tail(mips, mip_count)) {
@@ -236,7 +238,7 @@
 int launch_build_hzb_tail(ur_ctx* ctx, float* hzb, const ur_mip_desc* mips, uint32_t mip_count)
 {
     {
-        const int rc = flush_hzb_tail(ctx);
+        const int rc = flush_held(ctx, true, false);
         if (rc != UR_OK) return rc;
     }
     if (!chain_is_wide_plus_tail(mips, mip_count)) {
@@ -248,7 +250,7 @@
     return UR_OK;
 }
 
-int flush_hzb_tail(ur_ctx* ctx)
+int launch_pending_chain(ur_ctx* ctx)
 {
     if (ctx->hzb_wide_pending) {
         ctx->hzb_wide_pending = false;
diff --git a/unclerenderer_amd/csrc/lighting.hip b/unclerenderer_amd/csrc/lighting.hip
--- a/unclerenderer_amd/csrc/lighting.hip
+++ b/unclerenderer_amd/csrc/lighting.hip
@@ -2,6 +2,8 @@
 #include "lighting_device.h"
 #include "ur_device.h"
 #include "hzb_tail.h"
+#define UR_CULL_BLOCK_ONLY
+#include "cull_kernels.h"
 
 #include <cstring>
 
@@ -187,7 +189,7 @@
     return e;
 }
 template <class P>
-__device__ __forceinline__ uint32_t dyn_claim(P kp, uint32_t* work, uint32_t* dynT, uint32_t c, uint32_t lane)
+__device__ __forceinline__ uint32_t dyn_claim(P kp, uint32_t* work, uint32_t* dynT, uint32_t c, uint32_t lane, uint32_t wg )
 {
     const uint32_t d = c - kp->hot.staticClaims;
     const uint32_t s = min(d >> kp->bal.dynShift, kDynSlots - 1u);
@@ -200,7 +202,7 @@
             uint32_t out = kDynEnd;
             if (dyn_slot_wait(dynT + (k - 1u), kp) < kDynEnd && k + 1u < kDynSlots) {
                 uint32_t v = 0;
-                if (lane == 0) v = __hip_atomic_fetch_add(kp->bal.words + (blockIdx.x >> 3) * ur::kClaimWordStride, 1u, __ATOMIC_RELAXED, __HIP_MEMORY_SCOPE_AGENT);
+                if (lane == 0) v = __hip_atomic_fetch_add(kp->bal.words + (wg >> 3) * ur::kClaimWordStride, 1u, __ATOMIC_RELAXED, __HIP_MEMORY_SCOPE_AGENT);
                 v = __builtin_amdgcn_readfirstlane(v);
                 if (v < dyn_slot_load(work + 5)) out = kp->bal.staticTiles + ((dyn_slot_load(work + 4) + v) << kp->bal.dynShift);
                 else {
@@ -235,13 +237,33 @@
 };
 
 template <int MODE, bool SHADOWS, bool IRR_LDS, int WPB, bool RIDE_ALL>
-__global__ __launch_bounds__(64 * WPB, 1) void lighting_stream_kernel(LightingParams p, ur::HzbTail hzbTail, HzbRide hzbRide)
+__global__ __launch_bounds__(64 * WPB, 1) void lighting_stream_kernel(LightingParams p, ur::HzbTail hzbTail, HzbRide hzbRide, ur::CullParams cull)
 {
     static_assert(MODE != ur::UR_MODE_SKY, "sky-only uses the per-tile kernel");
     ur::warm_kernarg<sizeof(LightingParams)>();
     extern __shared__ __attribute__((aligned(16))) unsigned char smem[];
     ur::timeline_entry(p.timeline);
-    if (blockIdx.x >= p.hot.groups) {
+    constexpr bool kCullRides = WPB == 16 && !RIDE_ALL;
+    uint32_t wg = blockIdx.x;
+    if constexpr (kCullRides) asm("s_sub_u32 %0, %0, %1" : "+s"(wg) : "s"(p.wgShift) : "scc");
+    if (wg >= p.hot.groups) {
+        if constexpr (kCullRides) {
+            if (__builtin_expect(wg == 0xFFFFFFFFu, 0)) {
+                if (threadIdx.x < 256u) {
+                    auto ka = __builtin_amdgcn_kernarg_segment_ptr();
+                    asm volatile("" : "+s"(ka));
+                    typedef const __attribute__((address_space(4))) char* KBytes;
+                    typedef const __attribute__((address_space(4))) HzbRide* KRide;
+                    constexpr uint32_t kRideAt = sizeof(LightingParams) + sizeof(ur::HzbTail);
+                    constexpr uint32_t kCullAt = (kRideAt + (uint32_t)sizeof(HzbRide) + (uint32_t)alignof(ur::CullParams) - 1u) & ~((uint32_t)alignof(ur::CullParams) - 1u);
+                    static_assert(sizeof(HzbRide) % 8 == 0 && kCullLdsBytes <= kLdsTiles, "the fourth argument's place; the cull's LDS fits in front of the tile buffers");
+                    uint32_t* gate = ((KRide)((KBytes)ka + kRideAt))->done + ur::kCullGateWord;
+                    const ur::CullParams* C = (const ur::CullParams*)((KBytes)ka + kCullAt);
+                    cull_block<true, false, false, true>(*C, smem, gate);
+                }
+                return;
+            }
+        }
         if constexpr (WPB == 16) {
             static_assert(kLdsTiles + 16u * 2u * kTileBytes >= (ur::kTailTexels + ur::kTailTexels / 2u) * sizeof(float), "the tail's two level buffers fit the launch's LDS");
             float* bufA = reinterpret_cast<float*>(smem);
@@ -269,6 +291,7 @@
                         if (gave_up) __hip_atomic_store(done + 1, 1u, __ATOMIC_RELAXED, __HIP_MEMORY_SCOPE_AGENT);
                     } else {
                         __hip_atomic_store(done, 0u, __ATOMIC_RELAXED, __HIP_MEMORY_SCOPE_AGENT);
+                        __hip_atomic_store(done + ur::kCullGateWord, 0u, __ATOMIC_RELAXED, __HIP_MEMORY_SCOPE_AGENT);
                     }
                 }
                 __syncthreads();
@@ -307,7 +330,7 @@
         ih = p.env[t0]; ih10 = p.env[t0 + 1u]; ih01 = p.env[t0 + irrE]; ih11 = p.env[t0 + irrE + 1u];
     }
     constexpr uint32_t cs = kChunkShift, cmask = (1u << cs) - 1u;
-    const uint32_t chunkStride = p.hot.groups << cs, base = blockIdx.x << cs;
+    const uint32_t chunkStride = p.hot.groups << cs, base = wg << cs;
     uint32_t tile = (wave >> cs) * chunkStride + base + (wave & cmask);
     uint32_t tile1 = ((wave + WPB) >> cs) * chunkStride + base + ((wave + WPB) & cmask);
     const bool have0 = tile < p.hot.numTiles;
@@ -343,7 +366,7 @@
     {
         if (threadIdx.x == 0) { work[0] = 2u * WPB; work[1] = 0u; work[2] = 0u; work[3] = 0u; }
         if (p.bal.poolChunks != 0u && threadIdx.x < kDynSlots) {
-            const uint32_t q8 = blockIdx.x & ~7u, nq = min(8u, p.hot.groups - q8), j = blockIdx.x - q8, la = p.bal.lookahead;
+            const uint32_t q8 = wg & ~7u, nq = min(8u, p.hot.groups - q8), j = wg - q8, la = p.bal.lookahead;
             const uint32_t P0 = (uint32_t)(((unsigned long long)q8 * p.bal.poolMagic) >> 32);
             const uint32_t P1 = (uint32_t)(((unsigned long long)(q8 + nq) * p.bal.poolMagic) >> 32);
             const uint32_t first = P0 + la * nq;
@@ -398,7 +421,21 @@
             if (pieces != 0u) {
                 const uint32_t gx = ride->grid_x, groups = p.hot.groups;
                 float* sh2 = reinterpret_cast<float*>(smem + kLdsHzb) + (RIDE_ALL ? wave * 80u : 0u);
-                const uint32_t first = RIDE_ALL ? blockIdx.x + (kWalkers - 1u - wave) * groups : blockIdx.x, step = RIDE_ALL ? groups * kWalkers : groups;
+                const uint32_t first = RIDE_ALL ? wg + (kWalkers - 1u - wave) * groups : wg, step = RIDE_ALL ? groups * kWalkers : groups;
+                if constexpr (kCullRides) {
+                    if (fresh_params()->wgShift != 0u) {
+                        const uint32_t* gate = ride->done + ur::kCullGateWord;
+                        const uint32_t limit = ride->spin_limit;
+                        uint32_t spins = 0;
+                        while (__builtin_amdgcn_readfirstlane(__hip_atomic_load(gate, __ATOMIC_RELAXED, __HIP_MEMORY_SCOPE_AGENT)) < 4u) {
+                            __builtin_amdgcn_s_sleep(32);
+                            if (++spins > limit) {
+                                __hip_atomic_store(ride->timed_out, 1u, __ATOMIC_RELAXED, __HIP_MEMORY_SCOPE_SYSTEM);
+                                break;
+                            }
+                        }
+                    }
+                }
                 __builtin_amdgcn_s_setprio(3);
                 for (uint32_t piece = first; piece < pieces; piece += step) {
                     const uint32_t by = piece / gx, bx = piece - by * gx;
@@ -429,7 +466,7 @@
 #define UR_PREFETCH_POINT()                                                                                              \
     do {                                                                                                                 \
         const uint32_t c = __builtin_amdgcn_readfirstlane(claim);             \
-        if (__builtin_expect(c >= p.hot.staticClaims, 0)) tile2 = dyn_claim(kp, work, dynT, c, lane);       \
+        if (__builtin_expect(c >= p.hot.staticClaims, 0)) tile2 = dyn_claim(kp, work, dynT, c, lane, base >> cs);        \
         else tile2 = (c >> cs) * chunkStride + base + (c & cmask);                                                       \
         uint32_t in_band;                                                                                                \
         asm("s_cmp_lt_u32 %1, %2\n\ts_cselect_b32 %0, 1, 0" : "=s"(in_band) : "s"(tile2), "s"(p.hot.numTiles) : "scc"); \
@@ -733,7 +770,7 @@
     }
 }
 
-typedef void (*kernel_t)(LightingParams, ur::HzbTail, HzbRide);
+typedef void (*kernel_t)(LightingParams, ur::HzbTail, HzbRide, ur::CullParams);
 #define UR_WAVES(M, S, I) lighting_stream_kernel<M, S, I, 12, true>, lighting_stream_kernel<M, S, I, 12, false>, lighting_stream_kernel<M, S, I, 16, true>, lighting_stream_kernel<M, S, I, 16, false>
 #define UR_MODE(M) UR_WAVES(M, true, true), UR_WAVES(M, true, false), UR_WAVES(M, false, true), UR_WAVES(M, false, false)
 const kernel_t kStreamKernels[32] = {UR_MODE(ur::UR_MODE_LIGHTING), UR_MODE(ur::UR_MODE_FUSED)};
@@ -750,13 +787,20 @@
     const ur_ctx::Options& o = ctx->opt;
     const StreamPlan s = plan_stream({ctx->cu_count, o.leave_cus, o.ride_walkers, o.balance, o.balance_pool_16ths, o.balance_chunk_shift, o.debug_hzb_ride_stall,
                                       params.W, params.rows, wpb, ctx->hzb_tail_pending, ctx->hzb_wide_pending, ctx->pending_wide_grid_x,
-                                      ctx->pending_wide_grid_y, ctx->claim_words != nullptr ? kClaimWords : 0u});
+                                      ctx->pending_wide_grid_y, ctx->claim_words != nullptr ? kClaimWords : 0u, ctx->cull_pending});
     LightingParams p = params;
     p.timeline = next_timeline_pair(ctx);
     StreamHot& h = p.hot;
     h.tilesX = s.tilesX; h.numTiles = s.numTiles; h.tilesXMagic = s.tilesXMagic; h.groups = s.groups; h.staticClaims = s.staticClaims;
+    p.wgShift = s.rides_cull ? 1u : 0u;
     p.bal = Balance{};
     if (s.poolChunks != 0u) p.bal = Balance{s.poolChunks, s.staticTiles, s.dynShift, s.lookahead, s.poolMagic, ctx->claim_words, ctx->claim_timed_out_dev};
+    if (s.flush_cull_first) {
+        const int frc = launch_pending_cull(ctx);
+        if (frc != UR_OK) return frc;
+    }
+    CullParams cull{};
+    if (s.rides_cull) { cull = ctx->pending_cull; ctx->cull_pending = false; }
     HzbTail tail{};
     HzbRide ride{};
     if (s.carry_tail) { tail = ctx->pending_tail; ctx->hzb_tail_pending = false; }
@@ -781,7 +825,7 @@
         if (dev >= 0) attr_set[form][dev] = true;
     }
     std::memcpy(ctx->last_schedule, s.reported, sizeof(ctx->last_schedule));
-    launch_timed(ctx, kern, dim3(s.groups + (s.carry_tail ? 1u : 0u)), dim3(64 * wpb), lds, p, tail, ride);
+    launch_timed(ctx, kern, dim3(s.groups + (s.carry_tail ? 1u : 0u) + (s.rides_cull ? 1u : 0u)), dim3(64 * wpb), lds, p, tail, ride, cull);
     return UR_OK;
 }
 
diff --git a/unclerenderer_amd/csrc/lighting_host.hip b/unclerenderer_amd/csrc/lighting_host.hip
--- a/unclerenderer_amd/csrc/lighting_host.hip
+++ b/unclerenderer_amd/csrc/lighting_host.hip
@@ -197,7 +197,7 @@
         }
     }
     if (!streamed) {
-        const int frc = flush_hzb_tail(ctx);
+        const int frc = flush_held(ctx, true, false);
         if (frc != UR_OK) return frc;
         launch_lighting_tiled(ctx, p, mode, shadows);
     }
diff --git a/unclerenderer_amd/csrc/lighting_params.h b/unclerenderer_amd/csrc/lighting_params.h
--- a/unclerenderer_amd/csrc/lighting_params.h
+++ b/unclerenderer_amd/csrc/lighting_params.h
@@ -70,6 +70,7 @@
     float skyScatterR[3];
     float skyMie[3];
     float sunAttenuation;
+    uint32_t wgShift;
     StreamHot hot;
     Balance bal;
     unsigned long long* timeline;
diff --git a/unclerenderer_amd/csrc/lighting_plan.cpp b/unclerenderer_amd/csrc/lighting_plan.cpp
--- a/unclerenderer_amd/csrc/lighting_plan.cpp
+++ b/unclerenderer_amd/csrc/lighting_plan.cpp
@@ -61,6 +61,8 @@
     } else {
         s.flush_first = in.wide_pending;
     }
+    s.rides_cull = in.cull_pending && s.carry_tail && s.rides && s.ride_pieces != 0u && s.ride_walkers == 1u && in.debug_hzb_ride_stall == 0;
+    s.flush_cull_first = in.cull_pending && !s.rides_cull;
     const uint32_t groups = std::min<uint32_t>((uint32_t)std::max(1, cus - (s.carry_tail ? 1 : 0) - leave_cus), (s.numTiles + WPB - 1) / WPB);
     s.groups = groups;
     s.ride_want = groups + (in.debug_hzb_ride_stall != 0 ? 1u : 0u);
@@ -96,4 +98,17 @@
     return s;
 }
 
+bool cull_holds(const CullCall& c)
+{
+    return c.ride_on && c.option != 0 && c.n >= 1u && c.n <= kCullBlock && !c.ranges && c.views == 0u && !c.timed;
 }
+
+FlushOrder flush_order(bool cull_pending, bool chain_pending, bool flush_chain, bool keep_cull)
+{
+    const bool chain = chain_pending && flush_chain;
+    const bool cull = cull_pending && (chain || !keep_cull);
+    if (cull) return {Held::cull, chain ? Held::chain : Held::none};
+    return {chain ? Held::chain : Held::none, Held::none};
+}
+
+}
diff --git a/unclerenderer_amd/csrc/lighting_plan.h b/unclerenderer_amd/csrc/lighting_plan.h
--- a/unclerenderer_amd/csrc/lighting_plan.h
+++ b/unclerenderer_amd/csrc/lighting_plan.h
@@ -28,6 +28,7 @@
     bool wide_pending;
     uint32_t wide_grid_x, wide_grid_y;
     uint32_t claim_words;
+    bool cull_pending;
 };
 
 struct StreamPlan {
@@ -37,6 +38,8 @@
     bool rides;
     uint32_t ride_pieces, ride_grid_x, ride_walkers, ride_want, ride_spin_limit;
     bool flush_first;
+    bool rides_cull;
+    bool flush_cull_first;
     uint32_t staticClaims;
     uint32_t poolChunks, staticTiles, dynShift, lookahead;
     unsigned long long poolMagic;
@@ -46,4 +49,19 @@
 
 uint32_t ride_walkers(uint32_t pieces, uint32_t tiles, uint32_t lighting_groups, uint32_t wpb, int forced);
 
+constexpr uint32_t kCullBlock = 256;
+struct CullCall {
+    bool ride_on;
+    int option;
+    uint32_t n;
+    bool ranges;
+    uint32_t views;
+    bool timed;
+};
+bool cull_holds(const CullCall& c);
+
+enum class Held : uint8_t { none, cull, chain };
+struct FlushOrder { Held first, second; };
+FlushOrder flush_order(bool cull_pending, bool chain_pending, bool flush_chain, bool keep_cull);
+
 }
diff --git a/unclerenderer_amd/csrc/post.hip b/unclerenderer_amd/csrc/post.hip
--- a/unclerenderer_amd/csrc/post.hip
+++ b/unclerenderer_amd/csrc/post.hip
@@ -415,6 +415,7 @@
     auto aligned = [](const void* q, uintptr_t m) { return (reinterpret_cast<uintptr_t>(q) & m) == 0u; };
     const bool pairs = (w % 2u) == 0u && aligned(src, mode == In::Hdr ? 15u : 7u) && aligned(out, 7u) && aligned(above, 15u) && aligned(below, 15u);
     const uint32_t px = pairs ? 2u : 1u;
+    UR_FLUSH_CULL(ctx);
     const dim3 grid((w + 256u * px - 1u) / (256u * px), grid_y);
     if (halo) {
         const CasHaloParams q{p, above, below};
@@ -463,6 +464,7 @@
     }
     AeParams p = ae_params(constants, w, h, prev_ev, out_ev);
     p.hdr = reinterpret_cast<const half4_t*>(hdr_full);
+    UR_FLUSH_CULL(ctx);
     hipLaunchKernelGGL(auto_exposure_kernel, dim3(1), dim3(256), 0, ctx->stream, p);
     UR_HIP_TRY(hipGetLastError());
     return UR_OK;
@@ -493,6 +495,7 @@
     if (overlaps(hdr_band, (size_t)w * rows * 8u, record, ur_post_record_bytes(w))) { ur::set_error("ur_pack_post_record: the record overlaps the band"); return UR_EINVAL; }
     PackParams p{reinterpret_cast<const half4_t*>(hdr_band), static_cast<half4_t*>(record), w, h, row0, rows};
     const uint32_t n = 2u * w + kTapTexels;
+    UR_FLUSH_CULL(ctx);
     hipLaunchKernelGGL(post_record_kernel, dim3((n + 255u) / 256u), dim3(256), 0, ctx->stream, p);
     UR_HIP_TRY(hipGetLastError());
     return UR_OK;
@@ -515,6 +518,7 @@
     q.records = static_cast<const half4_t*>(records);
     q.record_texels = 2u * w + kTapTexels;
     q.band_rows = h / n_ranks;
+    UR_FLUSH_CULL(ctx);
     hipLaunchKernelGGL(ae_records_kernel, dim3(1), dim3(256), 0, ctx->stream, q);
     UR_HIP_TRY(hipGetLastError());
     return UR_OK;
diff --git a/unclerenderer_amd/csrc/raster.hip b/unclerenderer_amd/csrc/raster.hip
--- a/unclerenderer_amd/csrc/raster.hip
+++ b/unclerenderer_amd/csrc/raster.hip
@@ -446,6 +446,7 @@
 int launch_raster(ur_ctx* ctx, const float* m0, const float* m1, const ur_raster_draws* draws, uint32_t* map, uint32_t n, uint32_t w, uint32_t h, float clear,
                   uint32_t* stats, const VisArgs* vis)
 {
+    UR_FLUSH_CULL(ctx);
     const ur_draw_ranges* rg = draws->ranges;
     const bool list = draws->visible_idx != nullptr;
     const uint32_t head = min((uint32_t)((16u - (reinterpret_cast<uintptr_t>(map) & 15u)) & 15u) / 4u, n);
@@ -525,6 +526,7 @@
 {
     if (!ctx) { ur::set_error("ur_raster_reserve: null context"); return UR_EINVAL; }
     if (max_large_work_items == ctx->raster_queue_cap) return UR_OK;
+    UR_FLUSH_CULL(ctx);
     UR_HIP_TRY(hipStreamSynchronize(ctx->stream));
     if (ctx->raster_queue) (void)hipFree(ctx->raster_queue);
     ctx->raster_queue = nullptr;
diff --git a/unclerenderer_amd/csrc/stream_ceiling.hip b/unclerenderer_amd/csrc/stream_ceiling.hip
--- a/unclerenderer_amd/csrc/stream_ceiling.hip
+++ b/unclerenderer_amd/csrc/stream_ceiling.hip
@@ -28,6 +28,7 @@
     }
     StreamPtrs p{{static_cast<const float4*>(in0), static_cast<const float4*>(in1), static_cast<const float4*>(in2), static_cast<const float4*>(in3)},
                  static_cast<float4*>(out), (uint32_t)elements16};
+    UR_FLUSH_CULL(ctx);
     const dim3 grid((uint32_t)((elements16 + 255u) / 256u));
     if (stop_event != nullptr)
         hipExtLaunchKernelGGL(stream4_kernel, grid, dim3(256), 0, ctx->stream, static_cast<hipEvent_t>(start_event), static_cast<hipEvent_t>(stop_event), 0, p);
diff --git a/unclerenderer_amd/csrc/taa.hip b/unclerenderer_amd/csrc/taa.hip
--- a/unclerenderer_amd/csrc/taa.hip
+++ b/unclerenderer_amd/csrc/taa.hip
@@ -228,6 +228,7 @@
     const int rc = fill_params("ur_temporal_aa", p, ctx, current_frame, history_band, output_band, history_weight, use_history, w, h, row0, rows);
     if (rc != UR_OK) return rc;
     if (rows == 0) return UR_OK;
+    UR_FLUSH_CULL(ctx);
     hipLaunchKernelGGL(taa_strip_kernel<NoPost>, dim3((w + 255u) / 256u, (rows + kStripRows - 1u) / kStripRows), dim3(256), 0, ctx->stream, p, NoPost{});
     UR_HIP_TRY(hipGetLastError());
     return UR_OK;
@@ -249,6 +250,7 @@
     tm.enable_auto_exposure = tonemap->EnableAutoExposure;
     tm.exposure = tonemap->Exposure;
     tm.inv_gamma = 1.0f / (tonemap->Gamma > 1e-3f ? tonemap->Gamma : 1e-3f);
+    UR_FLUSH_CULL(ctx);
     const dim3 grid((w + 255u) / 256u, (rows + kStripRows - 1u) / kStripRows);
     if (ctx->opt.taa_tonemap_history_store == 0) hipLaunchKernelGGL(taa_strip_kernel<TonemapPost<true>>, grid, dim3(256), 0, ctx->stream, p, TonemapPost<true>{tm});
     else hipLaunchKernelGGL(taa_strip_kernel<TonemapPost<false>>, grid, dim3(256), 0, ctx->stream, p, TonemapPost<false>{tm});
@@ -278,6 +280,7 @@
     }
     const TaaRecordParams p{reinterpret_cast<const u32x2_t*>(hdr_band), use_history ? reinterpret_cast<const u32x2_t*>(history_read_band) : nullptr,
                             static_cast<u32x2_t*>(record), w, rows};
+    UR_FLUSH_CULL(ctx);
     hipLaunchKernelGGL(taa_record_kernel, dim3((uint32_t)(((uint64_t)4u * w + 255u) / 256u)), dim3(256), 0, ctx->stream, p);
     UR_HIP_TRY(hipGetLastError());
     return UR_OK;
@@ -346,6 +349,7 @@
     const int rc = fill_band_params("ur_temporal_aa_halo", q, grid_y, ctx, current_band, cur_above, cur_below, history_band, output_band, above2, hist_above, below2,
                                     hist_below, resolved_above, resolved_below, history_weight, use_history, w, h, row0, rows);
     if (rc != UR_OK) return rc;
+    UR_FLUSH_CULL(ctx);
     hipLaunchKernelGGL(taa_band_kernel<NoPost>, dim3((w + 255u) / 256u, grid_y), dim3(256), 0, ctx->stream, q, NoPost{});
     UR_HIP_TRY(hipGetLastError());
     return UR_OK;
@@ -370,6 +374,7 @@
     tm.enable_auto_exposure = tonemap->EnableAutoExposure;
     tm.exposure = tonemap->Exposure;
     tm.inv_gamma = 1.0f / (tonemap->Gamma > 1e-3f ? tonemap->Gamma : 1e-3f);
+    UR_FLUSH_CULL(ctx);
     hipLaunchKernelGGL(taa_band_kernel<TonemapPost<true>>, dim3((w + 255u) / 256u, grid_y), dim3(256), 0, ctx->stream, q, TonemapPost<true>{tm});
     UR_HIP_TRY(hipGetLastError());
     return UR_OK;
diff --git a/unclerenderer_amd/csrc/tonemap.hip b/unclerenderer_amd/csrc/tonemap.hip
--- a/unclerenderer_amd/csrc/tonemap.hip
+++ b/unclerenderer_amd/csrc/tonemap.hip
@@ -57,6 +57,7 @@
     p.enable_auto_exposure = constants->EnableAutoExposure;
     p.exposure = constants->Exposure;
     p.inv_gamma = 1.0f / (constants->Gamma > 1e-3f ? constants->Gamma : 1e-3f);
+    UR_FLUSH_CULL(ctx);
     const bool aligned = ((reinterpret_cast<uintptr_t>(hdr) & 15u) == 0u) && ((reinterpret_cast<uintptr_t>(out_rgba8) & 7u) == 0u);
     if (aligned && n >= 2u) {
         if (n < (24u << 20)) hipLaunchKernelGGL(tonemap_pairs_kernel<1>, dim3((uint32_t)((n / 2u * 2u + 511u) / 512u)), dim3(256), 0, ctx->stream, p);
diff --git a/unclerenderer_amd/csrc/ur_api.hip b/unclerenderer_amd/csrc/ur_api.hip
--- a/unclerenderer_amd/csrc/ur_api.hip
+++ b/unclerenderer_amd/csrc/ur_api.hip
@@ -41,9 +41,10 @@
     }
     if (!ctx || !ctx->hzb_timed_out || *ctx->hzb_timed_out == 0u) return UR_OK;
     *ctx->hzb_timed_out = 0u;
-    (void)hipMemsetAsync(ctx->hzb_done, 0, 64, ctx->stream);
-    set_error("%s: the tail of a Build HZB chain that rode a Lighting launch gave up waiting for its producers: the HZB's small levels are stale — "
-              "build it again (reported once; the context is usable)", who);
+    (void)hipMemsetAsync(ctx->hzb_done, 0, kHzbDoneBytes, ctx->stream);
+    set_error("%s: the tail of a Build HZB chain that rode a Lighting launch gave up waiting for its producers (the HZB's small levels are stale), or a "
+              "walker of that chain gave up waiting for the cull riding in front of it (that cull may have read rewritten levels) — "
+              "build the HZB again (reported once; the context is usable)", who);
     return UR_ETIMEOUT;
 }
 
@@ -159,7 +160,7 @@
         ur_destroy(ctx);
         return nullptr;
     }
-    if (hipMalloc(&ctx->hzb_done, 64) != hipSuccess || hipMemset(ctx->hzb_done, 0, 64) != hipSuccess) {
+    if (hipMalloc(&ctx->hzb_done, ur::kHzbDoneBytes) != hipSuccess || hipMemset(ctx->hzb_done, 0, ur::kHzbDoneBytes) != hipSuccess) {
         set_error("ur_create: HZB arrival counter allocation failed");
         ur_destroy(ctx);
         return nullptr;
@@ -200,6 +201,7 @@
     if (!ctx) return;
     ctx->hzb_tail_pending = false;
     ctx->hzb_wide_pending = false;
+    ctx->cull_pending = false;
     if (ctx->hzb_done) (void)hipFree(ctx->hzb_done);
     if (ctx->claim_words) (void)hipFree(ctx->claim_words);
     if (ctx->hzb_timed_out) (void)hipHostFree(const_cast<uint32_t*>(ctx->hzb_timed_out));
@@ -266,6 +268,7 @@
     case UR_OPT_BALANCE_CHUNK_SHIFT: o = {&O::balance_chunk_shift, 2, 6, false}; return true;
     case UR_OPT_DEBUG_HZB_RIDE_STALL: o = {&O::debug_hzb_ride_stall, 0, 1, false}; return true;
     case UR_OPT_TAA_TONEMAP_HISTORY_STORE: o = {&O::taa_tonemap_history_store, 0, 1, false}; return true;
+    case UR_OPT_CULL_RIDE: o = {&O::cull_ride, 0, 1, false}; return true;
     default: return false;
     }
 }
@@ -297,7 +300,7 @@
     if (!ctx) { set_error("ur_flush: null context"); return UR_EINVAL; }
     const int trc = ur::check_hzb_timeout(ctx, "ur_flush");
     if (trc != UR_OK) return trc;
-    return ur::flush_hzb_tail(ctx);
+    return ur::flush_held(ctx, true, false);
 }
 
 int ur_debug_lighting_schedule(const ur_ctx* ctx, uint32_t out8[8])
@@ -318,6 +321,7 @@
 {
     if (!ctx) return UR_EINVAL;
     if (max_instances <= ctx->ws_instances) return UR_OK;
+    UR_FLUSH_CULL(ctx);
     UR_HIP_TRY(hipStreamSynchronize(ctx->stream));
     if (ctx->block_counts) (void)hipFree(ctx->block_counts);
     if (ctx->wave_masks) (void)hipFree(ctx->wave_masks);
@@ -665,6 +669,7 @@
         return UR_EINVAL;
     }
     if (mode != UR_GATHER_RING && mode != UR_GATHER_DIRECT) { set_error("ur_allgather_rows: mode %d (0 ring, 1 direct)", mode); return UR_EINVAL; }
+    UR_FLUSH_CULL(ctx);
     const size_t band_bytes = (size_t)row_bytes * (h / n_ranks);
     char* base = reinterpret_cast<char*>(image);
     const char* send = base + band_bytes * rank;
diff --git a/unclerenderer_amd/csrc/ur_internal.h b/unclerenderer_amd/csrc/ur_internal.h
--- a/unclerenderer_amd/csrc/ur_internal.h
+++ b/unclerenderer_amd/csrc/ur_internal.h
@@ -18,6 +18,26 @@
     uint32_t W[kTailMaxLevels], H[kTailMaxLevels];
     uint32_t magic[kTailMaxLevels];
 };
+struct CullParams {
+    float4 FrustumPlanes[6];
+    float ViewProjection[16];
+    uint32_t ModelCount, HZBEnabled, HZBMipCount, HZBWidth, HZBHeight, DebugPrintEnabled;
+    const float4* bounds;
+    const float* hzb;
+    uint8_t* args;
+    uint32_t* stats;
+    uint32_t* visible_idx;
+    uint32_t* visible_count;
+    uint32_t* block_counts;
+    uint64_t* wave_masks;
+    uint32_t index_base;
+    uint32_t store_flavour;
+    uint32_t record_valid;
+    uint32_t mip_offset[UR_MAX_HZB_MIPS];
+    uint32_t mip_width[UR_MAX_HZB_MIPS];
+    unsigned long long* timeline;
+};
+constexpr uint32_t kHzbDoneBytes = 256, kCullGateWord = 32;
 }
 #include "hzb_wide.h"
 
@@ -43,13 +63,16 @@
     unsigned long long* timeline = nullptr;
     uint32_t timeline_cap = 0, timeline_pos = 0;
     uint32_t* hzb_done = nullptr;
+    bool cull_ride_on = false;
+    bool cull_pending = false;
+    ur::CullParams pending_cull{};
     volatile uint32_t* hzb_timed_out = nullptr;
     uint32_t* hzb_timed_out_dev = nullptr;
     hipEvent_t time_start = nullptr, time_stop = nullptr;
     hipEvent_t time_cull_stop = nullptr;
     bool time_cull_carried = false;
     struct Options {
-        int lighting_stream = 1, lighting_wpb = 16, tiled_waves = 6, leave_cus = 0, ride_walkers = 0, cull_store = 3;
+        int lighting_stream = 1, lighting_wpb = 16, tiled_waves = 6, leave_cus = 0, ride_walkers = 0, cull_store = 3, cull_ride = 1;
         int balance = 1, balance_pool_16ths = 3, balance_chunk_shift = 4;
         int debug_hzb_ride_stall = 0;
         int taa_tonemap_history_store = 0;
@@ -121,7 +144,16 @@
     if (!ctx->timeline || ctx->timeline_pos >= ctx->timeline_cap) return nullptr;
     return ctx->timeline + 2u * (size_t)ctx->timeline_pos++;
 }
-int flush_hzb_tail(ur_ctx* ctx);
+int flush_held(ur_ctx* ctx, bool flush_chain, bool keep_cull);
+inline int flush_hzb_tail(ur_ctx* ctx) { return flush_held(ctx, true, true); }
+inline int flush_cull(ur_ctx* ctx) { return flush_held(ctx, false, false); }
+#define UR_FLUSH_CULL(ctx)                             \
+    do {                                               \
+        const int _frc = ::ur::flush_cull(ctx);        \
+        if (_frc != UR_OK) return _frc;                \
+    } while (0)
+int launch_pending_chain(ur_ctx* ctx);
+int launch_pending_cull(ur_ctx* ctx);
 int check_hzb_timeout(ur_ctx* ctx, const char* who);
 
 }
diff --git a/unclerenderer_amd/lib.py b/unclerenderer_amd/lib.py
--- a/unclerenderer_amd/lib.py
+++ b/unclerenderer_amd/lib.py
@@ -21,6 +21,7 @@
 UR_OPT_LIGHTING_STREAM, UR_OPT_LIGHTING_WAVES_PER_WG, UR_OPT_LIGHTING_TILED_WAVES, UR_OPT_LIGHTING_LEAVE_CUS, UR_OPT_RIDE_WALKERS = 1, 2, 3, 4, 5
 UR_OPT_CULL_STORE, UR_OPT_LIGHTING_BALANCE, UR_OPT_BALANCE_POOL_16THS, UR_OPT_BALANCE_CHUNK_SHIFT, UR_OPT_DEBUG_HZB_RIDE_STALL = 7, 8, 9, 10, 11
 UR_OPT_TAA_TONEMAP_HISTORY_STORE = 12
+UR_OPT_CULL_RIDE = 13
 
 
 class MipDesc(C.Structure):
```

Result: no change. 108,600 (median of 2 runs) (-0.4%).
